# zeahmed/NeuralASR

Hardware: AMD Instinct MI355X
Metric: audio-frames/sec (fwd+bwd+CTC+Adam) at batch 16 per GPU (higher is better)
Workload: dtype f32

## Files before the change

### neuralasr_amd/build.py

```python
import os
import subprocess
import sys
from concurrent.futures import ThreadPoolExecutor

HERE = os.path.dirname(os.path.abspath(__file__))
CSRC = os.path.join(HERE, 'csrc')
LIB = os.path.join(HERE, 'libnasr.so')
KT_LIB = os.path.join(HERE, 'libnasr_kt.so')
KT_DIR = os.path.join(HERE, '..', 'tests', 'kernel_harness')
KT_SRCS = ['harness.hip', 'rec_harness.hip']
KT_HEADERS = [os.path.join(KT_DIR, 'arena.h')]
KT_OBJS = ['gemm.o', 'gemm_tph.o', 'optim.o', 'lstm.o', 'lstm_persist.o', 'lstm_wide.o']
SOURCES = ['gemm.hip', 'gemm_tph.hip', 'lstm.hip', 'rows.hip', 'lstm_persist.hip', 'lstm_wide.hip', 'ctc.hip', 'dense.hip', 'optim.hip', 'nasr_layout.hip',
           'nasr_rec.hip', 'nasr_batch.hip', 'nasr_pass.hip', 'nasr_stream.hip', 'nasr_lstm.hip', 'nasr_api.hip', 'nasr_comm.hip', 'beam.cpp',
           'wavenet.hip', 'nasr_wavenet.hip', 'las.hip', 'las_beam.hip', 'nasr_las.hip', 'mfcc.hip', 'nasr_fz.hip', 'resample.hip', 'wave_aug.hip']
HEADERS = [os.path.join(CSRC, 'kernels.h'), os.path.join(CSRC, 'lstm_device.h'), os.path.join(CSRC, 'nasr_ctx.h'), os.path.join(CSRC, 'nasr_lstm.h'), os.path.join(CSRC, 'wavenet.h'), os.path.join(CSRC, 'las.h'), os.path.join(CSRC, 'las_beam.h'), os.path.join(CSRC, 'resample.h'), os.path.join(CSRC, 'wave_aug.h'),
           os.path.join(CSRC, 'mfcc.h'), os.path.join(CSRC, 'nasr_fz.h'), os.path.join(HERE, '..', 'include', 'nasr.h')]
FLAGS = ['--offload-arch=gfx950', '-O3', '-std=c++17', '-fPIC', '-Wall', '-Wno-unused-function']
EXTRA_FLAGS = {'wave_aug.hip': ['-fno-slp-vectorize']}


def _hipcc():
    for c in (os.environ.get('HIPCC'), '/opt/rocm/bin/hipcc', 'hipcc'):
        if c and (os.path.isabs(c) and os.path.exists(c) or not os.path.isabs(c)):
            return c
    return 'hipcc'


def _stale(target, deps):
    if not os.path.exists(target):
        return True
    t = os.path.getmtime(target)
    return any(os.path.getmtime(d) > t for d in deps if os.path.exists(d))


def build(force=False, verbose=False):
    hipcc = _hipcc()
    bdir = os.path.join(HERE, 'build')
    os.makedirs(bdir, exist_ok=True)
    jobs = []
    objs = []
    for s in SOURCES:
        src = os.path.join(CSRC, s)
        obj = os.path.join(bdir, os.path.splitext(s)[0] + '.o')
        objs.append(obj)
        if force or _stale(obj, [src] + HEADERS):
            jobs.append([hipcc] + FLAGS + EXTRA_FLAGS.get(s, []) + ['-c', src, '-o', obj])

    def run(cmd):
        if verbose:
            print(' '.join(cmd), flush=True)
        r = subprocess.run(cmd, capture_output=True, text=True)
        if r.returncode != 0:
            raise RuntimeError('hipcc failed:\n' + ' '.join(cmd) + '\n' + r.stdout + r.stderr)
        if verbose and r.stderr.strip():
            print(r.stderr)

    kt_objs = []
    for s in KT_SRCS:
        src = os.path.join(KT_DIR, s)
        obj = os.path.join(bdir, 'kt_' + os.path.splitext(s)[0] + '.o')
        kt_objs.append(obj)
        if force or _stale(obj, [src] + KT_HEADERS + HEADERS):
            jobs.append([hipcc] + FLAGS + ['-c', src, '-o', obj])

    with ThreadPoolExecutor(max_workers=min(4, max(1, len(jobs)))) as ex:
        list(ex.map(run, jobs))
    if force or jobs or _stale(LIB, objs):
        run([hipcc, '--offload-arch=gfx950', '-shared', '-fPIC', '-o', LIB] + objs + ['-lpthread'])
    kt_objs += [os.path.join(bdir, o) for o in KT_OBJS]
    if force or jobs or _stale(KT_LIB, kt_objs):
        run([hipcc, '--offload-arch=gfx950', '-shared', '-fPIC', '-o', KT_LIB] + kt_objs)
    return LIB


if __name__ == '__main__':
    print(build(force='--force' in sys.argv, verbose=True))
```

### neuralasr_amd/csrc/ctc.hip

```cpp
#include "kernels.h"

#include <cmath>
#include <cstdlib>
#include <type_traits>

namespace nasr {

constexpr float NEG = -1e30f;
typedef __attribute__((address_space(3))) void* lds_ptr_t;
typedef const __attribute__((address_space(1))) void* gbl_ptr_t;

__device__ __forceinline__ float ldf(const float* base, unsigned byteoff) {
  return *reinterpret_cast<const float*>(reinterpret_cast<const char*>(base) + byteoff);
}
__device__ __forceinline__ void stf(float* base, unsigned byteoff, float v) {
  *reinterpret_cast<float*>(reinterpret_cast<char*>(base) + byteoff) = v;
}

__device__ __forceinline__ float lse3(float a, float b, float c) {
  const float m = fmaxf(a, fmaxf(b, c));
  const float L2E = 1.44269504088896341f, LN2 = 0.69314718055994531f;
  const float s = __builtin_amdgcn_exp2f((a - m) * L2E) + __builtin_amdgcn_exp2f((b - m) * L2E) +
                  __builtin_amdgcn_exp2f((c - m) * L2E);
  return m + __builtin_amdgcn_logf(s) * LN2;
}

__device__ __forceinline__ float lane_up1(float v, float edge) {
  return __int_as_float(__builtin_amdgcn_update_dpp(__float_as_int(edge), __float_as_int(v), 0x138, 0xf, 0xf, false));
}
__device__ __forceinline__ float lane_down1(float v, float edge) {
  return __int_as_float(__builtin_amdgcn_update_dpp(__float_as_int(edge), __float_as_int(v), 0x130, 0xf, 0xf, false));
}

__device__ __forceinline__ float wave_max(float v) {
#pragma unroll
  for (int o = 32; o > 0; o >>= 1) v = fmaxf(v, __shfl_xor(v, o));
  return v;
}
__device__ __forceinline__ float wave_max_dpp(float v) {
  auto dpp = [](float x, auto ctrl) {
    return __int_as_float(__builtin_amdgcn_update_dpp(__float_as_int(x), __float_as_int(x), decltype(ctrl)::value, 0xf, 0xf, false));
  };
  v = fmaxf(v, dpp(v, std::integral_constant<int, 0xB1>{}));
  v = fmaxf(v, dpp(v, std::integral_constant<int, 0x4E>{}));
  v = fmaxf(v, dpp(v, std::integral_constant<int, 0x141>{}));
  v = fmaxf(v, dpp(v, std::integral_constant<int, 0x140>{}));
  const int vi = __float_as_int(v);
  const float r0 = __int_as_float(__builtin_amdgcn_readlane(vi, 0)), r1 = __int_as_float(__builtin_amdgcn_readlane(vi, 16));
  const float r2 = __int_as_float(__builtin_amdgcn_readlane(vi, 32)), r3 = __int_as_float(__builtin_amdgcn_readlane(vi, 48));
  return fmaxf(fmaxf(r0, r1), fmaxf(r2, r3));
}
__device__ __forceinline__ float wave_sum(float v) {
#pragma unroll
  for (int o = 32; o > 0; o >>= 1) v += __shfl_xor(v, o);
  return v;
}

static bool ctc_fast_ok(const CtcDims& d) { return d.lprobs && d.goff && d.Cp == 32 && d.C <= 31 && d.KS >= 2; }

__global__ __launch_bounds__(256) void ctc_logz_kernel(const float* __restrict__ logits, const int* __restrict__ seq_len,
                                                       float* __restrict__ logz, float* __restrict__ lprobs, int Tp, int B, int Bp,
                                                       int C, int Cp) {
  const int row = blockIdx.x * 4 + (threadIdx.x >> 6);
  const int lane = threadIdx.x & 63;
  if (row >= Tp * Bp) return;
  const int t = row / Bp, b = row % Bp;
  if (b >= B || t >= seq_len[b]) return;
  const float* x = logits + (size_t)row * Cp;
  float m = NEG;
  for (int c = lane; c < C; c += 64) m = fmaxf(m, x[c]);
  m = wave_max(m);
  float s = 0.f;
  for (int c = lane; c < C; c += 64) s += __expf(x[c] - m);
  s = wave_sum(s);
  const float z = m + __logf(s);
  if (lane == 0) logz[row] = z;
  if (lprobs)
    for (int c = lane; c < Cp; c += 64) lprobs[(size_t)row * Cp + c] = c < C ? (x[c] - z) * 1.44269504088896341f : NEG;
}

void launch_ctc_logz(const CtcDims& d, const float* logits, const int* seq_len, float* logz, hipStream_t st) {
  const int rows = d.Tp * d.Bp;
  hipLaunchKernelGGL(ctc_logz_kernel, dim3((rows + 3) / 4), dim3(256), 0, st, logits, seq_len, logz, ctc_fast_ok(d) ? d.lprobs : nullptr,
                     d.Tp, d.B, d.Bp, d.C, d.Cp);
}

template <int KS>
__device__ __forceinline__ void ctc_ab_log(
    const float* __restrict__ logits, const float* __restrict__ logz, const int* __restrict__ labels,
    const int* __restrict__ label_len, const int* __restrict__ seq_len, float* __restrict__ alpha,
    float* __restrict__ beta, double* __restrict__ aoff, double* __restrict__ boff, float* __restrict__ nll,
    double* __restrict__ logp_out, int Bp, int Cp, int C, int Lmax, int Tws, float* fin) {
  constexpr int G = 4;
  const int b = blockIdx.x;
  const int lane = threadIdx.x & 63, w = threadIdx.x >> 6;
  const int L = label_len[b], Tb = seq_len[b], S = 2 * L + 1;
  const int blank = C - 1;
  const int* lab = labels + (size_t)b * Lmax;

  int ext[KS];
  bool act[KS], skip[KS];
#pragma unroll
  for (int i = 0; i < KS; ++i) {
    const int s = lane * KS + i;
    act[i] = s < S;
    ext[i] = (act[i] && (s & 1)) ? lab[s >> 1] : blank;
  }
  const unsigned rstride = (unsigned)Bp * (unsigned)Cp;
  const float* lg = logits + (size_t)b * Cp;
  const float* lz = logz + b;
  auto emit = [&](int t, float (&e)[KS]) {
    const float z = ldf(lz, (unsigned)t * (unsigned)Bp * 4u);
    float v[KS];
#pragma unroll
    for (int i = 0; i < KS; ++i) v[i] = ldf(lg, ((unsigned)t * rstride + (unsigned)ext[i]) * 4u);
#pragma unroll
    for (int i = 0; i < KS; ++i) e[i] = act[i] ? v[i] - z : NEG;
  };
  auto emit_raw = [&](int t, float (&v)[KS], float& z) {
    z = ldf(lz, (unsigned)t * (unsigned)Bp * 4u);
#pragma unroll
    for (int i = 0; i < KS; ++i) v[i] = ldf(lg, ((unsigned)t * rstride + (unsigned)ext[i]) * 4u);
  };
  auto emit_finish = [&](float (&v)[KS], float z, float (&e)[KS]) {
    asm volatile("" : "+v"(z));
#pragma unroll
    for (int i = 0; i < KS; ++i) {
      float x = v[i];
      asm volatile("" : "+v"(x));
      e[i] = act[i] ? x - z : NEG;
    }
  };
  float* ws = (w == 0 ? alpha : beta) + (size_t)b * Tws * KS * 64;
  double* off = (w == 0 ? aoff : boff) + (size_t)b * Tws;
  auto store = [&](int t, const float (&a)[KS], double o) {
#pragma unroll
    for (int i = 0; i < KS; ++i) stf(ws, (((unsigned)t * KS + i) * 64u + (unsigned)lane) * 4u, a[i]);
    if (lane == 0) off[t] = o;
  };
  auto renorm = [&](float (&a)[KS], double& o) {
    float m = a[0];
#pragma unroll
    for (int i = 1; i < KS; ++i) m = fmaxf(m, a[i]);
    m = wave_max_dpp(m);
#pragma unroll
    for (int i = 0; i < KS; ++i) a[i] = a[i] > 0.5f * NEG ? a[i] - m : NEG;
    o += (double)m;
  };

  if (w == 0) {
#pragma unroll
    for (int i = 0; i < KS; ++i) {
      const int s = lane * KS + i;
      const int e2 = (act[i] && s >= 2 && (s & 1)) ? lab[(s >> 1) - 1] : blank;
      skip[i] = act[i] && s >= 2 && ext[i] != blank && ext[i] != e2;
    }
    float a[KS], e[G][KS];
    double A = 0.0;
    emit(0, e[0]);
#pragma unroll
    for (int i = 0; i < KS; ++i) {
      const int s = lane * KS + i;
      a[i] = (s < 2 && act[i]) ? e[0][i] : NEG;
    }
    store(0, a, A);
#pragma unroll
    for (int k = 0; k < G; ++k) emit(min(1 + k, Tb - 1), e[k]);
    for (int t0 = 1; t0 < Tb; t0 += G) {
      float vn[G][KS], zn[G];
#pragma unroll
      for (int k = 0; k < G; ++k) emit_raw(min(t0 + G + k, Tb - 1), vn[k], zn[k]);
      renorm(a, A);
#pragma unroll
      for (int k = 0; k < G; ++k) {
        const int t = t0 + k;
        const bool live = t < Tb;
        float p1 = lane_up1(a[KS - 1], NEG);
        float p2 = (KS >= 2) ? lane_up1(a[KS >= 2 ? KS - 2 : 0], NEG) : __shfl_up(a[0], 2);
        if (KS == 1 && lane <= 1) p2 = NEG;
        float na[KS];
#pragma unroll
        for (int i = 0; i < KS; ++i) {
          const float x1 = (i >= 1) ? a[i >= 1 ? i - 1 : 0] : p1;
          const float x2 = (i >= 2) ? a[i >= 2 ? i - 2 : 0] : (i == 1 ? p1 : p2);
          na[i] = e[k][i] + lse3(a[i], x1, skip[i] ? x2 : NEG);
        }
#pragma unroll
        for (int i = 0; i < KS; ++i) a[i] = live ? na[i] : a[i];
        store(t, a, A);
      }
      asm volatile("" ::: "memory");
#pragma unroll
      for (int k = 0; k < G; ++k) emit_finish(vn[k], zn[k], e[k]);
    }
#pragma unroll
    for (int i = 0; i < KS; ++i) fin[lane * KS + i] = a[i];
    __builtin_amdgcn_s_waitcnt(0xc07f);
    if (lane == 0) {
      const float x = fin[S - 1];
      const float y = S > 1 ? fin[S - 2] : NEG;
      const double lp = A + (double)lse3(x, y, NEG);
      logp_out[b] = lp;
      nll[b] = (float)(-lp);
    }
  } else {
#pragma unroll
    for (int i = 0; i < KS; ++i) {
      const int s = lane * KS + i;
      const int e2 = (s + 2 < S && (s & 1)) ? lab[(s >> 1) + 1] : blank;
      skip[i] = (s + 2 < S) && e2 != blank && e2 != ext[i];
    }
    float bt[KS], e[G][KS];
    double Bo = 0.0;
#pragma unroll
    for (int i = 0; i < KS; ++i) {
      const int s = lane * KS + i;
      bt[i] = (act[i] && (s == S - 1 || s == S - 2)) ? 0.f : NEG;
    }
    store(Tb - 1, bt, Bo);
#pragma unroll
    for (int k = 0; k < G; ++k) emit(max(Tb - 1 - k, 0), e[k]);
    for (int t0 = Tb - 2; t0 >= 0; t0 -= G) {
      float vn[G][KS], zn[G];
#pragma unroll
      for (int k = 0; k < G; ++k) emit_raw(max(t0 - G - k + 1, 0), vn[k], zn[k]);
      renorm(bt, Bo);
#pragma unroll
      for (int k = 0; k < G; ++k) {
        const int t = t0 - k;
        const bool live = t >= 0;
        float bb[KS];
#pragma unroll
        for (int i = 0; i < KS; ++i) bb[i] = bt[i] + e[k][i];
        float n1 = lane_down1(bb[0], NEG);
        float n2 = (KS >= 2) ? lane_down1(bb[KS >= 2 ? 1 : 0], NEG) : __shfl_down(bb[0], 2);
        if (KS == 1 && lane >= 62) n2 = NEG;
        float nb[KS];
#pragma unroll
        for (int i = 0; i < KS; ++i) {
          const float x1 = (i + 1 < KS) ? bb[i + 1 < KS ? i + 1 : 0] : n1;
          const float x2 = (i + 2 < KS) ? bb[i + 2 < KS ? i + 2 : 0] : (i + 1 < KS ? n1 : n2);
          nb[i] = lse3(bb[i], x1, skip[i] ? x2 : NEG);
        }
#pragma unroll
        for (int i = 0; i < KS; ++i) bt[i] = live ? nb[i] : bt[i];
        if (live) store(t, bt, Bo);
      }
      asm volatile("" ::: "memory");
#pragma unroll
      for (int k = 0; k < G; ++k) emit_finish(vn[k], zn[k], e[k]);
    }
  }
}

constexpr int FAST_G = 4, FAST_CH = 32, FAST_RING = 64;

typedef float fast_f2 __attribute__((ext_vector_type(2)));
typedef float fast_f3 __attribute__((ext_vector_type(3)));
typedef float fast_f4 __attribute__((ext_vector_type(4)));
template <int KS>
__device__ __forceinline__ void fast_store(float* base, unsigned voff, const float (&a)[KS]) {
#pragma unroll
  for (int j = 0; j + 4 <= KS; j += 4) {
    const fast_f4 v = {a[j], a[j + 1], a[j + 2], a[j + 3]};
    asm volatile("global_store_dwordx4 %0, %1, %2 offset:%3\n\ts_nop 1" : : "v"(voff), "v"(v), "s"(base), "n"(j * 4) : "memory");
  }
  constexpr int j = KS & ~3;
  if constexpr (KS % 4 == 3) {
    const fast_f3 v = {a[j], a[j + 1], a[j + 2]};
    asm volatile("global_store_dwordx3 %0, %1, %2 offset:%3\n\ts_nop 1" : : "v"(voff), "v"(v), "s"(base), "n"(j * 4) : "memory");
  } else if constexpr (KS % 4 == 2) {
    const fast_f2 v = {a[j], a[j + 1]};
    asm volatile("global_store_dwordx2 %0, %1, %2 offset:%3" : : "v"(voff), "v"(v), "s"(base), "n"(j * 4) : "memory");
  } else if constexpr (KS % 4 == 1) {
    asm volatile("global_store_dword %0, %1, %2 offset:%3" : : "v"(voff), "v"(a[j]), "s"(base), "n"(j * 4) : "memory");
  }
}
__device__ __forceinline__ float fast_up(float v) { return lane_up1(v, NEG); }
__device__ __forceinline__ float fast_down(float v) { return lane_down1(v, NEG); }

__device__ __forceinline__ float lse3_2(float a, float b, float c) {
  const float mx = __builtin_fmaxf(a, __builtin_fmaxf(b, c));
  const float md = __builtin_amdgcn_fmed3f(a, b, c);
  const float mn = __builtin_fminf(a, __builtin_fminf(b, c));
  const float s = 1.f + __builtin_amdgcn_exp2f(md - mx) + __builtin_amdgcn_exp2f(mn - mx);
  return mx + __builtin_amdgcn_logf(s);
}

template <int KS, bool fwd>
__device__ __forceinline__ void ctc_fast_walk(const int* __restrict__ labels, const int* __restrict__ label_len,
                                              const int* __restrict__ seq_len, float* __restrict__ alpha, float* __restrict__ beta,
                                              double* __restrict__ goff, float* __restrict__ nll, double* __restrict__ logp_out,
                                              const float* __restrict__ lprobs, int Bp, int C, int Lmax, int Tws, int KG, float* ring,
                                              float* fin, int* sync) {
  static_assert(KS >= 2, "two states per lane at least: the skip transition then never reaches past the neighbour lane");
  constexpr int G = FAST_G;
  constexpr double LN2 = 0.693147180559945309417;
  const int b = blockIdx.x;
  const int lane = threadIdx.x & 63, w = fwd ? 0 : 1;
  const int L = label_len[b], Tb = seq_len[b], S = 2 * L + 1;
  const int blank = C - 1;
  const int* lab = labels + (size_t)b * Lmax;
  int ext[KS];
  bool skip[KS];
#pragma unroll
  for (int i = 0; i < KS; ++i) {
    const int s = lane * KS + i;
    const bool act = s < S;
    ext[i] = act ? ((s & 1) ? lab[s >> 1] : blank) : 31;
    if (fwd) {
      const int e2 = (act && s >= 2 && (s & 1)) ? lab[(s >> 1) - 1] : blank;
      skip[i] = act && s >= 2 && ext[i] != blank && ext[i] != e2;
    } else {
      const int e2 = (s + 2 < S && (s & 1)) ? lab[(s >> 1) + 1] : blank;
      skip[i] = (s + 2 < S) && e2 != blank && e2 != ext[i];
    }
  }
  const int npos = Tb - 1;
  float* rg = ring + w * (FAST_RING * 32);
  auto read_group = [&](int g, float (&e)[G][KS]) {
    asm volatile("" ::: "memory");
    const float* r0 = rg + ((G * g) & (FAST_RING - 1)) * 32;
#pragma unroll
    for (int i = 0; i < KS; ++i)
#pragma unroll
      for (int k = 0; k < G; ++k) e[k][i] = r0[k * 32 + ext[i]];
    asm volatile("" ::: "memory");
  };
  const unsigned sync_lds = (unsigned)(size_t)((lds_ptr_t)sync);
  auto wait_ready = [&](int n) {
    for (unsigned spin = 0; spin < (1u << 24); ++spin) {
      int v;
      asm volatile("ds_read_b32 %0, %1\n\ts_waitcnt lgkmcnt(0)" : "=v"(v) : "v"(sync_lds) : "memory");
      if (v >= n) break;
      __builtin_amdgcn_s_sleep(1);
    }
  };
  float* ws = (fwd ? alpha : beta) + (size_t)b * Tws * KS * 64;
  double* go = goff + ((size_t)b * 2 + w) * KG;
  constexpr unsigned ROWB = 64u * KS * 4u;
  const unsigned lane_off = (unsigned)lane * (KS * 4u);
  auto store = [&](int t, const float (&a)[KS]) { fast_store<KS>(ws, lane_off + (unsigned)t * ROWB, a); };

  float a[KS];
  double A = 0.0;
  if (fwd) {
    const float* y0 = lprobs + (size_t)b * 32;
#pragma unroll
    for (int i = 0; i < KS; ++i) a[i] = (lane * KS + i < 2) ? y0[ext[i]] : NEG;
    store(0, a);
  } else {
#pragma unroll
    for (int i = 0; i < KS; ++i) {
      const int s = lane * KS + i;
      a[i] = (s < S && (s == S - 1 || s == S - 2)) ? 0.f : NEG;
    }
    store(Tb - 1, a);
  }
  if (lane == 0) go[0] = 0.0;
  auto group = [&](int g, float (&e)[G][KS], float (&en)[G][KS], auto maskedc) {
    constexpr bool MASKED = decltype(maskedc)::value;
    const int p0 = G * g;
    read_group(g + 1, en);
    {
      float m = a[0];
#pragma unroll
      for (int i = 1; i < KS; ++i) m = fmaxf(m, a[i]);
      m = wave_max_dpp(m);
#pragma unroll
      for (int i = 0; i < KS; ++i) a[i] = a[i] > 0.5f * NEG ? a[i] - m : NEG;
      A += (double)m;
      if (lane == 0) go[g + 1] = A;
    }
#pragma unroll
    for (int k = 0; k < G; ++k) {
      float na[KS];
      if (fwd) {
        const float p1 = fast_up(a[KS - 1]), p2 = fast_up(a[KS - 2]);
#pragma unroll
        for (int i = 0; i < KS; ++i) {
          const float x1 = (i >= 1) ? a[i >= 1 ? i - 1 : 0] : p1;
          const float x2 = (i >= 2) ? a[i >= 2 ? i - 2 : 0] : (i == 1 ? p1 : p2);
          na[i] = e[k][i] + lse3_2(a[i], x1, skip[i] ? x2 : NEG);
        }
      } else {
        float bb[KS];
#pragma unroll
        for (int i = 0; i < KS; ++i) bb[i] = a[i] + e[k][i];
        const float n1 = fast_down(bb[0]), n2 = fast_down(bb[1]);
#pragma unroll
        for (int i = 0; i < KS; ++i) {
          const float x1 = (i + 1 < KS) ? bb[i + 1 < KS ? i + 1 : 0] : n1;
          const float x2 = (i + 2 < KS) ? bb[i + 2 < KS ? i + 2 : 0] : (i + 1 < KS ? n1 : n2);
          na[i] = lse3_2(bb[i], x1, skip[i] ? x2 : NEG);
        }
      }
      if constexpr (MASKED) {
        const bool live = p0 + k < npos;
#pragma unroll
        for (int i = 0; i < KS; ++i) a[i] = live ? na[i] : a[i];
      } else {
#pragma unroll
        for (int i = 0; i < KS; ++i) a[i] = na[i];
      }
      store(fwd ? p0 + k + 1 : max(Tb - 2 - p0 - k, 0), a);
    }
  };
  if (npos > 0) {
    const int nch = (npos + FAST_CH - 1) / FAST_CH;
    wait_ready(1);
    float e[G][KS], en[G][KS];
    read_group(0, e);
    for (int c = 0; c < nch; ++c) {
      for (int gi = 0; gi < FAST_CH / G; gi += 2) {
        const int g = c * (FAST_CH / G) + gi;
        if (G * g >= npos) break;
        if (G * g + G <= npos) group(g, e, en, std::false_type{});
        else group(g, e, en, std::true_type{});
        if (G * (g + 1) >= npos) break;
        if (gi + 2 == FAST_CH / G && c + 1 < nch) wait_ready(c + 2);
        if (G * (g + 1) + G <= npos) group(g + 1, en, e, std::false_type{});
        else group(g + 1, en, e, std::true_type{});
      }
      asm volatile("s_waitcnt lgkmcnt(0)\n\tds_write_b32 %0, %1 offset:%2" : : "v"(sync_lds), "v"(c + 1), "n"(4 * (1 + w)) : "memory");
    }
  }
  if (fwd) {
#pragma unroll
    for (int i = 0; i < KS; ++i) fin[lane * KS + i] = a[i];
    __builtin_amdgcn_s_waitcnt(0xc07f);
    if (lane == 0) {
      const float x = fin[S - 1];
      const float y = S > 1 ? fin[S - 2] : NEG;
      const double lp = (A + (double)lse3_2(x, y, NEG)) * LN2;
      logp_out[b] = lp;
      nll[b] = (float)(-lp);
    }
  }
}

__device__ __forceinline__ void ctc_fast_loader(const float* __restrict__ lprobs, const int* __restrict__ seq_len, int Bp, float* ring,
                                                volatile int* sync) {
  const int b = blockIdx.x, lane = threadIdx.x & 63;
  const int Tb = seq_len[b], npos = Tb - 1;
  const int nch = (npos + FAST_CH - 1) / FAST_CH;
  const char* yb = reinterpret_cast<const char*>(lprobs + (size_t)b * 32);
  const unsigned rstride = (unsigned)Bp * 32u * 4u;
  for (int n = 0; n < nch; ++n) {
    if (n >= 2)
      for (unsigned spin = 0; (sync[1] < n - 1 || sync[2] < n - 1) && spin < (1u << 24); ++spin) __builtin_amdgcn_s_sleep(1);
#pragma unroll
    for (int w = 0; w < 2; ++w)
#pragma unroll
      for (int q = 0; q < 4; ++q) {
        const int p = min(FAST_CH * n + 8 * q + (lane >> 3), npos - 1);
        const int f = w == 0 ? p + 1 : Tb - 1 - p;
        const char* g = yb + (size_t)((unsigned)f * rstride) + (lane & 7) * 16;
        __builtin_amdgcn_global_load_lds((gbl_ptr_t)g, (lds_ptr_t)(ring + w * (FAST_RING * 32) + (((FAST_CH * n) & (FAST_RING - 1)) + 8 * q) * 32),
                                         16, 0, 0);
      }
    asm volatile("s_waitcnt vmcnt(0)" ::: "memory");
    if (lane == 0) sync[0] = n + 1;
  }
}

template <int KS, bool FAST>
__global__ __launch_bounds__(FAST ? 192 : 128) void ctc_alpha_beta_kernel(
    const float* __restrict__ logits, const float* __restrict__ logz, const float* __restrict__ lprobs,
    const int* __restrict__ labels, const int* __restrict__ label_len, const int* __restrict__ seq_len,
    float* __restrict__ alpha, float* __restrict__ beta, double* __restrict__ aoff, double* __restrict__ boff,
    double* __restrict__ goff, float* __restrict__ nll, double* __restrict__ logp_out, int Bp, int Cp, int C, int Lmax, int Tws,
    int KG) {
  __shared__ float fin[64 * KS];
  if constexpr (FAST) {
    __shared__ __attribute__((aligned(1024))) float ring[2 * FAST_RING * 32];
    __shared__ int sync[3];
    if (threadIdx.x < 3) sync[threadIdx.x] = 0;
    __syncthreads();
    constexpr int K2 = KS >= 2 ? KS : 2;
    const int w = __builtin_amdgcn_readfirstlane(threadIdx.x >> 6);
    if (w == 0)
      ctc_fast_walk<K2, true>(labels, label_len, seq_len, alpha, beta, goff, nll, logp_out, lprobs, Bp, C, Lmax, Tws, KG, ring, fin, sync);
    else if (w == 1)
      ctc_fast_walk<K2, false>(labels, label_len, seq_len, alpha, beta, goff, nll, logp_out, lprobs, Bp, C, Lmax, Tws, KG, ring, fin, sync);
    else
      ctc_fast_loader(lprobs, seq_len, Bp, ring, sync);
  } else {
    ctc_ab_log<KS>(logits, logz, labels, label_len, seq_len, alpha, beta, aoff, boff, nll, logp_out, Bp, Cp, C, Lmax, Tws, fin);
  }
}

void launch_ctc_alpha_beta(const CtcDims& d, const float* logits, const float* logz, const int* labels,
                           const int* label_len, const int* seq_len, float* alpha, float* beta, double* aoff,
                           double* boff, float* nll, double* logp, hipStream_t st) {
  const bool fast = ctc_fast_ok(d);
  const int KG = d.Tws / FAST_G + 3;
#define NASR_AB2(K, F)                                                                                                   \
  hipLaunchKernelGGL((ctc_alpha_beta_kernel<K, F>), dim3(d.B), dim3(F ? 192 : 128), 0, st, logits, logz, d.lprobs, labels, \
                     label_len, seq_len, alpha, beta, aoff, boff, d.goff, nll, logp, d.Bp, d.Cp, d.C, d.Lmax, d.Tws, KG)
#define NASR_AB(K)                                                                                                       \
  if (fast) NASR_AB2(K, true);                                                                                           \
  else NASR_AB2(K, false)
  switch (d.KS) {
    case 1: NASR_AB2(1, false); break;
    case 2: NASR_AB(2); break;
    case 3: NASR_AB(3); break;
    case 4: NASR_AB(4); break;
    case 5: NASR_AB(5); break;
    case 6: NASR_AB(6); break;
    case 7: NASR_AB(7); break;
    case 8: NASR_AB(8); break;
    case 9: case 10: case 11: case 12: NASR_AB(12); break;
    default: NASR_AB(16); break;
  }
#undef NASR_AB2
#undef NASR_AB
}

__global__ __launch_bounds__(256) void ctc_grad_kernel(float* __restrict__ logits, const float* __restrict__ logz,
                                                       const int* __restrict__ label_len,
                                                       const int* __restrict__ seq_len,
                                                       const int* __restrict__ cstart, const int* __restrict__ cpos,
                                                       const float* __restrict__ alpha, const float* __restrict__ beta,
                                                       const double* __restrict__ aoff, const double* __restrict__ boff,
                                                       const double* __restrict__ logp, const double* __restrict__ goff,
                                                       float scale, int Tp, int B, int Bp, int C, int Cp, int Lmax, int KS,
                                                       int Tws, int KG) {
  extern __shared__ __attribute__((aligned(16))) float wl_all[];
  const int wv = threadIdx.x >> 6, lane = threadIdx.x & 63;
  const int row = blockIdx.x * (blockDim.x >> 6) + wv;
  if (row >= Tp * Bp) return;
  const int t = row / Bp, b = row % Bp;
  float* x = logits + (size_t)row * Cp;
  if (b >= B || t >= seq_len[b]) {
    for (int c = lane; c < Cp; c += 64) x[c] = 0.f;
    return;
  }
  float* wl = wl_all + (size_t)wv * KS * 64;
  const int L = label_len[b], S = 2 * L + 1;
  const float* al = alpha + ((size_t)b * Tws + t) * KS * 64;
  const float* be = beta + ((size_t)b * Tws + t) * KS * 64;
  float blank = 0.f;
  if (goff) {
    const int Tb = seq_len[b];
    const int ga = t == 0 ? 0 : 1 + (t - 1) / FAST_G, gb = t == Tb - 1 ? 0 : 1 + (Tb - 2 - t) / FAST_G;
    const float coff2 = (float)(goff[(size_t)b * 2 * KG + ga] + goff[((size_t)b * 2 + 1) * KG + gb] - logp[b] * 1.44269504088896341);
    for (int i = 0; i < KS; ++i) {
      const int s = lane * KS + i;
      const float wgt = s < S ? exp2f(al[lane * KS + i] + be[lane * KS + i] + coff2) : 0.f;
      wl[s] = wgt;
      if (!(s & 1)) blank += wgt;
    }
  } else {
    const float coff = (float)(aoff[(size_t)b * Tws + t] + boff[(size_t)b * Tws + t] - logp[b]);
    for (int i = 0; i < KS; ++i) {
      const int s = lane * KS + i;
      const float wgt = s < S ? __expf(al[i * 64 + lane] + be[i * 64 + lane] + coff) : 0.f;
      wl[s] = wgt;
      if (!(s & 1)) blank += wgt;
    }
  }
  blank = wave_sum(blank);
  __builtin_amdgcn_s_waitcnt(0xc07f);
  const float z = logz[row];
  const int* cs = cstart + (size_t)b * (C + 1);
  const int* cp = cpos + (size_t)b * Lmax;
  for (int c = lane; c < Cp; c += 64) {
    float g = 0.f;
    if (c < C) {
      float post = blank;
      if (c < C - 1) {
        post = 0.f;
        const int j1 = cs[c + 1];
        for (int j = cs[c]; j < j1; ++j) post += wl[2 * cp[j] + 1];
      }
      g = (__expf(x[c] - z) - post) * scale;
    }
    x[c] = g;
  }
}

void launch_ctc_grad(const CtcDims& d, float* logits, const float* logz, const int* label_len, const int* seq_len,
                     const int* cstart, const int* cpos, const float* alpha, const float* beta, const double* aoff,
                     const double* boff, const double* logp, float scale, hipStream_t st) {
  const int rows = d.Tp * d.Bp;
  const int rpb = 4;
  hipLaunchKernelGGL(ctc_grad_kernel, dim3((rows + rpb - 1) / rpb), dim3(64 * rpb), (size_t)rpb * d.KS * 64 * 4, st, logits,
                     logz, label_len, seq_len, cstart, cpos, alpha, beta, aoff, boff, logp, ctc_fast_ok(d) ? d.goff : nullptr, scale,
                     d.Tp, d.B, d.Bp, d.C, d.Cp, d.Lmax, d.KS, d.Tws, d.Tws / FAST_G + 3);
}

__global__ void mean_kernel(const float* __restrict__ v, int n, float* __restrict__ out) {
  if (threadIdx.x == 0 && blockIdx.x == 0) {
    float s = 0.f;
    for (int i = 0; i < n; ++i) s += v[i];
    *out = s / (float)n;
  }
}
void launch_mean(const float* v, int n, float* out, hipStream_t st) {
  hipLaunchKernelGGL(mean_kernel, dim3(1), dim3(64), 0, st, v, n, out);
}

__global__ __launch_bounds__(256) void argmax_kernel(const float* __restrict__ logits, const int* __restrict__ seq_len,
                                                     int* __restrict__ am, int Tp, int B, int Bp, int C, int Cp) {
  const int row = blockIdx.x * 4 + (threadIdx.x >> 6);
  const int lane = threadIdx.x & 63;
  if (row >= Tp * Bp) return;
  const int t = row / Bp, b = row % Bp;
  if (b >= B || t >= seq_len[b]) return;
  const float* x = logits + (size_t)row * Cp;
  float best = -INFINITY;
  int bi = 0x7fffffff;
  for (int c = lane; c < C; c += 64) {
    const float v = x[c];
    if (v > best) { best = v; bi = c; }
  }
#pragma unroll
  for (int o = 32; o > 0; o >>= 1) {
    const float ov = __shfl_xor(best, o);
    const int oi = __shfl_xor(bi, o);
    if (ov > best || (ov == best && oi < bi)) { best = ov; bi = oi; }
  }
  if (lane == 0) am[row] = bi;
}

__global__ __launch_bounds__(64) void collapse_kernel(const int* __restrict__ am, const int* __restrict__ seq_len,
                                                      int* __restrict__ ids, int* __restrict__ lens, int Tp, int B, int Bp,
                                                      int blank) {
  const int b = blockIdx.x, lane = threadIdx.x;
  const int Tb = seq_len[b];
  int n = 0, carry = -1;
  for (int t0 = 0; t0 < Tb; t0 += 64) {
    const int t = t0 + lane;
    const int k = t < Tb ? am[t * Bp + b] : blank;
    int prev = __shfl_up(k, 1);
    if (lane == 0) prev = carry;
    const bool keep = t < Tb && k != prev && k != blank;
    const unsigned long long m = __ballot(keep);
    if (keep) ids[(size_t)b * Tp + n + __popcll(m & ((1ull << lane) - 1ull))] = k;
    n += __popcll(m);
    carry = __shfl(k, 63);
  }
  if (lane == 0) lens[b] = n;
}

void launch_greedy(const CtcDims& d, const float* logits, const int* seq_len, int* argmax_ws, int* ids, int* lens,
                   hipStream_t st) {
  const int rows = d.Tp * d.Bp;
  hipLaunchKernelGGL(argmax_kernel, dim3((rows + 3) / 4), dim3(256), 0, st, logits, seq_len, argmax_ws, d.Tp, d.B, d.Bp,
                     d.C, d.Cp);
  hipLaunchKernelGGL(collapse_kernel, dim3(d.B), dim3(64), 0, st, argmax_ws, seq_len, ids, lens, d.Tp, d.B, d.Bp, d.C - 1);
}

constexpr int ALIGN_G = 4;
constexpr int ALIGN_LDS_BYTES = 56 * 1024;
constexpr int align_bpf(int KS) { return KS <= 4 ? 8 : KS <= 8 ? 16 : 32; }
constexpr int align_words(int KS) { return align_bpf(KS) * ALIGN_G / 32; }
static int align_ks(int L) {
  const int KS = std::max(1, (2 * std::max(L, 0) + 1 + 63) / 64);
  return KS <= 1 ? 2 : KS <= 8 ? KS : (KS <= 12 ? 12 : 16);
}
static int align_groups(int F) { return (std::max(F, 1) - 1 + ALIGN_G - 1) / ALIGN_G; }

bool ctc_align_bp_in_lds(int F, int L) { return (size_t)align_groups(F) * 256 * align_words(align_ks(L)) <= (size_t)ALIGN_LDS_BYTES; }
size_t ctc_align_ws_words(int B, int F, int L) {
  return ctc_align_bp_in_lds(F, L) ? 0 : (size_t)B * align_groups(F) * 64 * align_words(align_ks(L));
}

template <int KS, bool LDSBP>
__global__ __launch_bounds__(64) void ctc_align_kernel(const float* __restrict__ logits, const float* __restrict__ logz,
                                                       const int* __restrict__ labels, const int* __restrict__ label_len,
                                                       const int* __restrict__ seq_len, unsigned* __restrict__ bpws,
                                                       size_t bp_stride, int* __restrict__ path, double* __restrict__ score,
                                                       int Tp, int Bp, int Cp, int C, int Lmax) {
  static_assert(KS >= 2 && KS <= 16, "two states per lane at least (the skip never reaches past the neighbour lane), 32 bits of back-pointers at most");
  constexpr int G = ALIGN_G, BPF = align_bpf(KS), W = align_words(KS);
  extern __shared__ __attribute__((aligned(16))) unsigned bplds[];
  __shared__ float fin[64 * KS];
  const int b = blockIdx.x, lane = threadIdx.x;
  const int L = label_len[b], F = seq_len[b], S = 2 * L + 1;
  const int blank = C - 1;
  const int* lab = labels + (size_t)b * Lmax;
  int ext[KS];
  bool act[KS], skip[KS];
#pragma unroll
  for (int i = 0; i < KS; ++i) {
    const int s = lane * KS + i;
    act[i] = s < S;
    ext[i] = (act[i] && (s & 1)) ? lab[s >> 1] : blank;
    const int e2 = (act[i] && s >= 2 && (s & 1)) ? lab[(s >> 1) - 1] : blank;
    skip[i] = act[i] && s >= 2 && ext[i] != blank && ext[i] != e2;
  }
  const unsigned rstride = (unsigned)Bp * (unsigned)Cp;
  const float* lg = logits + (size_t)b * Cp;
  auto gather = [&](int t, float (&x)[KS]) {
#pragma unroll
    for (int i = 0; i < KS; ++i) x[i] = ldf(lg, ((unsigned)t * rstride + (unsigned)ext[i]) * 4u);
  };
  unsigned* bp = LDSBP ? bplds : bpws + (size_t)b * bp_stride;
  const int ngroups = (F - 1 + G - 1) / G;

  constexpr int NB = KS <= 4 ? 8 : KS <= 8 ? 4 : 2, PF = G * NB;
  float v[KS], e[PF][KS];
  gather(0, e[0]);
#pragma unroll
  for (int i = 0; i < KS; ++i) v[i] = (act[i] && lane * KS + i < 2) ? e[0][i] : NEG;
#pragma unroll
  for (int k = 0; k < PF; ++k) gather(min(1 + k, F - 1), e[k]);
  for (int g0 = 0; g0 < ngroups; g0 += NB) {
    float vn[PF][KS];
#pragma unroll
    for (int k = 0; k < PF; ++k) gather(min(1 + G * g0 + PF + k, F - 1), vn[k]);
#pragma unroll
    for (int sub = 0; sub < NB; ++sub) {
      const int g = g0 + sub;
      if (g < ngroups) {
        const int t0 = 1 + G * g;
        {
          float m = v[0];
#pragma unroll
          for (int i = 1; i < KS; ++i) m = fmaxf(m, v[i]);
          m = wave_max_dpp(m);
#pragma unroll
          for (int i = 0; i < KS; ++i) v[i] = v[i] > 0.5f * NEG ? v[i] - m : NEG;
        }
        unsigned w[W];
#pragma unroll
        for (int j = 0; j < W; ++j) w[j] = 0u;
#pragma unroll
        for (int k = 0; k < G; ++k) {
          const bool live = t0 + k < F;
          const float p1 = lane_up1(v[KS - 1], NEG), p2 = lane_up1(v[KS - 2], NEG);
          float nv[KS];
          unsigned code = 0u;
#pragma unroll
          for (int i = 0; i < KS; ++i) {
            const float x1 = (i >= 1) ? v[i >= 1 ? i - 1 : 0] : p1;
            const float x2r = (i >= 2) ? v[i >= 2 ? i - 2 : 0] : (i == 1 ? p1 : p2);
            const float x2 = skip[i] ? x2r : NEG;
            float best = v[i];
            unsigned c = 0u;
            if (x1 > best) { best = x1; c = 1u; }
            if (x2 > best) { best = x2; c = 2u; }
            nv[i] = act[i] ? best + e[sub * G + k][i] : NEG;
            code |= c << (2 * i);
          }
#pragma unroll
          for (int i = 0; i < KS; ++i) v[i] = live ? nv[i] : v[i];
          w[(k * BPF) / 32] |= code << ((k * BPF) % 32);
        }
#pragma unroll
        for (int j = 0; j < W; ++j) bp[((size_t)g * 64 + lane) * W + j] = w[j];
      }
    }
    asm volatile("" ::: "memory");
#pragma unroll
    for (int k = 0; k < PF; ++k)
#pragma unroll
      for (int i = 0; i < KS; ++i) {
        float x = vn[k][i];
        asm volatile("" : "+v"(x));
        e[k][i] = x;
      }
  }
#pragma unroll
  for (int i = 0; i < KS; ++i) fin[lane * KS + i] = v[i];
  if (!LDSBP) __threadfence();
  __syncthreads();

  int s = (S > 1 && fin[S - 2] > fin[S - 1]) ? S - 2 : S - 1;
  s = __builtin_amdgcn_readfirstlane(s);
  int* prow = path + (size_t)b * Tp;
  const float* lz = logz + b;
  double acc = 0.0;
  auto frame_score = [&](int t, int st) {
    const int cls = (st & 1) ? lab[st >> 1] : blank;
    return (double)lg[(size_t)t * rstride + cls] - (double)lz[(size_t)t * Bp];
  };
  const int nturns = (F - 1 + 63) / 64;
  for (int c = nturns - 1; c >= 0; --c) {
    const int tlo = 64 * c + 1, thi = min(tlo + 63, F - 1);
    const int g0 = 16 * c;
    if (!LDSBP) {
      const int nw = min(16, ngroups - g0) * 64 * W;
      __syncthreads();
      for (int j = lane; j < nw; j += 64) bplds[j] = bp[(size_t)g0 * 64 * W + j];
      __syncthreads();
    }
    const int gbase = LDSBP ? 0 : g0;
    int mine = 0;
    for (int t = thi; t >= tlo; --t) {
      if (lane == t - tlo) mine = s;
      const int g = (t - 1) >> 2, k = (t - 1) & 3;
      const int ls = s / KS, i = s - ls * KS;
      const unsigned word = bplds[((g - gbase) * 64 + ls) * W + ((k * BPF) >> 5)];
      s = max(s - (int)((word >> (((k * BPF) & 31) + 2 * i)) & 3u), 0);
      s = __builtin_amdgcn_readfirstlane(s);
    }
    const int t = tlo + lane;
    if (t <= thi) {
      prow[t] = mine;
      acc += frame_score(t, mine);
    }
  }
  if (lane == 0) {
    prow[0] = s;
    acc += frame_score(0, s);
  }
  for (int t = F + lane; t < Tp; t += 64) prow[t] = -1;
#pragma unroll
  for (int o = 32; o > 0; o >>= 1) acc += __shfl_xor(acc, o);
  if (lane == 0) score[b] = acc;
}

int launch_ctc_align(const CtcDims& d, int Fmax, const float* logits, const float* logz, const int* labels, const int* label_len,
                     const int* seq_len, unsigned* bpws, int* path, double* score, hipStream_t st) {
  if ((size_t)d.Tp * d.Bp * d.Cp * 4 >= ((size_t)1 << 32)) return -1;
  const int KS = align_ks(d.Lmax);
  const bool lds = ctc_align_bp_in_lds(Fmax, d.Lmax);
  const int W = align_words(KS);
  const size_t stride = (size_t)align_groups(Fmax) * 64 * W;
  const size_t shm = lds ? std::max<size_t>(stride * 4, 16) : (size_t)16 * 64 * W * 4;
  if (!lds && !bpws) return -2;
#define NASR_AL2(K, LD)                                                                                                     \
  hipLaunchKernelGGL((ctc_align_kernel<K, LD>), dim3(d.B), dim3(64), shm, st, logits, logz, labels, label_len, seq_len, bpws, \
                     stride, path, score, d.Tp, d.Bp, d.Cp, d.C, d.Lmax)
#define NASR_AL(K)                                                                                                          \
  if (lds) NASR_AL2(K, true);                                                                                               \
  else NASR_AL2(K, false)
  switch (KS) {
    case 2: NASR_AL(2); break;
    case 3: NASR_AL(3); break;
    case 4: NASR_AL(4); break;
    case 5: NASR_AL(5); break;
    case 6: NASR_AL(6); break;
    case 7: NASR_AL(7); break;
    case 8: NASR_AL(8); break;
    case 12: NASR_AL(12); break;
    default: NASR_AL(16); break;
  }
#undef NASR_AL2
#undef NASR_AL
  return 0;
}

}
```

### neuralasr_amd/csrc/gemm.hip

```cpp
#include "kernels.h"

namespace nasr {

typedef float f32x16 __attribute__((ext_vector_type(16)));

constexpr int BM = 128, BN = 128, BK = 16, LDT = 132;

struct GemmParams {
  const float* A;
  const float* B;
  float* C;
  int M, N, K, lda, ldb, ldc;
  const int* a_map;
  int a_shift, a_rows;
  const int* c_map;
  const float* bias;
  int split_k, kchunk;
  float* slabs;
};

__device__ __forceinline__ int phys_row(const int* map, int shift, int rows, int logical) {
  int r = map ? map[logical] : logical + shift;
  return (r >= 0 && r < rows) ? r : -1;
}

__device__ __forceinline__ float4 ld4(const float* __restrict__ p) { return *reinterpret_cast<const float4*>(p); }
__device__ __forceinline__ float4 sel4(bool ok, float4 v) {
  return make_float4(ok ? v.x : 0.f, ok ? v.y : 0.f, ok ? v.z : 0.f, ok ? v.w : 0.f);
}

template <bool ACOL, bool BCOL>
__global__ __launch_bounds__(256, 2) void gemm_kernel(GemmParams p) {
  __shared__ __attribute__((aligned(16))) float As[2][BK][LDT];
  __shared__ __attribute__((aligned(16))) float Bs[2][BK][LDT];
  const int tid = threadIdx.x, lane = tid & 63, w = tid >> 6;
  const int m0 = blockIdx.y * BM, n0 = blockIdx.x * BN;
  const int kbeg = blockIdx.z * p.kchunk;
  const int kend = min(p.K, kbeg + p.kchunk);
  const int nk = (kend - kbeg + BK - 1) / BK;
  const float* __restrict__ Ag = p.A;
  const float* __restrict__ Bg = p.B;

  constexpr int NS = BK / 8, KQ = BK / 4;
  bool aok[NS], bok[NS];
  size_t ao[NS], bo[NS];
#pragma unroll
  for (int j = 0; j < NS; ++j) {
    const int idx = tid + 256 * j;
    const int r = idx / KQ, kq = idx % KQ, q = idx & 31;
    if (!ACOL) {
      const int pa = (m0 + r < p.M) ? phys_row(p.a_map, p.a_shift, p.a_rows, m0 + r) : -1;
      aok[j] = pa >= 0;
      ao[j] = aok[j] ? (size_t)pa * p.lda + 4 * kq : 0;
    } else {
      aok[j] = (m0 + 4 * q < p.M);
      ao[j] = aok[j] ? (size_t)(m0 + 4 * q) : 0;
    }
    if (BCOL) {
      bok[j] = n0 + r < p.N;
      bo[j] = bok[j] ? (size_t)(n0 + r) * p.ldb + 4 * kq : 0;
    } else {
      bok[j] = (n0 + 4 * q < p.N);
      bo[j] = bok[j] ? (size_t)(n0 + 4 * q) : 0;
    }
  }

  float4 ra[NS], rb[NS];
#define NASR_GLOAD(K0)                                                                              \
  _Pragma("unroll") for (int j = 0; j < NS; ++j) {                                                  \
    const int kk_ = (tid + 256 * j) >> 5;                                                           \
    const bool kr_ = (K0) + 4 * ((tid + 256 * j) % KQ) < kend, kc_ = (K0) + kk_ < kend;             \
    if (!ACOL) {                                                                                    \
      const bool o_ = aok[j] && kr_;                                                                \
      ra[j] = sel4(o_, ld4(Ag + (o_ ? ao[j] + (K0) : 0)));                                          \
    } else {                                                                                        \
      const int pr_ = kc_ ? phys_row(p.a_map, p.a_shift, p.a_rows, (K0) + kk_) : -1;                \
      const bool o_ = aok[j] && pr_ >= 0;                                                           \
      ra[j] = sel4(o_, ld4(Ag + (o_ ? (size_t)pr_ * p.lda + ao[j] : 0)));                           \
    }                                                                                               \
    if (BCOL) {                                                                                     \
      const bool o_ = bok[j] && kr_;                                                                \
      rb[j] = sel4(o_, ld4(Bg + (o_ ? bo[j] + (K0) : 0)));                                          \
    } else {                                                                                        \
      const bool o_ = bok[j] && kc_;                                                                \
      rb[j] = sel4(o_, ld4(Bg + (o_ ? (size_t)((K0) + kk_) * p.ldb + bo[j] : 0)));                  \
    }                                                                                               \
  }
#define NASR_LSTORE(BUF)                                                                            \
  _Pragma("unroll") for (int j = 0; j < NS; ++j) {                                                  \
    const int idx_ = tid + 256 * j;                                                                 \
    const int r_ = idx_ / KQ, kq_ = idx_ % KQ, kk_ = idx_ >> 5, q_ = idx_ & 31;                     \
    if (!ACOL) {                                                                                    \
      As[BUF][4 * kq_ + 0][r_] = ra[j].x; As[BUF][4 * kq_ + 1][r_] = ra[j].y;                       \
      As[BUF][4 * kq_ + 2][r_] = ra[j].z; As[BUF][4 * kq_ + 3][r_] = ra[j].w;                       \
    } else {                                                                                        \
      *reinterpret_cast<float4*>(&As[BUF][kk_][4 * q_]) = ra[j];                                    \
    }                                                                                               \
    if (BCOL) {                                                                                     \
      Bs[BUF][4 * kq_ + 0][r_] = rb[j].x; Bs[BUF][4 * kq_ + 1][r_] = rb[j].y;                       \
      Bs[BUF][4 * kq_ + 2][r_] = rb[j].z; Bs[BUF][4 * kq_ + 3][r_] = rb[j].w;                       \
    } else {                                                                                        \
      *reinterpret_cast<float4*>(&Bs[BUF][kk_][4 * q_]) = rb[j];                                    \
    }                                                                                               \
  }

  f32x16 acc00, acc01, acc10, acc11;
#pragma unroll
  for (int r = 0; r < 16; ++r) { acc00[r] = 0.f; acc01[r] = 0.f; acc10[r] = 0.f; acc11[r] = 0.f; }

  const int wm = (w >> 1) * 64, wn = (w & 1) * 64;
  const int li = lane & 31, lk = lane >> 5;

  if (nk > 0) {
    NASR_GLOAD(kbeg);
    NASR_LSTORE(0);
  }
  __syncthreads();
  for (int kt = 0; kt < nk; ++kt) {
    const int buf = kt & 1;
    const bool more = kt + 1 < nk;
    if (more) NASR_GLOAD(kbeg + (kt + 1) * BK);
    float a0 = As[buf][lk][wm + li], a1 = As[buf][lk][wm + 32 + li];
    float b0 = Bs[buf][lk][wn + li], b1 = Bs[buf][lk][wn + 32 + li];
#pragma unroll
    for (int ks = 0; ks < BK / 2; ++ks) {
      float na0 = 0.f, na1 = 0.f, nb0 = 0.f, nb1 = 0.f;
      if (ks + 1 < BK / 2) {
        const int k = 2 * (ks + 1) + lk;
        na0 = As[buf][k][wm + li]; na1 = As[buf][k][wm + 32 + li];
        nb0 = Bs[buf][k][wn + li]; nb1 = Bs[buf][k][wn + 32 + li];
      }
      acc00 = __builtin_amdgcn_mfma_f32_32x32x2f32(a0, b0, acc00, 0, 0, 0);
      acc01 = __builtin_amdgcn_mfma_f32_32x32x2f32(a0, b1, acc01, 0, 0, 0);
      acc10 = __builtin_amdgcn_mfma_f32_32x32x2f32(a1, b0, acc10, 0, 0, 0);
      acc11 = __builtin_amdgcn_mfma_f32_32x32x2f32(a1, b1, acc11, 0, 0, 0);
      a0 = na0; a1 = na1; b0 = nb0; b1 = nb1;
    }
    if (more) NASR_LSTORE(buf ^ 1);
    __syncthreads();
  }
#undef NASR_GLOAD
#undef NASR_LSTORE

#pragma unroll
  for (int t = 0; t < 4; ++t) {
    const int mi = t >> 1, ni = t & 1;
    const f32x16 acc = t == 0 ? acc00 : t == 1 ? acc01 : t == 2 ? acc10 : acc11;
    const int col = n0 + wn + 32 * ni + li;
    if (col >= p.N) continue;
    const float bv = (p.bias && p.split_k == 1) ? p.bias[col] : 0.f;
#pragma unroll
    for (int r = 0; r < 16; ++r) {
      const int row = m0 + wm + 32 * mi + (r & 3) + 8 * (r >> 2) + 4 * lk;
      if (row >= p.M) continue;
      if (p.split_k > 1) {
        p.slabs[((size_t)blockIdx.z * p.M + row) * p.N + col] = acc[r];
      } else {
        const int pr = p.c_map ? p.c_map[row] : row;
        if (pr >= 0) p.C[(size_t)pr * p.ldc + col] = acc[r] + bv;
      }
    }
  }
}

__global__ __launch_bounds__(256) void gemm_reduce_kernel(GemmParams p) {
  const int64_t n4 = (int64_t)p.M * p.N / 4;
  for (int64_t i = blockIdx.x * (int64_t)blockDim.x + threadIdx.x; i < n4; i += (int64_t)gridDim.x * blockDim.x) {
    const int64_t e = i * 4;
    const int row = (int)(e / p.N), col = (int)(e % p.N);
    float4 s = *reinterpret_cast<const float4*>(p.slabs + e);
    for (int k = 1; k < p.split_k; ++k) {
      const float4 v = *reinterpret_cast<const float4*>(p.slabs + (size_t)k * p.M * p.N + e);
      s.x += v.x; s.y += v.y; s.z += v.z; s.w += v.w;
    }
    if (p.bias) { s.x += p.bias[col]; s.y += p.bias[col + 1]; s.z += p.bias[col + 2]; s.w += p.bias[col + 3]; }
    const int pr = p.c_map ? p.c_map[row] : row;
    if (pr >= 0) *reinterpret_cast<float4*>(p.C + (size_t)pr * p.ldc + col) = s;
  }
}

int gemm_pick_split(int M, int N, int K) {
  const int tiles = ((M + BM - 1) / BM) * ((N + BN - 1) / BN);
  int s = (512 + tiles - 1) / tiles;
  const int max_s = K / 128;
  if (s > max_s) s = max_s;
  if (s < 1) s = 1;
  return s;
}

void launch_gemm(const GemmDesc& g, hipStream_t st) {
  GemmParams p;
  p.A = g.A; p.B = g.B; p.C = g.C;
  p.M = g.M; p.N = g.N; p.K = g.K; p.lda = g.lda; p.ldb = g.ldb; p.ldc = g.ldc;
  p.a_map = g.a_map; p.a_shift = g.a_shift; p.a_rows = g.a_rows; p.c_map = g.c_map; p.bias = g.bias;
  p.split_k = g.split_k < 1 ? 1 : g.split_k;
  p.slabs = g.slabs;
  int kt = (g.K + BK - 1) / BK;
  int per = (kt + p.split_k - 1) / p.split_k;
  p.kchunk = per * BK;
  p.split_k = (kt + per - 1) / per;
  dim3 grid((g.N + BN - 1) / BN, (g.M + BM - 1) / BM, p.split_k), block(256);
  if (!g.a_col && !g.b_col) hipLaunchKernelGGL((gemm_kernel<false, false>), grid, block, 0, st, p);
  else if (g.a_col && !g.b_col) hipLaunchKernelGGL((gemm_kernel<true, false>), grid, block, 0, st, p);
  else if (!g.a_col && g.b_col) hipLaunchKernelGGL((gemm_kernel<false, true>), grid, block, 0, st, p);
  else hipLaunchKernelGGL((gemm_kernel<true, true>), grid, block, 0, st, p);
  if (p.split_k > 1) {
    int64_t n4 = (int64_t)g.M * g.N / 4;
    int blocks = (int)((n4 + 255) / 256);
    if (blocks > 2048) blocks = 2048;
    hipLaunchKernelGGL(gemm_reduce_kernel, dim3(blocks), dim3(256), 0, st, p);
  }
}

}
```

### neuralasr_amd/csrc/kernels.h

```cpp
#pragma once
#include <hip/hip_runtime.h>
#include <stdint.h>

namespace nasr {

const char* test_hook(const char* name);

struct GemmDesc {
  const float* A;
  const float* B;
  float* C;
  int M, N, K;
  int lda, ldb, ldc;
  bool a_col;
  bool b_col;
  const int* a_map;
  int a_shift;
  int a_rows;
  const int* c_map;
  const float* bias;
  int split_k;
  float* slabs;
};
void launch_gemm(const GemmDesc& g, hipStream_t st);
int gemm_pick_split(int M, int N, int K);

int tp_split2_parts(int rows);
int gemm_tp_tile_rows(int M);
size_t tph_bytes(int rows, int K);
size_t tph_scale_ws_floats(int rows, int K);
void launch_tph_scales(const float* src, int rows, int K, int ld, float* row_scale, float* row_inv, float* col_scale,
                       float* col_inv, float* ws, hipStream_t st);
constexpr int TPH_MAX_JOBS = 16;
struct TphScaleJob { const float* src; int rows, K, ld; float *row_scale, *row_inv, *col_scale, *col_inv; };
size_t tph_scale_batch_ws_floats(const TphScaleJob* jobs, int n);
void launch_tph_scales_batch(const TphScaleJob* jobs, int n, float* ws, hipStream_t st);
void launch_tph_scales_from_parts(const float* rowpart, int nrp, int rows, float* row_scale, float* row_inv, const float* colpart,
                                  int ncp, int K, float* col_scale, float* col_inv, hipStream_t st);
void launch_fill(float* p, float v, int n, hipStream_t st);
void launch_tph_split2(const float* src, unsigned char* tpN, unsigned char* tpT, int rows, int K, int ld,
                       const float* row_scale, float rs, const float* col_scale, float cs, float* colpart, hipStream_t st,
                       const int* rowmap = nullptr, const int* rowmap2 = nullptr, int col2 = 0);
void launch_gather_rows(float* dst, const float* src, const int* map, int n, float fill, hipStream_t st);
struct GemmTPHDesc {
  const unsigned char* A;
  const unsigned char* B;
  float* C;
  int M, N, K;
  int nkbA, nkbB;
  int ldc;
  int a_kshift;
  const float* bias;
  const float* a_inv;
  const float* b_inv;
  int split_k;
  float* slabs;
  int tile_rows;
  int nbatch;
  size_t a_bstride, b_bstride;
  int64_t c_bstride, ainv_bstride, binv_bstride;
  int a_kshift1;
  bool side;
  const int* c_map;
};
hipError_t gemm_tph_prepare();
int gemm_tph_pick_split(int M, int N, int K, int nbatch = 1);
void launch_gemm_tph(const GemmTPHDesc& g, hipStream_t st);

struct LstmDims { int T, B, Bp, H, Hp, D; };
void launch_repack_u(const float* U, float* Uf, float* Ub, int Hp, hipStream_t st);
int lstm_bwd_partials(int Hp);
struct StepWindow {
  LstmDims dm;
  const float *Uf, *Ub;
  float *hstate, *partial, *dcstate;
  float *gates, *cbuf, *out;
  float* dg;
  const float* dout;
  const int* seq_len;
  float forget_bias;
  const float* c0;
};
void lstm_steps_fwd(const StepWindow& w, int s0, int s1, hipStream_t st);
void lstm_steps_bwd(const StepWindow& w, int s0, int s1, hipStream_t st);
struct StepLeft { float *partial, *dc; };
float* lstm_steps_dcin(const StepWindow& w, int s);
StepLeft lstm_steps_left(const StepWindow& w, int s);
constexpr int LA_MAX_SLOTS = 64;
struct LaSlots { int held[LA_MAX_SLOTS], n[LA_MAX_SLOTS], emit[LA_MAX_SLOTS]; };
void launch_stream_load_state(const float* state, float* himg, float* cimg, int S, int H, int Bp, int Hp, hipStream_t st, int D = 1);
void launch_stream_save_state(const float* out, const float* cbuf, const LaSlots& sl, float* state, int S, int H, int Bp, int DH,
                              hipStream_t st);

struct LcGeom { int C, W, K, T, Bp; };
__host__ __device__ inline int lc_last_window(int len, int C, int W) { return len <= W ? 0 : (len - W + C - 1) / C; }
__host__ __device__ inline int lc_window_rows(int len, int k, int C, int W) {
  if (len < 1 || k > lc_last_window(len, C, W)) return 0;
  return len - k * C < W ? len - k * C : W;
}
void launch_lc_load_carry(const float* out, const float* cbuf, const int* wlen, int k, const LcGeom& g, float* himg, float* cimg,
                          int Hp, int D, hipStream_t st);
void launch_lc_carry_out(const float* part, int np, const float* dcs, const int* wlen_k, float* drow, float* dcc, int Bp, int Hp,
                         int DH, hipStream_t st);
void launch_lc_carry_dc(float* dcin, const float* dcc, int n, hipStream_t st);

void launch_pack_feats(const float* feats_bm, float* X0, int B, int Bp, int T, int F, int Fp, hipStream_t st);
void launch_expand_context(const float* centre, const float* pad, const int* seq_len, float* X0, int B, int Bp, int T,
                           int ctx, int ncep, int Fp, hipStream_t st);
void launch_expand_context_masked(const float* centre, const float* pad, const int* seq_len, const int* masks, int nm,
                                  int static_width, float* X0, int B, int Bp, int T, int ctx, int ncep, int Fp,
                                  hipStream_t st);
void launch_la_window(const float* hold_in, const float* fresh, const LaSlots& sl, float* win, float* hold_out, int S, int R,
                      int Tc, int T, int rows, int F, hipStream_t st);
void launch_lc_gather(const float* src, const int* wlen, float* dst, const LcGeom& g, int F, hipStream_t st);
void launch_lc_emit(const float* outv, const int* seq_len, float* top, const LcGeom& g, int DH, hipStream_t st);
void launch_lc_scatter(const float* dtop, const int* seq_len, const int* wlen, float* doutv, const LcGeom& g, int DH,
                       hipStream_t st);

struct XcdCtl {
  unsigned xcc_count[8];
  unsigned error;
  unsigned pad[23];
};
static_assert(sizeof(XcdCtl) == 32 * sizeof(unsigned), "the control blocks' head is 32 words");
struct PersistCtl : XcdCtl {
  unsigned flags[8 * 128];
#if defined(NASR_PSTAMP) && NASR_PSTAMP
  unsigned stamps[256][12];
#endif
};
bool persist_supported(int Hp);
size_t persist_image_floats(int Hp, bool bwd);
size_t persist_xch_floats(int Hp);
size_t persist_hx_bytes(int Hp);
size_t persist_px_bytes();
hipError_t persist_prepare();
constexpr int PERSIST_MAX_MATS = 16;
void launch_repack_persist(const float* P, const int64_t* offs, int n, float* Upf, float* Upb, int Hp, const float* col_scale,
                           hipStream_t st);
void launch_lstm_persist_fwd(const LstmDims& dm, const float* Upf, const float* cinv, float* gates, float* cbuf,
                             float* out, const int* seq_len, float* xch, PersistCtl* ctl, unsigned* sticky, float* fault,
                             float forget_bias, hipStream_t st, bool ctl_zeroed = false);
void launch_lstm_persist_bwd(const LstmDims& dm, const float* Upb, const float* gates, float* dgbuf, const float* cbuf,
                             const float* dout, const int* seq_len, float* xch, PersistCtl* ctl, unsigned* sticky,
                             float* fault, hipStream_t st, bool ctl_zeroed = false, float* rowpart = nullptr,
                             float* colpart = nullptr, bool lean = false);
size_t persist_dgmax_floats(int T, int Bp, int Hp, int D);

struct WideCtl : XcdCtl {
  unsigned stamps[160];
};
struct WideGeom {
  int T, Bp, Hp, D, d;
  int inject;
  int scale_shift;
  float* fault;
};
bool wide_supported(int Hp, int Bp);
size_t wide_image_bytes(int Hp);
size_t wide_hx_bytes(int Bp);
size_t wide_part_bytes(int Bp);
hipError_t wide_prepare();
void launch_repack_wide(const float* U, const float* cs, void* Uw, int Hp, hipStream_t st);
void launch_lstm_wide_fwd(const LstmDims& dm, int d, const void* Uw, const float* cinv, float* gates, float* cbuf,
                          float* out, const int* seq_len, void* hx, float* part, WideCtl* ctl, unsigned* sticky,
                          float* fault, float forget_bias, hipStream_t st);

size_t wide_px_bytes(int Bp);
void launch_repack_wide_bwd(const float* U, const float* rs, void* Uwb, int Hp, hipStream_t st);
void launch_wide_row_scales(const LstmDims& dm, const float* dout, const int* seq_len, float* srow, hipStream_t st);
void launch_lstm_wide_bwd(const LstmDims& dm, int d, const void* Uwb, const float* rinv, const float* srow,
                          const float* gates, float* dgbuf, const float* cbuf, const float* dout, const int* seq_len,
                          float* inbox, void* px, WideCtl* ctl, unsigned* sticky, float* fault, hipStream_t st);

void launch_dense_act(float* z, int R, int Bp, int B, int W, int ld, float clip, float p, uint32_t seed, uint32_t counter,
                      int stage, hipStream_t st);
void launch_dense_act_bwd(float* dy, const float* y, int64_t n, float clip, float p, hipStream_t st);

struct CtcDims {
  int Tp;
  int B, Bp, C, Cp, Lmax;
  int KS;
  int Tws;
  float* lprobs = nullptr;
  double* goff = nullptr;
};
void launch_ctc_logz(const CtcDims& d, const float* logits, const int* seq_len, float* logz, hipStream_t st);
void launch_ctc_alpha_beta(const CtcDims& d, const float* logits, const float* logz, const int* labels,
                           const int* label_len, const int* seq_len, float* alpha, float* beta, double* aoff,
                           double* boff, float* nll, double* logp, hipStream_t st);
void launch_ctc_grad(const CtcDims& d, float* logits, const float* logz, const int* label_len, const int* seq_len,
                     const int* cstart, const int* cpos, const float* alpha, const float* beta, const double* aoff,
                     const double* boff, const double* logp, float scale, hipStream_t st);
void launch_mean(const float* v, int n, float* out, hipStream_t st);
void launch_greedy(const CtcDims& d, const float* logits, const int* seq_len, int* argmax_ws, int* ids, int* lens,
                   hipStream_t st);

bool ctc_align_bp_in_lds(int F, int L);
size_t ctc_align_ws_words(int B, int F, int L);
int launch_ctc_align(const CtcDims& d, int F, const float* logits, const float* logz, const int* labels, const int* label_len,
                     const int* seq_len, unsigned* bpws, int* path, double* score, hipStream_t st);

struct AdamDev { long long step; float lr_t; int applied; };
void launch_adam(float* p, float* m, float* v, const float* g, int64_t n, AdamDev* state, float lr, float beta1, float beta2,
                 float eps, float gscale, const float* fault, hipStream_t st);
struct ClipDev { double last_norm; float last_coef, s; int skip, pad; double window_max_norm; long long steps, clipped, skipped; };
constexpr int GRAD_SUMSQ_MAX_BLOCKS = 1024;
int grad_sumsq_blocks(int64_t n);
void launch_adam_clipped(float* p, float* m, float* v, const float* g, int64_t n, AdamDev* state, ClipDev* clip, double* part,
                         float lr, float beta1, float beta2, float eps, float gscale, float max_norm, const float* fault,
                         hipStream_t st);
void launch_colsum(const float* M, int R, int N, int ld, float* out, float* ws, hipStream_t st);
void launch_colsum_parts(const float* part, int nparts, int N, float* out, hipStream_t st);
void launch_reduce_slabs(const float* slabs, int S, int64_t n, float* out, hipStream_t st);
void launch_reduce_slabs_rows(const float* slabs, int S, int M, int N, int ldc, const int* map, float* out, hipStream_t st);
void launch_ring_standin(float* buf, int64_t n, int nblocks, int passes, hipStream_t st);

}
```

### neuralasr_amd/csrc/nasr_batch.hip

```cpp
#include "nasr_lstm.h"

using namespace nasr;
using namespace nasr_impl;

namespace nasr_impl {

int ensure_ctc_buffers(nasr_ctx* h, int B, int Bp, int T, int Tp, int Lmax, bool* grew) {
  const int KS = std::max(1, (2 * std::max(Lmax, 0) + 1 + 63) / 64);
  if (KS > 16) return h->fail(NASR_ERR_ARG, "label length > 511 not supported by the CTC lattice kernel");
  const int KSa = KS <= 1 ? 2 : KS <= 8 ? KS : (KS <= 12 ? 12 : 16);
  bool ok = true;
  ok &= h->logits.ensure((size_t)Tp * Bp * h->Cp * 4, grew);
  ok &= h->logz.ensure((size_t)Tp * Bp * 4, grew);
  ok &= h->alpha.ensure((size_t)B * (T + 8) * KSa * 64 * 4, grew);
  ok &= h->beta.ensure((size_t)B * (T + 8) * KSa * 64 * 4, grew);
  ok &= h->aoff.ensure((size_t)B * (T + 8) * 8, grew);
  ok &= h->boff.ensure((size_t)B * (T + 8) * 8, grew);
  ok &= h->logp.ensure((size_t)Bp * 8, grew);
  ok &= h->ctcprobs.ensure((size_t)Tp * Bp * h->Cp * 4, grew);
  ok &= h->ctckexp.ensure((size_t)B * 2 * ((T + 8) / 4 + 3) * 8, grew);
  ok &= h->nll.ensure((size_t)Bp * 4, grew);
  ok &= h->loss.ensure(16, grew);
  ok &= h->amax.ensure((size_t)Tp * Bp * 4, grew);
  ok &= h->ids.ensure((size_t)B * Tp * 4, grew);
  ok &= h->lens.ensure((size_t)Bp * 4, grew);
  if (!ok) return h->fail(NASR_ERR_HIP, "hipMalloc failed while sizing batch buffers");
  return KSa;
}

int ensure_shape(nasr_ctx* h, int B, int T, int Lmax, bool chunked) {
  switch (h->family) {
    case Family::WaveNet: return wn_ensure_shape(h, B, T, Lmax);
    case Family::Las: return las_ensure_shape(h, B, T, Lmax);
    default: return lstm_ensure_shape(h, B, T, Lmax, chunked);
  }
}

int lstm_ensure_shape(nasr_ctx* h, int B, int T, int Lmax, bool chunked) {
  LstmState* const ls = h->lstm.get();
  const int Bp = rup(B, 16);
  const int Tp = lstm_logit_frames(h, T);
  LcGeom lg{};
  if (chunked) {
    lg.C = ls->lcC; lg.W = std::min(ls->lcC + ls->lcR, T); lg.K = lc_last_window(T, lg.C, lg.W) + 1; lg.T = T; lg.Bp = Bp;
    if ((int64_t)lg.K * lg.W * Bp > ((int64_t)1 << 22))
      return h->fail(NASR_ERR_ARG, "chunked batch: " + std::to_string(lg.K) + " windows of " + std::to_string(lg.W) + " rows x " +
                                       std::to_string(Bp) + " utterances are more than 2^22 rows: use a longer chunk or a shorter look-ahead");
  }
  const int Tv = chunked ? lg.K * lg.W : T;
  const size_t R = (size_t)Tv * Bp;
  const int D = ls->D, Hp = ls->Hp, N4 = ls->N4;
  bool grew = false;
  bool ok = true;
  const int KSa = ensure_ctc_buffers(h, B, Bp, T, Tp, Lmax, &grew);
  if (KSa < 0) return KSa;
  ok &= h->X0.ensure(R * h->Fp * 4, &grew);
  if (chunked) {
    ok &= ls->lc_x0.ensure((size_t)T * Bp * h->Fp * 4, &grew);
    ok &= ls->lc_top.ensure((size_t)T * Bp * ls->Pinp * 4, &grew) && ls->lc_dtop.ensure((size_t)T * Bp * ls->Pinp * 4, &grew);
    ok &= ls->lc_cimg.ensure((size_t)D * Bp * Hp * 4, &grew) && ls->lc_dcc.ensure((size_t)Bp * Hp * 4, &grew);
  }
  ok &= h->seqbuf.ensure((size_t)Bp * 4, &grew);
  ok &= ls->dout.ensure(R * D * Hp * 4, &grew);
  ok &= ls->hstate.ensure((size_t)2 * D * Bp * Hp * 4, &grew);
  ok &= ls->partial.ensure((size_t)2 * D * (Hp / 32) * Bp * Hp * 4, &grew);
  ok &= ls->dcstate.ensure((size_t)2 * D * Bp * Hp * 4, &grew);
  ok &= ls->dgbuf.ensure(R * D * N4 * 4, &grew);
  if (ls->rec_kind == RecKind::Persist) ok &= ls->dgmax.ensure(persist_dgmax_floats(T, Bp, Hp, D) * 4, &grew);
  {
    int ipmax = h->Fp, wmax = D * N4;
    for (int l = 0; l < ls->L; ++l) ipmax = std::max(ipmax, ls->Ip[l]);
    for (int i = 0; i < ls->ndense; ++i) { ipmax = std::max(ipmax, ls->dIp[i]); wmax = std::max(wmax, ls->dWp[i]); }
    ok &= ls->XTP.ensure(tph_bytes((int)R, ipmax), &grew);
    ok &= ls->X0TTP.ensure(tph_bytes(ls->Ip[0], (int)R), &grew);
    for (int l = 0; l < ls->L; ++l) ok &= ls->OTT[l].ensure(tph_bytes(D * Hp, (int)R), &grew);
    ok &= ls->GTP.ensure(tph_bytes((int)R, wmax), &grew);
    ok &= ls->GTTP.ensure(tph_bytes(wmax, (int)R), &grew);
    if (ls->wg_overlap) {
      ok &= ls->GTTP2.ensure(tph_bytes(wmax, (int)R), &grew);
      ok &= ls->sc_gc2.ensure((size_t)wmax);
    }
    if (ls->ndense) ok &= ls->DTP.ensure(tph_bytes(ipmax, (int)R), &grew);
    {
      const size_t n15 = std::max<size_t>(R, (size_t)std::max(ipmax, wmax));
      if (n15 > ls->sc15_n) {
        ok &= ls->sc15.ensure(n15);
        if (ok) {
          launch_fill(ls->sc15.sp(), 32768.f, (int)n15, h->st);
          launch_fill(ls->sc15.ip(), 1.f / 32768.f, (int)n15, h->st);
          ls->sc15_n = n15;
        }
      }
      ok &= ls->sc_x0r.ensure(R) && ls->sc_x0c.ensure((size_t)h->Fp);
      ok &= ls->sc_gr.ensure(R) && ls->sc_gc.ensure((size_t)wmax);
      if (ls->compactable || chunked) {
        ok &= ls->sc_cr.ensure(R + 64) && ls->sc_cx.ensure(R + 64);
        ok &= ls->OTS.ensure((ls->wg_overlap ? 2 : 1) * tph_bytes(D * Hp, (int)R), &grew);
      }
      for (int i = 0; i < ls->ndense; ++i) ok &= ls->sc_yr[i].ensure(R) && ls->sc_yc[i].ensure((size_t)ls->dWp[i]);
      bool g2 = false;
      ok &= ls->scws.ensure(tph_scale_ws_floats((int)R, std::max(ipmax, wmax)) * 4, &g2);
    }
  }
  int csw = std::max(D * N4, h->Cp);
  for (int i = 0; i < ls->ndense; ++i) csw = std::max(csw, ls->dWp[i]);
  ok &= ls->csws.ensure((size_t)std::max(32, tp_split2_parts((int)R)) * csw * 4, &grew);
  if (ls->wg_overlap) ok &= ls->csws2.ensure((size_t)std::max(32, tp_split2_parts((int)R)) * csw * 4, &grew);
  for (int i = 0; i < ls->ndense; ++i) {
    ok &= ls->Ybuf[i].ensure(R * ls->dWp[i] * 4, &grew);
    ok &= ls->dYbuf[i].ensure(R * ls->dWp[i] * 4, &grew);
  }
  for (int l = 0; l < ls->L; ++l) {
    ok &= ls->gates[l].ensure(R * D * N4 * 4, &grew);
    ok &= ls->outb[l].ensure(R * D * Hp * 4, &grew);
    ok &= ls->cbuf[l].ensure(R * D * Hp * 4, &grew);
  }
  if (!ok) return h->fail(NASR_ERR_HIP, "hipMalloc failed while sizing batch buffers");
  if (grew || Bp != h->Bp) drop_graphs(h);
  h->B = B; h->Bp = Bp; h->T = T; h->Lmax = Lmax; h->Tp = Tp; h->KS = KSa;
  ls->Tv = Tv; ls->lc_live = chunked; ls->lcg = lg;
  return NASR_OK;
}

int validate_batch(nasr_ctx* h, const int32_t* seq_len, const int32_t* labels, const int32_t* label_len, int B, int T,
                   int Lmax, int num_classes) {
  const bool las = !num_classes && h->family == Family::Las;
  const int C = num_classes ? num_classes : h->C;
  if (B < 1 || B > 64) return h->fail(NASR_ERR_ARG, "per-GPU batch must be in [1,64]");
  if (T < 1) return h->fail(NASR_ERR_ARG, "T must be >= 1");
  for (int b = 0; b < B; ++b) {
    if (seq_len[b] < 1 || seq_len[b] > T)
      return h->fail(NASR_ERR_ARG, "seq_len[" + std::to_string(b) + "] out of [1,T]");
    if (!labels) continue;
    if (las) {
      if (label_len[b] < 0 || label_len[b] > Lmax)
        return h->fail(NASR_ERR_ARG, "label_len[" + std::to_string(b) + "] out of [0,Lmax]");
      for (int i = 0; i < Lmax; ++i) {
        const int v = labels[(size_t)b * Lmax + i];
        if (v < 0 || v >= C) return h->fail(NASR_ERR_ARG, "label id out of [0, num_classes-1]");
      }
      continue;
    }
    const int L = label_len[b];
    if (L < 0 || L > Lmax) return h->fail(NASR_ERR_ARG, "label_len[" + std::to_string(b) + "] out of [0,Lmax]");
    int rep = 0;
    for (int i = 0; i < L; ++i) {
      const int v = labels[(size_t)b * Lmax + i];
      if (v < 0 || v >= C - 1)
        return h->fail(NASR_ERR_ARG, "label id out of [0, num_classes-2] (blank = num_classes-1 is not a label)");
      if (i > 0 && v == labels[(size_t)b * Lmax + i - 1]) ++rep;
    }
    if (L + rep > seq_len[b])
      return h->fail(NASR_ERR_INFEASIBLE, "Not enough time for target transition sequence (required: " +
                                              std::to_string(L + rep) + ", available: " + std::to_string(seq_len[b]) +
                                              ") in sequence " + std::to_string(b));
  }
  return NASR_OK;
}

int validate_chunk(nasr_ctx* h, const int32_t* n_frames, int S, int Tc) {
  if (Tc < 1) return h->fail(NASR_ERR_ARG, "a stream chunk needs Tc >= 1");
  for (int b = 0; b < S; ++b)
    if (n_frames[b] < 0 || n_frames[b] > Tc)
      return h->fail(NASR_ERR_ARG, "n_frames[" + std::to_string(b) + "] = " + std::to_string(n_frames[b]) + " out of [0,Tc = " +
                                       std::to_string(Tc) + "]");
  return NASR_OK;
}

static int validate_aug(nasr_ctx* h, const nasr_batch_aug* a, const int32_t* seq_len, int B, int ctx, int ncep, bool* masked) {
  *masked = false;
  if (a->n_time < 0 || a->n_time > NASR_AUG_MAX_MASKS || a->n_freq < 0 || a->n_freq > NASR_AUG_MAX_MASKS)
    return h->fail(NASR_ERR_ARG, "augmentation: n_time = " + std::to_string(a->n_time) + ", n_freq = " + std::to_string(a->n_freq) +
                                     ": each must be in [0," + std::to_string(NASR_AUG_MAX_MASKS) + "]");
  if (a->static_width < 1 || ncep % a->static_width)
    return h->fail(NASR_ERR_ARG, "augmentation: static_width " + std::to_string(a->static_width) + " does not divide the frame width " +
                                     std::to_string(ncep));
  if ((a->n_time && !a->time_mask) || (a->n_freq && !a->freq_mask)) return h->fail(NASR_ERR_ARG, "augmentation: null mask array");
  if (2 * (int64_t)ctx + 1 + ncep > 32768) return h->fail(NASR_ERR_ARG, "augmentation: 2*numcontext+1 + frame width > 32768");
  for (int b = 0; b < B; ++b) {
    for (int k = 0; k < a->n_time; ++k) {
      const int64_t t0 = a->time_mask[((size_t)b * a->n_time + k) * 2], tw = a->time_mask[((size_t)b * a->n_time + k) * 2 + 1];
      if (t0 < 0 || tw < 0 || t0 + tw > seq_len[b])
        return h->fail(NASR_ERR_ARG, "augmentation: time mask " + std::to_string(k) + " of utterance " + std::to_string(b) + " [" +
                                         std::to_string(t0) + ", " + std::to_string(t0 + tw) + ") is not inside its " +
                                         std::to_string(seq_len[b]) + " frames");
      *masked |= tw > 0;
    }
    for (int k = 0; k < a->n_freq; ++k) {
      const int64_t f0 = a->freq_mask[((size_t)b * a->n_freq + k) * 2], fw = a->freq_mask[((size_t)b * a->n_freq + k) * 2 + 1];
      if (f0 < 0 || fw < 0 || f0 + fw > a->static_width)
        return h->fail(NASR_ERR_ARG, "augmentation: frequency mask " + std::to_string(k) + " of utterance " + std::to_string(b) + " [" +
                                         std::to_string(f0) + ", " + std::to_string(f0 + fw) + ") is not inside the static block of " +
                                         std::to_string(a->static_width) + " columns");
      *masked |= fw > 0;
    }
  }
  return NASR_OK;
}

bool pinned_ensure(Pinned<void>& p, size_t* cap, size_t bytes) {
  if (bytes <= *cap) return true;
  *cap = 0;
  const size_t want = bytes + bytes / 8;
  if (hipHostMalloc(p.out(), want, hipHostMallocMapped) != hipSuccess) return false;
  *cap = want;
  return true;
}

BatchSlot* slot_acquire(nasr_ctx* h, bool for_stage) {
  std::lock_guard<std::mutex> lk(h->slot_mu);
  if (for_stage) {
    int ahead = 0;
    for (const BatchSlot& s : h->slots) ahead += s.state == SLOT_STAGED || s.state == SLOT_FILLING;
    if (ahead >= NSTAGE) return nullptr;
  }
  for (int k = 0; k < NSLOT; ++k) {
    BatchSlot& s = h->slots[(h->slot_rr + k) % NSLOT];
    if (s.state == SLOT_FREE) {
      h->slot_rr = (h->slot_rr + k + 1) % NSLOT;
      s.state = SLOT_FILLING;
      s.gen += 1;
      return &s;
    }
  }
  return nullptr;
}

void slot_set_state(nasr_ctx* h, BatchSlot* s, int st) {
  std::lock_guard<std::mutex> lk(h->slot_mu);
  s->state = st;
}

static bool stack_reshape(const nasr_ctx* h) {
  return h->lstm && h->lstm->cfg.merge == NASR_MERGE_STACK_RESHAPE && h->lstm->D == 2;
}

static int check_batch(nasr_ctx* h, const BatchSrc& b, bool* masked) {
  *masked = false;
  if ((b.feats != nullptr) + (b.centre != nullptr) + (b.producer != nullptr) + (b.stacked != nullptr) != 1 || !b.seq_len)
    return h->fail(NASR_ERR_ARG, "null input buffer");
  if (b.centre_form() && ((b.centre && !b.pad_value) || b.ctx < 0 || b.ncep < 1 || (2 * b.ctx + 1) * b.ncep != h->F))
    return h->fail(NASR_ERR_ARG, "context upload: feature_size must equal (2*numcontext+1)*numcep");
  if (b.labels && !b.label_len) return h->fail(NASR_ERR_ARG, "labels without label_len");
  if (b.chunk) return validate_chunk(h, b.seq_len, b.B, b.T);
  if (int rc = validate_batch(h, b.seq_len, b.labels, b.label_len, b.B, b.T, b.Lmax)) return rc;
  if (!b.aug) return NASR_OK;
  if (!b.centre_form()) return h->fail(NASR_ERR_ARG, "augmentation masks need a batch in the centre form");
  return validate_aug(h, b.aug, b.seq_len, b.B, b.ctx, b.ncep, masked);
}

static void meta_layout(nasr_ctx* h, BatchSlot* s, const BatchSrc& b, bool masked) {
  const LstmState* const ls = h->lstm.get();
  const int B = b.B, T = b.T;
  s->B = B; s->T = T; s->Lmax = b.labels ? b.Lmax : 0; s->ctx = b.ctx; s->ncep = b.ncep;
  s->Bp = rup(B, 16);
  s->Tp = h->family == Family::Las ? T : nasr_logit_frames(h, T);
  s->has_labels = b.labels != nullptr;
  s->centre = b.centre_form();
  s->masked = masked;
  s->aug_nm = masked ? std::max(b.aug->n_time, b.aug->n_freq) : 0;
  s->aug_sw = masked ? b.aug->static_width : 0;
  s->frames = 0;
  for (int i = 0; i < B; ++i) s->frames += b.seq_len[i];
  const size_t BLm = (size_t)B * std::max(s->Lmax, 1);
  s->o_seq = 0;
  s->o_lablen = s->o_seq + s->Bp;
  s->o_labels = s->o_lablen + s->Bp;
  s->o_cstart = s->o_labels + BLm;
  s->o_cpos = s->o_cstart + (b.labels ? (size_t)B * (h->C + 1) : 0);
  s->o_rowmap = s->o_cpos + BLm;
  s->cmp = ls && ls->compactable && b.labels && s->frames * 20 <= (int64_t)T * s->Bp * 17;
  s->Rv = s->cmp ? (int)s->frames : 0;
  const bool lc = ls && ls->lcC > 0 && !b.chunk;
  s->chunk = b.chunk;
  s->lcC = lc ? ls->lcC : 0; s->lcR = lc ? ls->lcR : 0;
  s->lcW = lc ? std::min(s->lcC + s->lcR, T) : 0;
  s->lcK = lc ? lc_last_window(T, s->lcC, s->lcW) + 1 : 0;
  if (lc) {
    int64_t rows = 0;
    for (int i = 0; i < B; ++i)
      for (int k = 0; k < s->lcK; ++k) rows += lc_window_rows(b.seq_len[i], k, s->lcC, s->lcW);
    s->cmp = true;
    s->Rv = (int)std::min<int64_t>(rows, (int64_t)1 << 22);
  }
  s->Rvp = s->cmp ? rup(s->Rv, 64) : 0;
  s->o_vrow = s->o_rowmap + (stack_reshape(h) ? (size_t)s->Tp * s->Bp : 0);
  s->o_vprev = s->o_vrow + s->Rvp;
  s->o_vnext = s->o_vprev + s->Rvp;
  s->o_wlen = s->o_vnext + s->Rvp;
  const size_t end = s->o_wlen + (size_t)s->lcK * s->Bp;
  s->o_aug = (end + 3) / 4 * 4;
  s->nmeta = masked ? s->o_aug + (size_t)B * s->aug_nm * 4 : end;
  s->nfeat = s->centre ? (size_t)B * T * b.ncep + B : (size_t)B * T * h->F;
}

static void write_meta(const nasr_ctx* h, BatchSlot* s, const BatchSrc& src) {
  const int B = src.B, T = src.T, Bp = s->Bp, Tp = s->Tp, C = h->C, Lmax = src.Lmax, Lm = std::max(s->Lmax, 1), nm = s->aug_nm;
  const int32_t *seq_len = src.seq_len, *labels = src.labels, *label_len = src.label_len;
  const nasr_batch_aug* aug = src.aug;
  int32_t* m = static_cast<int32_t*>(s->hmeta.get());
  memset(m, 0, s->nmeta * 4);
  memcpy(m + s->o_seq, seq_len, (size_t)B * 4);
  if (labels) {
    memcpy(m + s->o_lablen, label_len, (size_t)B * 4);
    if (Lmax > 0) memcpy(m + s->o_labels, labels, (size_t)B * Lmax * 4);
    std::vector<int32_t> fill((size_t)C);
    for (int b = 0; b < B; ++b) {
      int32_t* c0 = m + s->o_cstart + (size_t)b * (C + 1);
      const int32_t* lb = labels + (size_t)b * Lmax;
      for (int i = 0; i < label_len[b]; ++i) c0[lb[i] + 1] += 1;
      for (int c = 0; c < C; ++c) c0[c + 1] += c0[c];
      std::copy(c0, c0 + C, fill.begin());
      for (int i = 0; i < label_len[b]; ++i) m[s->o_cpos + (size_t)b * Lm + fill[lb[i]]++] = i;
    }
  }
  if (stack_reshape(h)) {
    int32_t* map = m + s->o_rowmap;
    for (size_t i = 0; i < (size_t)Tp * Bp; ++i) map[i] = -1;
    for (int tp = 0; tp < Tp; ++tp)
      for (int bq = 0; bq < B; ++bq) {
        const int64_t q = (int64_t)bq * 2 * T + tp;
        const int d = (int)(q / ((int64_t)B * T));
        const int64_t rem = q % ((int64_t)B * T);
        const int b = (int)(rem / T), t = (int)(rem % T);
        map[(size_t)tp * Bp + bq] = (t * Bp + b) * 2 + d;
      }
  }
  if (s->lcC) {
    const int Cc = s->lcC, W = s->lcW;
    int32_t *vr = m + s->o_vrow, *vp = m + s->o_vprev, *vn = m + s->o_vnext, *wl = m + s->o_wlen;
    int i = 0;
    for (int k = 0; k < s->lcK; ++k) {
      for (int b = 0; b < B; ++b) wl[(size_t)k * Bp + b] = lc_window_rows(seq_len[b], k, Cc, W);
      for (int tl = 0; tl < W && i < s->Rv; ++tl)
        for (int b = 0; b < B && i < s->Rv; ++b) {
          const int P = wl[(size_t)k * Bp + b];
          if (tl >= P) continue;
          const int r = (k * W + tl) * Bp + b;
          vr[i] = r;
          vp[i] = tl > 0 ? r - Bp : k > 0 ? ((k - 1) * W + Cc - 1) * Bp + b : -1;
          vn[i] = tl + 1 < P ? r + Bp : -1;
          ++i;
        }
    }
    for (; i < s->Rvp; ++i) vr[i] = vp[i] = vn[i] = -1;
  } else if (s->cmp) {
    int32_t *vr = m + s->o_vrow, *vp = m + s->o_vprev, *vn = m + s->o_vnext;
    int i = 0;
    for (int t = 0; t < T; ++t)
      for (int b = 0; b < B; ++b)
        if (seq_len[b] > t) {
          vr[i] = t * Bp + b;
          vp[i] = t > 0 ? (t - 1) * Bp + b : -1;
          vn[i] = t + 1 < seq_len[b] ? (t + 1) * Bp + b : -1;
          ++i;
        }
    for (; i < s->Rvp; ++i) vr[i] = vp[i] = vn[i] = -1;
  }
  if (s->masked)
    for (int b = 0; b < B; ++b)
      for (int k = 0; k < nm; ++k) {
        int32_t* q = m + s->o_aug + ((size_t)b * nm + k) * 4;
        if (k < aug->n_time) { q[0] = aug->time_mask[((size_t)b * aug->n_time + k) * 2]; q[1] = aug->time_mask[((size_t)b * aug->n_time + k) * 2 + 1]; }
        if (k < aug->n_freq) { q[2] = aug->freq_mask[((size_t)b * aug->n_freq + k) * 2]; q[3] = aug->freq_mask[((size_t)b * aug->n_freq + k) * 2 + 1]; }
      }
}

static int copy_feats(nasr_ctx* h, BatchSlot* s, const BatchSrc& b, hipStream_t cs, bool pinned_feats) {
  const size_t nc = s->nfeat - b.B;
  float* d = s->dfeats.as<float>();
  if (b.producer || b.stacked) {
    const int rc = b.stacked ? b.stacked->run(d, cs) : b.producer->run(d, d + nc, pinned_feats ? s->hfeats.get() : nullptr, cs);
    if (rc && hipEventRecord(s->ev_copy, cs) == hipSuccess) s->copy_valid = true;
    return rc;
  }
  if (pinned_feats) {
    float* p = static_cast<float*>(s->hfeats.get());
    memcpy(p, b.centre ? b.centre : b.feats, (b.centre ? nc : s->nfeat) * 4);
    if (b.centre) memcpy(p + nc, b.pad_value, (size_t)b.B * 4);
    HIPCHK(h, hipMemcpyAsync(d, p, s->nfeat * 4, hipMemcpyHostToDevice, cs));
  } else if (b.centre) {
    HIPCHK(h, hipMemcpyAsync(d, b.centre, nc * 4, hipMemcpyHostToDevice, cs));
    HIPCHK(h, hipMemcpyAsync(d + nc, b.pad_value, (size_t)b.B * 4, hipMemcpyHostToDevice, cs));
  } else {
    HIPCHK(h, hipMemcpyAsync(d, b.feats, s->nfeat * 4, hipMemcpyHostToDevice, cs));
  }
  return NASR_OK;
}

static int slot_fill(nasr_ctx* h, BatchSlot* s, const BatchSrc& b, hipStream_t cs, bool pinned_feats) {
  bool masked = false;
  if (int rc = check_batch(h, b, &masked)) return rc;
  HIPCHK(h, hipSetDevice(h->device));
  meta_layout(h, s, b, masked);
  bool grew = false;
  if (!s->dmeta.ensure(s->nmeta * 4, &grew) || !s->dfeats.ensure(s->nfeat * 4, &grew) ||
      !pinned_ensure(s->hmeta, &s->hmeta_cap, s->nmeta * 4) ||
      (pinned_feats && !b.stacked &&
       !pinned_ensure(s->hfeats, &s->hfeats_cap, b.producer ? b.producer->stage_bytes : s->nfeat * 4)))
    return h->fail(NASR_ERR_HIP, "allocation of a batch slot failed");
  if (s->copy_valid) HIPCHK(h, hipEventSynchronize(s->ev_copy));
  if (s->released_valid && cs != h->st) HIPCHK(h, hipStreamWaitEvent(cs, s->ev_released, 0));
  write_meta(h, s, b);
  if (int rc = copy_feats(h, s, b, cs, pinned_feats)) return rc;
  HIPCHK(h, hipMemcpyAsync(s->dmeta.p, s->hmeta, s->nmeta * 4, hipMemcpyHostToDevice, cs));
  HIPCHK(h, hipEventRecord(s->ev_copy, cs));
  s->copy_valid = true;
  return NASR_OK;
}

int slot_commit(nasr_ctx* h, BatchSlot* s) {
  LstmState* const ls = h->lstm.get();
  HIPCHK(h, hipSetDevice(h->device));
  if (ls && !s->chunk && (s->lcC != ls->lcC || s->lcR != (ls->lcC ? ls->lcR : 0)))
    return h->fail(NASR_ERR_STATE, "the batch was staged under another nasr_set_chunking than the handle has now: stage it again");
  int rc = ensure_shape(h, s->B, s->T, s->Lmax, s->lcC > 0);
  if (rc) return rc;
  const int B = s->B, T = s->T, Bp = h->Bp;
  {
    std::lock_guard<std::mutex> lk(h->slot_mu);
    if (h->cur && h->cur != s) {
      (void)hipEventRecord(h->cur->ev_released, h->st);
      h->cur->released_valid = true;
      h->cur->state = SLOT_FREE;
    }
    s->state = SLOT_RESIDENT;
    h->cur = s;
  }
  HIPCHK(h, hipStreamWaitEvent(h->st, s->ev_copy, 0));
  int32_t* md = s->meta_d();
  HIPCHK(h, hipMemcpyAsync(h->seqbuf.p, md + s->o_seq, (size_t)Bp * 4, hipMemcpyDeviceToDevice, h->st));
  h->seq_p = h->seqbuf.as<int32_t>(); h->lablen_p = md + s->o_lablen; h->labels_p = md + s->o_labels;
  h->cstart_p = md + s->o_cstart; h->cpos_p = md + s->o_cpos; h->rowmap_p = md + s->o_rowmap;
  const bool cmp = s->cmp && ls && (ls->compactable || s->lcC);
  h->wlen_p = md + s->o_wlen;
  h->cmp_rows = cmp ? s->Rv : 0;
  h->cmp_rows_p = cmp ? s->Rvp : 0;
  h->vrow_p = md + s->o_vrow; h->vprev_p = md + s->o_vprev; h->vnext_p = md + s->o_vnext;
  h->ev_used = 0;
  h->spans.clear();
  if (h->profiling) {
    (void)hipEventRecord(h->ev_total_a, h->st);
    h->window_open = true;
    h->total_valid = false;
  }
  h->h_seq.assign((size_t)Bp, 0);
  const int32_t* hm = static_cast<const int32_t*>(s->hmeta.get());
  for (int b = 0; b < B; ++b) h->h_seq[b] = hm[s->o_seq + b];
  h->frames = s->frames;
  {
    PhaseScope ps(h, PH_PACK);
    const bool lc = ls && ls->lc_live;
    float* x0 = (lc ? ls->lc_x0 : h->X0).as<float>();
    if (s->centre && s->masked)
      launch_expand_context_masked(s->dfeats.as<float>(), s->dfeats.as<float>() + (size_t)B * T * s->ncep, h->seq_p,
                                   md + s->o_aug, s->aug_nm, s->aug_sw, x0, B, Bp, T, s->ctx, s->ncep,
                                   h->Fp, h->st);
    else if (s->centre)
      launch_expand_context(s->dfeats.as<float>(), s->dfeats.as<float>() + (size_t)B * T * s->ncep, h->seq_p,
                            x0, B, Bp, T, s->ctx, s->ncep, h->Fp, h->st);
    else
      launch_pack_feats(s->dfeats.as<float>(), x0, B, Bp, T, h->F, h->Fp, h->st);
    if (lc) launch_lc_gather(x0, h->wlen_p, h->X0.as<float>(), ls->lcg, h->Fp, h->st);
    if (ls)
      pl_scales(h, h->X0.as<float>(), ls->Tv * Bp, h->Fp, h->Fp, &ls->sc_x0r, &ls->sc_x0c, h->st);
    if (h->cmp_rows)
      launch_gather_rows(ls->sc_cx.sp(), ls->sc_x0r.sp(), h->vrow_p, h->cmp_rows_p, 1.f, h->st),
      launch_gather_rows(ls->sc_cx.ip(), ls->sc_x0r.ip(), h->vrow_p, h->cmp_rows_p, 1.f, h->st);
    if (ls && s->has_labels && ls->npre == 0)
      launch_tph_split2(h->X0.as<float>(), nullptr, ls->X0TTP.as<unsigned char>(), h->cmp_rows ? h->cmp_rows : ls->Tv * Bp, h->Fp, h->Fp,
                        nullptr, 1.f, ls->sc_x0c.sp(), 1.f, nullptr, h->st, h->cmp_rows ? h->vrow_p : nullptr);
    HIPCHK(h, hipGetLastError());
  }
  h->resident = true;
  h->have_grads = false;
  h->have_fwd = false;
  h->have_decoded = false;
  return NASR_OK;
}

int upload(nasr_ctx* h, const BatchSrc& b) {
  BatchSlot* s = slot_acquire(h, false);
  if (!s) return h->fail(NASR_ERR_STATE, "every batch slot holds a staged batch: commit or discard one first");
  int rc = slot_fill(h, s, b, h->st, false);
  if (!rc) rc = slot_commit(h, s);
  if (rc && h->cur != s) slot_set_state(h, s, SLOT_FREE);
  return rc;
}

BatchSlot* slot_of_ticket(nasr_ctx* h, int ticket) {
  if (ticket < 0 || (ticket & 255) >= NSLOT) return nullptr;
  BatchSlot* s = &h->slots[ticket & 255];
  std::lock_guard<std::mutex> lk(h->slot_mu);
  return (s->state == SLOT_STAGED && (int)(s->gen & 0x7fffff) == (ticket >> 8)) ? s : nullptr;
}

int stage(nasr_ctx* h, const BatchSrc& b, int* ticket) {
  if (!ticket) return h->fail(NASR_ERR_ARG, "null ticket");
  *ticket = -1;
  BatchSlot* s = slot_acquire(h, true);
  if (!s) return h->fail(NASR_ERR_STATE, "no free batch slot: commit or discard a staged batch first");
  const int rc = slot_fill(h, s, b, h->cst, true);
  slot_set_state(h, s, rc ? SLOT_FREE : SLOT_STAGED);
  if (!rc) *ticket = (int)(s - h->slots) | (int)((s->gen & 0x7fffff) << 8);
  return rc;
}
}
```

### neuralasr_amd/csrc/nasr_ctx.h

```cpp
#pragma once
#include <hip/hip_runtime.h>

#include <dlfcn.h>
#include <sched.h>
#include <unistd.h>

#include <chrono>

#include <algorithm>
#include <cmath>
#include <cstdio>
#include <cstdlib>
#include <cstring>
#include <functional>
#include <memory>
#include <mutex>
#include <string>
#include <vector>

#include "../../include/nasr.h"
#include "kernels.h"

namespace nasr_impl {
using namespace nasr;

extern std::string g_create_error;
extern thread_local std::string t_err;
extern thread_local const void* t_err_handle;

inline int rup(int x, int m) { return (x + m - 1) / m * m; }

template <typename T, hipError_t (*Free)(T)>
class Owned {
 public:
  Owned() = default;
  Owned(const Owned&) = delete;
  Owned& operator=(const Owned&) = delete;
  Owned(Owned&& o) noexcept : v_(o.v_) { o.v_ = T{}; }
  Owned& operator=(Owned&& o) noexcept { std::swap(v_, o.v_); return *this; }
  ~Owned() { reset(); }
  void reset() {
    if (v_) (void)Free(v_);
    v_ = T{};
  }
  T* out() { reset(); return &v_; }
  T get() const { return v_; }
  operator T() const { return v_; }

 private:
  T v_{};
};
template <typename T> hipError_t free_device(T* p) { return hipFree(p); }
template <typename T> hipError_t free_pinned(T* p) { return hipHostFree(p); }
template <typename T> using DevPtr = Owned<T*, free_device<T>>;
template <typename T> using Pinned = Owned<T*, free_pinned<T>>;
using Event = Owned<hipEvent_t, hipEventDestroy>;

class Stream {
 public:
  Stream() = default;
  Stream(const Stream&) = delete;
  Stream& operator=(const Stream&) = delete;
  ~Stream() { reset(); }
  void reset() {
    if (s_ && own_) (void)hipStreamDestroy(s_);
    s_ = nullptr;
    own_ = false;
  }
  hipStream_t* out() { reset(); own_ = true; return &s_; }
  void borrow(hipStream_t s) { reset(); s_ = s; }
  operator hipStream_t() const { return s_; }

 private:
  hipStream_t s_ = nullptr;
  bool own_ = false;
};

struct DevBuf {
  void* p = nullptr;
  size_t cap = 0;
  DevBuf() = default;
  DevBuf(const DevBuf&) = delete;
  DevBuf& operator=(const DevBuf&) = delete;
  DevBuf(DevBuf&& o) noexcept : p(o.p), cap(o.cap) { o.p = nullptr; o.cap = 0; }
  DevBuf& operator=(DevBuf&& o) noexcept { std::swap(p, o.p); std::swap(cap, o.cap); return *this; }
  ~DevBuf() { release(); }
  bool ensure(size_t bytes, bool* grew) {
    if (bytes <= cap) return true;
    release();
    size_t want = bytes + bytes / 8;
    if (hipMalloc(&p, want) != hipSuccess) {
      if (hipMalloc(&p, bytes) != hipSuccess) return false;
      want = bytes;
    }
    cap = want;
    if (grew) *grew = true;
    return true;
  }
  void release() {
    if (p) (void)hipFree(p);
    p = nullptr;
    cap = 0;
  }
  template <typename T>
  T* as() const { return reinterpret_cast<T*>(p); }
};

struct TensorInfo {
  std::string name;
  int64_t offset, rows, cols;
};

enum Phase { PH_PACK = 0, PH_XPROJ, PH_RECF, PH_PROJCTC, PH_PROJB, PH_RECB, PH_WGRAD, PH_ADAM, PH_COUNT };

constexpr int GRAD_HEAD = 32;
constexpr int MAX_BUCKETS = 16;

constexpr int NSLOT = 4;
constexpr int NSTAGE = 2;
enum SlotState { SLOT_FREE = 0, SLOT_FILLING, SLOT_STAGED, SLOT_RESIDENT };
struct BatchSlot {
  DevBuf dfeats, dmeta;
  Pinned<void> hfeats, hmeta;
  size_t hfeats_cap = 0, hmeta_cap = 0;
  Event ev_copy, ev_released;
  bool copy_valid = false, released_valid = false;
  int state = SLOT_FREE;
  unsigned gen = 0;
  int B = 0, T = 0, Lmax = 0, Bp = 0, Tp = 0, ctx = 0, ncep = 0;
  bool has_labels = false, centre = false;
  int64_t frames = 0;
  size_t o_seq = 0, o_lablen = 0, o_labels = 0, o_cstart = 0, o_cpos = 0, o_rowmap = 0;
  size_t o_vrow = 0, o_vprev = 0, o_vnext = 0;
  int Rv = 0, Rvp = 0;
  bool cmp = false;
  int lcC = 0, lcR = 0, lcK = 0, lcW = 0;
  bool chunk = false;
  size_t o_wlen = 0;
  size_t nmeta = 0, nfeat = 0;
  size_t o_aug = 0;
  int aug_nm = 0, aug_sw = 0;
  bool masked = false;
  int32_t* meta_d() const { return dmeta.as<int32_t>(); }
};

enum class Family { Lstm, WaveNet, Las, Featurizer };

struct WnState;
struct WnStateDelete { void operator()(WnState* w) const; };
struct FzState;
struct FzStateDelete { void operator()(FzState* f) const; };
struct LasState;
struct LasStateDelete { void operator()(LasState* s) const; };
struct LstmState;
struct LstmStateDelete { void operator()(LstmState* s) const; };

struct FzStream;
struct FzStreamDelete { void operator()(FzStream* f) const; };

}

using namespace nasr;
using namespace nasr_impl;

struct nasr_ctx {

  Family family = Family::Lstm;
  std::unique_ptr<WnState, WnStateDelete> wn;
  std::unique_ptr<FzState, FzStateDelete> fz;
  std::unique_ptr<LasState, LasStateDelete> las;
  int device = 0;
  Stream st;
  void* comm = nullptr;
  void* comm2 = nullptr;
  Stream comm_st2;
  int comm_rank = 0, comm_n = 1;
  Stream comm_st;
  Event ev_comm;
  DevPtr<float> comm_scratch;

  int F, Fp, C, Cp;
  int64_t np_int = 0;
  std::vector<TensorInfo> tensors;
  int64_t np_tf = 0;
  std::vector<int32_t> tf2int;

  DevPtr<float> P, M, V;
  float* G = nullptr;
  DevPtr<float> Gbase;
  std::vector<std::pair<int64_t, int64_t>> buckets;
  std::vector<Event> ev_bucket;
  DevPtr<AdamDev> adam_dev;
  float lr;
  float beta1 = 0.f, beta2 = 0.f, epsilon = 0.f;
  float max_grad_norm = 0.f;
  DevPtr<ClipDev> clip_dev;
  DevPtr<double> clip_part;
  struct StepRes { Pinned<void> host; size_t cap = 0; Pinned<uint32_t> stamp; uint32_t seq = 0; bool valid = false; int B = 0, Bp = 0, Tp = 0; bool logits = false, greedy = false;
                   Event ev_lg; };
  StepRes res[2];
  int res_cur = 0;
  struct StepEnd { Pinned<float> host; uint32_t* stamp = nullptr; uint32_t seq = 0; bool valid = false; int64_t token = 0; };
  static constexpr int NEND = 4;
  StepEnd endw[NEND];
  int end_cur = 0;
  int64_t step_token = 0;
  uint32_t stamp_seq = 0;

  bool resident = false, have_grads = false, have_fwd = false;
  int B = 0, Bp = 0, T = 0, Lmax = 0, Tp = 0, KS = 1;
  int64_t frames = 0;
  std::vector<int32_t> h_seq;
  BatchSlot slots[NSLOT];
  BatchSlot* cur = nullptr;
  Stream cst;
  Stream d2h;
  Event ev_snap;
  DevBuf logits_snap;
  std::mutex slot_mu;
  int slot_rr = 0;
  int32_t *seq_p = nullptr, *lablen_p = nullptr, *labels_p = nullptr, *cstart_p = nullptr, *cpos_p = nullptr,
          *rowmap_p = nullptr;
  int cmp_rows = 0, cmp_rows_p = 0;
  int32_t *vrow_p = nullptr, *vprev_p = nullptr, *vnext_p = nullptr;
  int32_t* wlen_p = nullptr;

  DevBuf ctcprobs, ctckexp;
  DevBuf seqbuf, X0, logits, logz, alpha, beta, aoff, boff, logp, nll, loss, slabs, amax, ids, lens;
  DevBuf al_logz, al_bp, al_path, al_score, al_logits, al_meta;

  bool graph_mode = true;
  bool step_decode = false, step_logits = false, have_decoded = false;
  bool step_greedy = false;

  bool profiling = false;
  std::vector<Event> ev_pool;
  size_t ev_used = 0;
  struct Span { int ph; hipEvent_t a, b; };
  std::vector<Span> spans;
  Event ev_total_a, ev_total_b;
  bool window_open = false, total_valid = false;
  int n_fwd_launch = 0, n_bwd_launch = 0;
  nasr_phase_times last_times;

  std::unique_ptr<LstmState, LstmStateDelete> lstm;

  int fail(int code, const std::string& m) {
    t_err = m;
    t_err_handle = this;
    return code;
  }
};

namespace nasr_impl {

#define HIPCHK(h, expr)                                                                                   \
  do {                                                                                                    \
    hipError_t e_ = (expr);                                                                               \
    if (e_ != hipSuccess)                                                                                 \
      return (h)->fail(NASR_ERR_HIP, std::string(#expr) + ": " + hipGetErrorString(e_));                  \
  } while (0)
#define MODEL_CALL(h)                                                                                     \
  do {                                                                                                    \
    if ((h) && (h)->family == Family::Featurizer)                                                         \
      return (h)->fail(NASR_ERR_STATE, std::string(__func__) + ": a featurizer handle has no model");     \
  } while (0)
#define LSTM_CALL(h, reason)                                                                              \
  do {                                                                                                    \
    if ((h) && !(h)->lstm)                                                                                \
      return (h)->fail(NASR_ERR_STATE, std::string(__func__) + ": a WaveNet or LAS handle " reason);      \
  } while (0)
#define FAMILY_CALL(h, state, text)                                                                       \
  do {                                                                                                    \
    if (!(h)) return NASR_ERR_ARG;                                                                        \
    if (!(h)->state) return (h)->fail(NASR_ERR_STATE, std::string(__func__) + ": " text);                 \
  } while (0)
#define LAS_CALL(h) FAMILY_CALL(h, las, "not a LAS handle")
#define WAVENET_CALL(h) FAMILY_CALL(h, wn, "not a WaveNet handle")
int handle_open(const char* fn, Family family, int device_id, void* stream, nasr_ctx** out, hipDeviceProp_t* prop);
int create_fail(nasr_ctx* h, int code, const std::string& m);
bool alloc_param_buffers(nasr_ctx* h);
int handle_finish(nasr_ctx* h);

int repack(nasr_ctx* h);
int scatter_to_device(nasr_ctx* h, const float* tf_flat, float* dev);
int gather_from_device(nasr_ctx* h, const float* dev, float* tf_flat);
void launch_stamp(unsigned* dst, unsigned value, float* f0_dst, const float* f0_src, hipStream_t st);
void launch_publish_results(const float* loss, const float* fault, const int* lens, int Bp, const int* ids, int n_ids, void* host,
                            unsigned* stamp, unsigned value, hipStream_t st);
bool wait_stamp(const uint32_t* w, uint32_t want, double timeout_s);
int sync_checked(nasr_ctx* h);
hipEvent_t next_event(nasr_ctx* h);
struct PhaseScope {
  nasr_ctx* h;
  int ph;
  hipEvent_t a = nullptr;
  PhaseScope(nasr_ctx* h_, int ph_) : h(h_), ph(ph_) {
    if (h->profiling) {
      a = next_event(h);
      (void)hipEventRecord(a, h->st);
    }
  }
  ~PhaseScope() {
    if (h->profiling) {
      hipEvent_t b = next_event(h);
      (void)hipEventRecord(b, h->st);
      h->spans.push_back({ph, a, b});
    }
  }
};

int rec_check(nasr_ctx* h);
void rec_rearm(nasr_ctx* h);

struct LstmSwitches {
  bool compact, persist, rec_f32, wgrad_overlap, bucket_defer;
  int64_t rearm_after;
};
int lstm_create(const nasr_model_cfg* cfg, int device_id, void* stream, const LstmSwitches& sw, nasr_ctx** out);
void drop_graphs(nasr_ctx* h);
void lstm_sync_side(nasr_ctx* h);
int lstm_logit_frames(const nasr_ctx* h, int T);

int ensure_shape(nasr_ctx* h, int B, int T, int Lmax, bool chunked = false);
int ensure_ctc_buffers(nasr_ctx* h, int B, int Bp, int T, int Tp, int Lmax, bool* grew);
int validate_batch(nasr_ctx* h, const int32_t* seq_len, const int32_t* labels, const int32_t* label_len, int B, int T, int Lmax,
                   int num_classes = 0);
int validate_chunk(nasr_ctx* h, const int32_t* n_frames, int S, int Tc);
bool pinned_ensure(Pinned<void>& p, size_t* cap, size_t bytes);
void slot_set_state(nasr_ctx* h, BatchSlot* s, int st);
int slot_commit(nasr_ctx* h, BatchSlot* s);
struct CentreProducer {
  size_t stage_bytes = 0;
  std::function<int(float* dcentre, float* dpad, void* pinned, hipStream_t cs)> run;
};
struct StackedProducer {
  std::function<int(float* dfeats, hipStream_t cs)> run;
};
struct BatchSrc {
  const float *feats = nullptr, *centre = nullptr, *pad_value = nullptr;
  const CentreProducer* producer = nullptr;
  const StackedProducer* stacked = nullptr;
  int ctx = 0, ncep = 0;
  const int32_t *seq_len = nullptr, *labels = nullptr, *label_len = nullptr;
  int B = 0, T = 0, Lmax = 0;
  const nasr_batch_aug* aug = nullptr;
  bool chunk = false;
  bool centre_form() const { return centre || producer; }
};
inline BatchSrc stacked_batch(const float* feats, const int32_t* seq_len, const int32_t* labels, const int32_t* label_len, int B,
                              int T, int Lmax) {
  BatchSrc b;
  b.feats = feats; b.seq_len = seq_len; b.labels = labels; b.label_len = label_len; b.B = B; b.T = T; b.Lmax = Lmax;
  return b;
}
inline BatchSrc centre_batch(const float* centre, const float* pad_value, int ctx, int ncep, const int32_t* seq_len,
                             const int32_t* labels, const int32_t* label_len, int B, int T, int Lmax,
                             const nasr_batch_aug* aug) {
  BatchSrc b = stacked_batch(nullptr, seq_len, labels, label_len, B, T, Lmax);
  b.centre = centre; b.pad_value = pad_value; b.ctx = ctx; b.ncep = ncep; b.aug = aug;
  return b;
}
inline BatchSrc produced_batch(const CentreProducer* producer, int ctx, int ncep, const int32_t* seq_len, const int32_t* labels,
                               const int32_t* label_len, int B, int T, int Lmax, const nasr_batch_aug* aug) {
  BatchSrc b = centre_batch(nullptr, nullptr, ctx, ncep, seq_len, labels, label_len, B, T, Lmax, aug);
  b.producer = producer;
  return b;
}
int upload(nasr_ctx* h, const BatchSrc& b);
BatchSlot* slot_of_ticket(nasr_ctx* h, int ticket);
int stage(nasr_ctx* h, const BatchSrc& b, int* ticket);

int gemm_f32(nasr_ctx* h, GemmDesc g);
int gemm_dense(nasr_ctx* h, const float* A, const float* B, float* C, int M, int N, int K, int lda, int ldb, int ldc, bool a_col,
               bool b_col, const float* bias = nullptr, int a_shift = 0, int a_rows = -1);
inline float* fp(const DevBuf& b, size_t off = 0) { return b.as<float>() + off; }
int forward(nasr_ctx* h);
int loss_pass(nasr_ctx* h, bool training);
CtcDims ctc_dims(nasr_ctx* h);
int ctc_forward(nasr_ctx* h);
int backward(nasr_ctx* h);
int fetch_logits(nasr_ctx* h, float* logits_out, int rows = -1);

int wn_ensure_shape(nasr_ctx* h, int B, int T, int Lmax);
int wn_forward(nasr_ctx* h, bool training);
int wn_backward(nasr_ctx* h);

int las_ensure_shape(nasr_ctx* h, int B, int T, int Lmax);
int las_forward(nasr_ctx* h, bool sample);
int las_backward(nasr_ctx* h);

int lstm_ensure_shape(nasr_ctx* h, int B, int T, int Lmax, bool chunked);
int lstm_forward(nasr_ctx* h, bool chunk = false);
int lstm_backward(nasr_ctx* h);

}
```

### neuralasr_amd/csrc/nasr_lstm.h

```cpp
#pragma once
#include "nasr_ctx.h"

#include <map>

namespace nasr_impl {

enum class RecKind { Step = 0, Persist = 1, Wide = 2 };

struct GraphKey {
  int T, l, bwd;
  bool operator<(const GraphKey& o) const {
    if (T != o.T) return T < o.T;
    if (l != o.l) return l < o.l;
    return bwd < o.bwd;
  }
};

struct StreamState {
  int S = 0;
  int R = 0;
  std::unique_ptr<FzStream, FzStreamDelete> audio;
  DevBuf state;
  DevBuf cimg;
  DevBuf hold[2];
  int cur = 0;
  DevBuf fresh;
  std::vector<int32_t> held;
  std::vector<uint8_t> done;
  LaSlots sl{};
  std::vector<int64_t> frames;
};

struct SV {
  DevBuf s, inv;
  bool ensure(size_t n) { bool g = false; return s.ensure(n * 4, &g) && inv.ensure(n * 4, &g); }
  float* sp() const { return s.as<float>(); }
  float* ip() const { return inv.as<float>(); }
};

struct LstmState {
  nasr_model_cfg cfg;

  int H, Hp, N4, D, L, Pin, Pinp;
  std::vector<int> Ip;
  std::vector<int64_t> off_wx, off_bias;
  std::vector<int64_t> off_u;
  int64_t off_w = 0, off_b = 0;

  int npre = 0, ndense = 0;
  bool has_post = false;
  int F0 = 0;
  std::vector<int> dWid, dWp, dIn, dIp;
  std::vector<int64_t> off_dw, off_db;
  std::vector<size_t> off_dftp, off_dbtp;
  DevPtr<unsigned char> DfTP, DbTP;
  std::vector<DevBuf> Ybuf, dYbuf;
  DevBuf DTP;
  uint32_t drop_seed = 4567u, drop_counter = 0;

  DevPtr<unsigned char> WfTP;
  DevPtr<unsigned char> WbTP;
  std::vector<size_t> off_wftp, off_wbtp;
  SV sc15;
  size_t sc15_n = 0;
  SV sc_x0r, sc_x0c;
  std::vector<SV> sc_yr, sc_yc;
  SV sc_gr, sc_gc;
  std::vector<SV> sc_wr, sc_wc;
  std::vector<SV> sc_dr, sc_dc;
  DevBuf scws;
  int gttp_layer = -1;
  int dgmax_layer = -1;
  DevBuf dgmax;
  DevBuf XTP, X0TTP, GTP, GTTP;
  std::vector<DevBuf> OTT;
  std::vector<char> ott_valid;
  DevBuf csws;

  RecKind rec_kind = RecKind::Step;
  RecKind rec_use = RecKind::Step;
  bool rec_wanted = false;
  bool rec_inflight = false;
  bool rec_refused = false;
  int64_t rearm_after = 0, rearm_wait = 0, clean_steps = 0;
  int persist_aborts = 0, persist_rearms = 0;
  uint64_t repack_seq = 0;
  uint64_t step_img_seq = ~0ull;
  DevPtr<float> Uf, Ub;
  Pinned<unsigned> perr;
  DevPtr<float> Ucs, Ucinv;
  bool rec_f16 = false;
  DevPtr<float> Upf, Upb;
  size_t imf = 0, imb = 0;
  DevPtr<float> xchf;
  DevPtr<float> xchb;
  DevPtr<PersistCtl> pctl;
  DevPtr<unsigned char> Uw;
  DevPtr<unsigned char> Uwb;
  DevPtr<float> Urs, Urinv;
  DevPtr<float> wsrow;
  DevPtr<void> whx;
  DevPtr<float> wpart;
  DevPtr<void> wpx;
  DevPtr<WideCtl> wctl;
  std::map<GraphKey, hipGraphExec_t> graphs;

  std::unique_ptr<StreamState> stream;

  std::vector<int> bucket_of_layer;
  bool bucket_defer = true;

  int lcC = 0, lcR = 0;
  int Tv = 0;
  bool lc_live = false;
  LcGeom lcg{};
  DevBuf lc_x0, lc_top, lc_dtop;
  DevBuf lc_cimg, lc_dcc;

  bool compactable = false;
  SV sc_cr, sc_cx;
  DevBuf OTS;

  bool wg_overlap = false;
  bool bwd_lean = false;
  Stream wst;
  Event ev_dx;
  std::vector<Event> ev_wg;
  std::vector<char> wg_pending;
  DevBuf GTTP2, csws2, slabs2;
  SV sc_gc2;

  std::vector<DevBuf> gates, outb, cbuf;
  DevBuf dout, hstate, partial, dcstate, dgbuf;
};

inline size_t pl_rb_bytes(int nkb) { return (size_t)nkb * 2 * 1024; }
void pl_scales(nasr_ctx* h, const float* src, int rows, int K, int ld, SV* row, SV* col, hipStream_t st);
void pl_split(const float* src, unsigned char* tpN, unsigned char* tpT, int rows, int K, int ld, const float* rs,
              const float* cs, float* colpart, hipStream_t st);
void pl_gemm(GemmTPHDesc g, const float* a_inv, const float* b_inv, hipStream_t st, int64_t ainv_bstride = 0,
             int64_t binv_bstride = 0);
struct ActScale { const float *rs, *rinv, *cs, *cinv; };
inline ActScale act_x0(const LstmState* ls) { return {ls->sc_x0r.sp(), ls->sc_x0r.ip(), ls->sc_x0c.sp(), ls->sc_x0c.ip()}; }
inline ActScale act_y(const LstmState* ls, int i) { return {ls->sc_yr[i].sp(), ls->sc_yr[i].ip(), ls->sc_yc[i].sp(), ls->sc_yc[i].ip()}; }
inline ActScale act_out(const LstmState* ls) { return {ls->sc15.sp(), ls->sc15.ip(), ls->sc15.sp(), ls->sc15.ip()}; }
inline ActScale lstm_in_scale(const LstmState* ls, int l) {
  if (l > 0) return act_out(ls);
  return ls->npre ? act_y(ls, ls->npre - 1) : act_x0(ls);
}
inline ActScale dense_in_scale(const LstmState* ls, int i) {
  if (i == 0 && ls->npre > 0) return act_x0(ls);
  if (i < ls->npre) return act_y(ls, i - 1);
  return act_out(ls);
}

int build_layout(nasr_ctx* h);

int rec_setup(nasr_ctx* h, bool allowed, bool f32);
void rec_start(nasr_ctx* h);
int rec_launch(nasr_ctx* h, int l, bool bwd, hipStream_t st, int* launches);
std::vector<TphScaleJob> rec_scale_jobs(const nasr_ctx* h);
void rec_images(nasr_ctx* h);
void ensure_step_images(nasr_ctx* h);

inline float* dout_of(LstmState* ls, int) { return ls->dout.as<float>(); }
inline float* dg_of(LstmState* ls, int) { return ls->dgbuf.as<float>(); }
inline bool wg_alt(const LstmState* ls, int l) { return ls->wg_overlap && (l & 1); }
inline unsigned char* gttp_of(LstmState* ls, int l) { return (wg_alt(ls, l) ? ls->GTTP2 : ls->GTTP).as<unsigned char>(); }
inline float* csws_of(LstmState* ls, int l) { return (wg_alt(ls, l) ? ls->csws2 : ls->csws).as<float>(); }
inline SV& gc_of(LstmState* ls, int l) { return wg_alt(ls, l) ? ls->sc_gc2 : ls->sc_gc; }
inline const float* lstm_input(nasr_ctx* h, int l) {
  LstmState* ls = h->lstm.get();
  if (l > 0) return ls->outb[l - 1].as<float>();
  return ls->npre ? ls->Ybuf[ls->npre - 1].as<float>() : h->X0.as<float>();
}

int lc_run_steps(nasr_ctx* h, int l, bool bwd, hipStream_t st, int* launches);

}
```

### neuralasr_amd/csrc/nasr_pass.hip

```cpp
#include "nasr_lstm.h"

using namespace nasr;
using namespace nasr_impl;

namespace nasr_impl {

static StepWindow step_window(nasr_ctx* h, int l, int T, size_t row, const int* seq, const float* c0) {
  LstmState* const ls = h->lstm.get();
  const size_t sU = (size_t)l * ls->D * ls->Hp * ls->N4, DH = (size_t)ls->D * ls->Hp, DN = (size_t)ls->D * ls->N4;
  StepWindow w{};
  w.dm = {T, h->B, h->Bp, ls->H, ls->Hp, ls->D};
  w.Uf = ls->Uf + sU; w.Ub = ls->Ub + sU;
  w.hstate = ls->hstate.as<float>(); w.partial = ls->partial.as<float>(); w.dcstate = ls->dcstate.as<float>();
  w.gates = ls->gates[l].as<float>() + row * DN; w.cbuf = ls->cbuf[l].as<float>() + row * DH; w.out = ls->outb[l].as<float>() + row * DH;
  w.dg = dg_of(ls, l) + row * DN; w.dout = dout_of(ls, l) + row * DH;
  w.seq_len = seq; w.forget_bias = ls->cfg.forget_bias; w.c0 = c0;
  return w;
}

static int run_steps(nasr_ctx* h, int l, bool bwd, hipStream_t st, int* launches) {
  LstmState* const ls = h->lstm.get();
  if (ls->rec_use != RecKind::Step) return rec_launch(h, l, bwd, st, launches);
  *launches += h->T;
  const StepWindow w = step_window(h, l, h->T, 0, h->seq_p, nullptr);
  auto body = [&]() { bwd ? lstm_steps_bwd(w, 0, h->T, st) : lstm_steps_fwd(w, 0, h->T, st); };
  if (!h->graph_mode) {
    body();
    HIPCHK(h, hipGetLastError());
    return NASR_OK;
  }
  const GraphKey key{h->T, l, bwd ? 1 : 0};
  auto it = ls->graphs.find(key);
  if (it == ls->graphs.end()) {
    if (ls->graphs.size() > 256) drop_graphs(h);
    hipGraph_t g = nullptr;
    HIPCHK(h, hipStreamBeginCapture(st, hipStreamCaptureModeThreadLocal));
    body();
    HIPCHK(h, hipStreamEndCapture(st, &g));
    hipGraphExec_t ex = nullptr;
    HIPCHK(h, hipGraphInstantiate(&ex, g, nullptr, nullptr, 0));
    (void)hipGraphDestroy(g);
    it = ls->graphs.emplace(key, ex).first;
  }
  HIPCHK(h, hipGraphLaunch(it->second, st));
  return NASR_OK;
}

int lc_run_steps(nasr_ctx* h, int l, bool bwd, hipStream_t st, int* launches) {
  LstmState* const ls = h->lstm.get();
  const LcGeom& g = ls->lcg;
  const int Bp = h->Bp, Hp = ls->Hp, D = ls->D, W = g.W, DH = D * Hp;
  const int Ce = std::min(g.C, W);
  float *cimg = ls->lc_cimg.as<float>(), *dcc = ls->lc_dcc.as<float>();
  float *cb = ls->cbuf[l].as<float>(), *ob = ls->outb[l].as<float>();
  for (int i = 0; i < g.K; ++i) {
    const int k = bwd ? g.K - 1 - i : i;
    const int* wl = h->wlen_p + (size_t)k * Bp;
    const StepWindow w = step_window(h, l, W, (size_t)k * W * Bp, wl, cimg);
    if (!bwd) {
      launch_lc_load_carry(ob, cb, h->wlen_p, k, g, w.hstate, cimg, Hp, D, st);
      lstm_steps_fwd(w, 0, W, st);
      continue;
    }
    lstm_steps_bwd(w, Ce, W, st);
    if (k + 1 < g.K) launch_lc_carry_dc(lstm_steps_dcin(w, Ce - 1), dcc, Bp * Hp, st);
    lstm_steps_bwd(w, 1, Ce, st);
    launch_lc_load_carry(ob, cb, h->wlen_p, k, g, w.hstate, cimg, Hp, D, st);
    lstm_steps_bwd(w, 0, 1, st);
    const StepLeft left = lstm_steps_left(w, 0);
    if (k > 0)
      launch_lc_carry_out(left.partial, lstm_bwd_partials(Hp), left.dc, wl, dout_of(ls, l) + ((size_t)(k - 1) * W + g.C - 1) * Bp * DH,
                          dcc, Bp, Hp, DH, st);
  }
  *launches += g.K * W;
  HIPCHK(h, hipGetLastError());
  return NASR_OK;
}

float* ensure_slabs(nasr_ctx* h, int split, int M, int N) {
  if (split <= 1) return nullptr;
  bool grew = false;
  if (!h->slabs.ensure((size_t)split * M * N * 4, &grew)) return nullptr;
  return h->slabs.as<float>();
}

int gemm_f32(nasr_ctx* h, GemmDesc g) {
  g.slabs = ensure_slabs(h, g.split_k, g.M, g.N);
  if (g.split_k > 1 && !g.slabs) return h->fail(NASR_ERR_HIP, "slab workspace allocation failed");
  launch_gemm(g, h->st);
  HIPCHK(h, hipGetLastError());
  return NASR_OK;
}

int gemm_dense(nasr_ctx* h, const float* A, const float* B, float* C, int M, int N, int K, int lda, int ldb, int ldc, bool a_col,
               bool b_col, const float* bias, int a_shift, int a_rows) {
  GemmDesc g{};
  g.A = A; g.B = B; g.C = C;
  g.M = M; g.N = N; g.K = K; g.lda = lda; g.ldb = ldb; g.ldc = ldc;
  g.a_col = a_col; g.b_col = b_col;
  g.a_shift = a_shift;
  g.a_rows = a_rows >= 0 ? a_rows : (a_col ? K : M);
  g.bias = bias;
  g.split_k = bias ? 1 : gemm_pick_split(M, N, K);
  return gemm_f32(h, g);
}

void dg_scales(nasr_ctx* h, int l, int R, bool rows, hipStream_t st) {
  LstmState* const ls = h->lstm.get();
  const int DN = ls->D * ls->N4;
  if (ls->dgmax_layer == l) {
    const float* rp = ls->dgmax.as<float>();
    launch_tph_scales_from_parts(rp, ls->D * 32, R, rows ? ls->sc_gr.sp() : nullptr, rows ? ls->sc_gr.ip() : nullptr,
                                 rp + (size_t)ls->D * 32 * R, 8 / ls->D, DN, gc_of(ls, l).sp(), gc_of(ls, l).ip(), st);
  } else {
    pl_scales(h, dg_of(ls, l), R, DN, DN, rows ? &ls->sc_gr : nullptr, &gc_of(ls, l), st);
  }
}

void gemm_xproj(nasr_ctx* h, int l, int R, hipStream_t st) {
  LstmState* const ls = h->lstm.get();
  const int D = ls->D, N4 = ls->N4, Ip = ls->Ip[l];
  const int rows = h->cmp_rows ? h->cmp_rows : R;
  const int* vm = h->cmp_rows ? h->vrow_p : nullptr;
  ActScale as = lstm_in_scale(ls, l);
  if (vm && l == 0) { as.rs = ls->sc_cx.sp(); as.rinv = ls->sc_cx.ip(); }
  const bool both = l > 0 && h->cur && h->cur->has_labels;
  launch_tph_split2(lstm_input(h, l), ls->XTP.as<unsigned char>(), both ? ls->OTT[l - 1].as<unsigned char>() : nullptr, rows, Ip, Ip,
                    as.rs, 1.f, both ? as.cs : nullptr, 1.f, nullptr, st, vm);
  if (l > 0) ls->ott_valid[l - 1] = both;
  GemmTPHDesc g{};
  g.A = ls->XTP.as<unsigned char>(); g.B = ls->WfTP + ls->off_wftp[l]; g.C = ls->gates[l].as<float>();
  g.M = rows; g.N = D * N4; g.K = Ip; g.nkbA = (Ip + 15) / 16; g.nkbB = g.nkbA; g.ldc = D * N4;
  g.bias = h->P + ls->off_bias[l]; g.split_k = 1;
  g.c_map = vm;
  pl_gemm(g, as.rinv, ls->sc_wc[l].ip(), st);
}

void gemm_dx(nasr_ctx* h, int l, int R, hipStream_t st) {
  LstmState* const ls = h->lstm.get();
  const int D = ls->D, N4 = ls->N4;
  const int rows = h->cmp_rows ? h->cmp_rows : R;
  const int* vm = h->cmp_rows ? h->vrow_p : nullptr;
  const float* A = dg_of(ls, l);
  float* C = l > 0 ? dout_of(ls, l - 1) : ls->dYbuf[ls->npre - 1].as<float>();
  dg_scales(h, l, R, true, st);
  const float *rs = ls->sc_gr.sp(), *rinv = ls->sc_gr.ip();
  if (vm) {
    launch_gather_rows(ls->sc_cr.sp(), ls->sc_gr.sp(), vm, h->cmp_rows_p, 1.f, st);
    launch_gather_rows(ls->sc_cr.ip(), ls->sc_gr.ip(), vm, h->cmp_rows_p, 1.f, st);
    rs = ls->sc_cr.sp(); rinv = ls->sc_cr.ip();
  }
  launch_tph_split2(A, ls->GTP.as<unsigned char>(), gttp_of(ls, l), rows, D * N4, D * N4, rs, 1.f, gc_of(ls, l).sp(), 1.f,
                    csws_of(ls, l), st, vm);
  ls->gttp_layer = l;
  GemmTPHDesc g{};
  g.A = ls->GTP.as<unsigned char>(); g.B = ls->WbTP + ls->off_wbtp[l]; g.C = C;
  g.M = rows; g.N = ls->Ip[l]; g.K = D * N4; g.nkbA = (D * N4 + 15) / 16; g.nkbB = g.nkbA; g.ldc = ls->Ip[l];
  g.split_k = gemm_tph_pick_split(g.M, g.N, g.K);
  g.slabs = ensure_slabs(h, g.split_k, g.M, g.N);
  if (g.split_k > 1 && !g.slabs) g.split_k = 1;
  g.c_map = vm;
  pl_gemm(g, rinv, ls->sc_wr[l].ip(), st);
}

int dense_forward(nasr_ctx* h, int i, const float* X) {
  LstmState* const ls = h->lstm.get();
  const int R = h->T * h->Bp, Ip = ls->dIp[i], Wp = ls->dWp[i];
  const ActScale as = dense_in_scale(ls, i);
  pl_split(X, ls->XTP.as<unsigned char>(), nullptr, R, Ip, Ip, as.rs, nullptr, nullptr, h->st);
  GemmTPHDesc g{};
  g.A = ls->XTP.as<unsigned char>(); g.B = ls->DfTP + ls->off_dftp[i]; g.C = ls->Ybuf[i].as<float>();
  g.M = R; g.N = Wp; g.K = Ip; g.nkbA = (Ip + 15) / 16; g.nkbB = g.nkbA; g.ldc = Wp;
  g.bias = h->P + ls->off_db[i]; g.split_k = 1;
  pl_gemm(g, as.rinv, ls->sc_dc[i].ip(), h->st);
  launch_dense_act(ls->Ybuf[i].as<float>(), R, h->Bp, h->B, ls->dWid[i], Wp, ls->cfg.relu_clip, ls->cfg.dropout[i],
                   ls->drop_seed, ls->drop_counter, i, h->st);
  pl_scales(h, ls->Ybuf[i].as<float>(), R, Wp, Wp, &ls->sc_yr[i], &ls->sc_yc[i], h->st);
  HIPCHK(h, hipGetLastError());
  return NASR_OK;
}

int dense_backward(nasr_ctx* h, int i, const float* X, float* dX) {
  LstmState* const ls = h->lstm.get();
  const int R = h->T * h->Bp, Ip = ls->dIp[i], Wp = ls->dWp[i];
  const int nkb = (R + 15) / 16;
  float* dZ = ls->dYbuf[i].as<float>();
  launch_dense_act_bwd(dZ, ls->Ybuf[i].as<float>(), (int64_t)R * Wp, ls->cfg.relu_clip, ls->cfg.dropout[i], h->st);
  const ActScale as = dense_in_scale(ls, i);
  pl_scales(h, dZ, R, Wp, Wp, dX ? &ls->sc_gr : nullptr, &ls->sc_gc, h->st);
  pl_split(dZ, dX ? ls->GTP.as<unsigned char>() : nullptr, ls->GTTP.as<unsigned char>(), R, Wp, Wp, ls->sc_gr.sp(),
           ls->sc_gc.sp(), ls->csws.as<float>(), h->st);
  pl_split(X, nullptr, ls->DTP.as<unsigned char>(), R, Ip, Ip, nullptr, as.cs, nullptr, h->st);
  {
    GemmTPHDesc g{};
    g.A = ls->DTP.as<unsigned char>(); g.B = ls->GTTP.as<unsigned char>(); g.C = h->G + ls->off_dw[i];
    g.M = Ip; g.N = Wp; g.K = R; g.nkbA = nkb; g.nkbB = nkb; g.ldc = Wp;
    g.split_k = gemm_tph_pick_split(g.M, g.N, g.K);
    g.slabs = ensure_slabs(h, g.split_k, g.M, g.N);
    if (g.split_k > 1 && !g.slabs) return h->fail(NASR_ERR_HIP, "slab workspace allocation failed");
    pl_gemm(g, as.cinv, ls->sc_gc.ip(), h->st);
  }
  launch_colsum_parts(ls->csws.as<float>(), tp_split2_parts(R), Wp, h->G + ls->off_db[i], h->st);
  if (dX) {
    GemmTPHDesc g{};
    g.A = ls->GTP.as<unsigned char>(); g.B = ls->DbTP + ls->off_dbtp[i]; g.C = dX;
    g.M = R; g.N = Ip; g.K = Wp; g.nkbA = (Wp + 15) / 16; g.nkbB = g.nkbA; g.ldc = Ip;
    g.split_k = gemm_tph_pick_split(g.M, g.N, g.K);
    g.slabs = ensure_slabs(h, g.split_k, g.M, g.N);
    if (g.split_k > 1 && !g.slabs) g.split_k = 1;
    pl_gemm(g, ls->sc_gr.ip(), ls->sc_dr[i].ip(), h->st);
  }
  HIPCHK(h, hipGetLastError());
  return NASR_OK;
}

static int run_chunk_steps(nasr_ctx* h, int l, hipStream_t st) {
  LstmState* const ls = h->lstm.get();
  StreamState& ss = *ls->stream;
  float* state = ss.state.as<float>() + (size_t)l * ss.S * 2 * ls->H;
  const StepWindow w = step_window(h, l, h->T, 0, h->seq_p, ss.cimg.as<float>());
  launch_stream_load_state(state, w.hstate, ss.cimg.as<float>(), ss.S, ls->H, h->Bp, ls->Hp, st, ls->D);
  lstm_steps_fwd(w, 0, h->T, st);
  launch_stream_save_state(w.out, w.cbuf, ss.sl, state, ss.S, ls->H, h->Bp, ls->D * ls->Hp, st);
  h->n_fwd_launch += h->T;
  HIPCHK(h, hipGetLastError());
  return NASR_OK;
}

int forward(nasr_ctx* h) {
  if (!h->resident) return h->fail(NASR_ERR_STATE, "no resident batch: call nasr_upload_batch first");
  switch (h->family) {
    case Family::WaveNet: return wn_forward(h, false);
    case Family::Las: return h->fail(NASR_ERR_STATE, "a LAS handle has no CTC logits: use nasr_las_forward");
    default: return lstm_forward(h);
  }
}

int lstm_forward(nasr_ctx* h, bool chunk) {
  LstmState* const ls = h->lstm.get();
  const int Bp = h->Bp, T = h->T, D = ls->D, Hp = ls->Hp;
  const int R = T * Bp, Rv = ls->Tv * Bp;
  const bool lc = ls->lc_live;
  if (lc) ensure_step_images(h);
  h->n_fwd_launch = 0;
  std::fill(ls->ott_valid.begin(), ls->ott_valid.end(), 0);
  if (!chunk) HIPCHK(h, hipMemsetAsync(h->Gbase, 0, GRAD_HEAD * 4, h->st));
  if (ls->rec_use == RecKind::Persist && !chunk && !lc) {
    HIPCHK(h, hipMemsetAsync(ls->pctl + 1, 0, (size_t)ls->L * sizeof(PersistCtl), h->st));
    HIPCHK(h, hipMemsetAsync(ls->xchf, 0, (size_t)ls->L * persist_hx_bytes(ls->Hp), h->st));
  }
  for (int i = 0; i < ls->npre; ++i) {
    PhaseScope ps(h, PH_XPROJ);
    int rc = dense_forward(h, i, i == 0 ? h->X0.as<float>() : ls->Ybuf[i - 1].as<float>());
    if (rc) return rc;
  }
  for (int l = 0; l < ls->L; ++l) {
    {
      PhaseScope ps(h, PH_XPROJ);
      gemm_xproj(h, l, Rv, h->st);
      HIPCHK(h, hipGetLastError());
    }
    PhaseScope ps(h, PH_RECF);
    int rc = chunk ? run_chunk_steps(h, l, h->st)
             : lc  ? lc_run_steps(h, l, false, h->st, &h->n_fwd_launch)
                   : run_steps(h, l, false, h->st, &h->n_fwd_launch);
    if (rc) return rc;
  }
  if (lc) {
    PhaseScope ps(h, PH_RECF);
    launch_lc_emit(ls->outb[ls->L - 1].as<float>(), h->seq_p, ls->lc_top.as<float>(), ls->lcg, D * Hp, h->st);
  }
  if (ls->has_post) {
    PhaseScope ps(h, PH_XPROJ);
    int rc = dense_forward(h, ls->npre, ls->outb[ls->L - 1].as<float>());
    if (rc) return rc;
  }
  if (ls->ndense && !chunk) ls->drop_counter += 1;
  {
    PhaseScope ps(h, PH_PROJCTC);
    const bool sr = ls->cfg.merge == NASR_MERGE_STACK_RESHAPE && D == 2;
    GemmDesc g{};
    g.A = ls->has_post ? ls->Ybuf[ls->npre].as<float>() : lc ? ls->lc_top.as<float>() : ls->outb[ls->L - 1].as<float>();
    g.B = h->P + ls->off_w;
    g.C = h->logits.as<float>();
    g.M = h->Tp * Bp; g.N = h->Cp; g.K = ls->Pinp;
    g.lda = sr ? Hp : ls->Pinp; g.ldb = h->Cp; g.ldc = h->Cp;
    g.a_map = sr ? h->rowmap_p : nullptr;
    g.a_rows = sr ? 2 * R : R;
    g.bias = h->P + ls->off_b;
    g.split_k = gemm_pick_split(g.M, g.N, g.K);
    if (int rc = gemm_f32(h, g)) return rc;
  }
  h->have_fwd = !chunk;
  return NASR_OK;
}

CtcDims ctc_dims(nasr_ctx* h) {
  CtcDims d;
  d.Tp = h->Tp; d.B = h->B; d.Bp = h->Bp; d.C = h->C; d.Cp = h->Cp; d.Lmax = std::max(h->Lmax, 1);
  d.KS = h->KS; d.Tws = h->T + 8;
  d.lprobs = h->ctcprobs.as<float>(); d.goff = h->ctckexp.as<double>();
  return d;
}

int ctc_forward(nasr_ctx* h) {
  PhaseScope ps(h, PH_PROJCTC);
  const CtcDims d = ctc_dims(h);
  launch_ctc_logz(d, h->logits.as<float>(), h->seq_p, h->logz.as<float>(), h->st);
  launch_ctc_alpha_beta(d, h->logits.as<float>(), h->logz.as<float>(), h->labels_p, h->lablen_p,
                        h->seq_p, h->alpha.as<float>(), h->beta.as<float>(), h->aoff.as<double>(),
                        h->boff.as<double>(), h->nll.as<float>(), h->logp.as<double>(), h->st);
  launch_mean(h->nll.as<float>(), h->B, h->loss.as<float>(), h->st);
  if (h->step_decode) {
    if (h->step_greedy)
      launch_greedy(d, h->logits.as<float>(), h->seq_p, h->amax.as<int>(), h->ids.as<int>(), h->lens.as<int>(), h->st);
    h->have_decoded = h->step_greedy;
    h->res_cur ^= 1;
    nasr_ctx::StepRes& r = h->res[h->res_cur];
    const size_t ids_bytes = 8 + (size_t)h->Bp * 4 + (size_t)h->B * h->Tp * 4;
    const size_t lg_off = (ids_bytes + 255) / 256 * 256, lg_bytes = h->step_logits ? (size_t)h->Tp * h->Bp * h->Cp * 4 : 0;
    const size_t bytes = lg_off + lg_bytes;
    if (!pinned_ensure(r.host, &r.cap, bytes)) return h->fail(NASR_ERR_HIP, "hipHostMalloc of the step results failed");
    char* hp = static_cast<char*>(r.host.get());
    if (lg_bytes) {
      bool grew = false;
      if (!h->logits_snap.ensure(lg_bytes, &grew)) return h->fail(NASR_ERR_HIP, "hipMalloc of the logits snapshot failed");
      if (!r.ev_lg) HIPCHK(h, hipEventCreateWithFlags(r.ev_lg.out(), hipEventDisableTiming));
      nasr_ctx::StepRes& prev = h->res[h->res_cur ^ 1];
      if (prev.logits && prev.ev_lg) HIPCHK(h, hipStreamWaitEvent(h->st, prev.ev_lg, 0));
      HIPCHK(h, hipMemcpyAsync(h->logits_snap.p, h->logits.p, lg_bytes, hipMemcpyDeviceToDevice, h->st));
      HIPCHK(h, hipEventRecord(h->ev_snap, h->st));
      HIPCHK(h, hipStreamWaitEvent(h->d2h, h->ev_snap, 0));
      HIPCHK(h, hipMemcpyAsync(hp + lg_off, h->logits_snap.p, lg_bytes, hipMemcpyDeviceToHost, h->d2h));
      HIPCHK(h, hipEventRecord(r.ev_lg, h->d2h));
    }
    r.logits = lg_bytes != 0;
    r.seq = ++h->stamp_seq;
    launch_publish_results(h->loss.as<float>(), h->Gbase, h->lens.as<int>(), h->step_greedy ? h->Bp : 0, h->ids.as<int>(),
                           h->step_greedy ? h->B * h->Tp : 0, r.host, r.stamp, r.seq, h->st);
    r.greedy = h->step_greedy;
    r.valid = true; r.B = h->B; r.Bp = h->Bp; r.Tp = h->Tp;
  }
  HIPCHK(h, hipGetLastError());
  return NASR_OK;
}

int loss_pass(nasr_ctx* h, bool training) {
  int rc;
  switch (h->family) {
    case Family::Las: return las_forward(h, true);
    case Family::WaveNet: rc = wn_forward(h, training); break;
    default: rc = forward(h); break;
  }
  return rc ? rc : ctc_forward(h);
}

int weight_grads(nasr_ctx* h, int l, hipStream_t ws, bool side) {
  LstmState* const ls = h->lstm.get();
  const int Bp = h->Bp, D = ls->D, Hp = ls->Hp, N4 = ls->N4;
  const int R = ls->Tv * Bp;
  float* dG = dg_of(ls, l);
  unsigned char* GT = gttp_of(ls, l);
  float* cs_part = csws_of(ls, l);
  SV& gc = gc_of(ls, l);
  DevBuf& slab_buf = side ? ls->slabs2 : h->slabs;
  auto slabs_for = [&](int split, int M, int N) -> float* {
    if (split <= 1) return nullptr;
    bool grew = false;
    return slab_buf.ensure((size_t)split * M * N * 4, &grew) ? slab_buf.as<float>() : nullptr;
  };
  const int rows = h->cmp_rows ? h->cmp_rows : R;
  const int* vm = h->cmp_rows ? h->vrow_p : nullptr;
  const int nkb = (rows + 15) / 16;
  if (ls->gttp_layer != l) {
    dg_scales(h, l, R, false, ws);
    launch_tph_split2(dG, nullptr, GT, rows, D * N4, D * N4, nullptr, 1.f, gc.sp(), 1.f, cs_part, ws, vm);
  }
  ls->gttp_layer = -1;
  const ActScale ao = act_out(ls), ai = lstm_in_scale(ls, l);
  for (int m = std::max(l - 1, 0); m <= (vm ? l - 1 : l); ++m)
    if (!ls->ott_valid[m]) {
      launch_tph_split2(ls->outb[m].as<float>(), nullptr, ls->OTT[m].as<unsigned char>(), rows, D * Hp, D * Hp, nullptr, 1.f, ao.cs, 1.f,
                        nullptr, ws, vm);
      ls->ott_valid[m] = 1;
    }
  unsigned char* OS = ls->OTS.as<unsigned char>() + (wg_alt(ls, l) ? tph_bytes(D * Hp, R) : 0);
  if (vm)
    launch_tph_split2(ls->outb[l].as<float>(), nullptr, OS, rows, D * Hp, D * Hp, nullptr, 1.f, ao.cs, 1.f, nullptr, ws, h->vprev_p,
                      D == 2 ? h->vnext_p : nullptr, Hp);
  if (l == 0 && ls->npre)
    pl_split(lstm_input(h, l), nullptr, ls->X0TTP.as<unsigned char>(), R, ls->Ip[0], ls->Ip[0], nullptr, ai.cs, nullptr, ws);
  {
    GemmTPHDesc g{};
    g.A = l == 0 ? ls->X0TTP.as<unsigned char>() : ls->OTT[l - 1].as<unsigned char>();
    g.B = GT; g.C = h->G + ls->off_wx[l];
    g.M = ls->Ip[l]; g.N = D * N4; g.K = rows; g.nkbA = nkb; g.nkbB = nkb; g.ldc = D * N4;
    g.side = side;
    g.split_k = gemm_tph_pick_split(g.M, g.N, g.K);
    g.slabs = slabs_for(g.split_k, g.M, g.N);
    if (g.split_k > 1 && !g.slabs) return h->fail(NASR_ERR_HIP, "slab workspace allocation failed");
    pl_gemm(g, ai.cinv, gc.ip(), ws);
  }
  launch_colsum_parts(cs_part, tp_split2_parts(rows), D * N4, h->G + ls->off_bias[l], ws);
  {
    GemmTPHDesc g{};
    g.A = vm ? OS : ls->OTT[l].as<unsigned char>(); g.B = GT; g.C = h->G + ls->off_u[(size_t)l * D];
    g.M = Hp; g.N = N4; g.K = rows; g.nkbA = nkb; g.nkbB = nkb; g.ldc = N4;
    g.a_kshift = vm ? 0 : -Bp;
    g.nbatch = D;
    g.a_bstride = (size_t)(Hp / 32) * pl_rb_bytes(nkb); g.b_bstride = (size_t)(N4 / 32) * pl_rb_bytes(nkb);
    g.c_bstride = (int64_t)Hp * N4;
    g.a_kshift1 = vm ? 0 : Bp;
    g.side = side;
    g.split_k = gemm_tph_pick_split(g.M, g.N, g.K, D);
    g.slabs = slabs_for(g.split_k * D, g.M, g.N);
    if (g.split_k > 1 && !g.slabs) return h->fail(NASR_ERR_HIP, "slab workspace allocation failed");
    pl_gemm(g, ao.cinv, gc.ip(), ws, Hp, N4);
  }
  HIPCHK(h, hipGetLastError());
  return NASR_OK;
}

int wg_join(nasr_ctx* h, int l) {
  LstmState* const ls = h->lstm.get();
  if (l >= 0 && l < ls->L && ls->wg_pending[l]) {
    HIPCHK(h, hipStreamWaitEvent(h->st, ls->ev_wg[l], 0));
    ls->wg_pending[l] = 0;
  }
  return NASR_OK;
}

int backward(nasr_ctx* h) {
  switch (h->family) {
    case Family::WaveNet: return wn_backward(h);
    case Family::Las: return las_backward(h);
    default: return lstm_backward(h);
  }
}

int lstm_backward(nasr_ctx* h) {
  LstmState* const ls = h->lstm.get();
  const int Bp = h->Bp, T = h->T, D = ls->D, Hp = ls->Hp;
  const int R = T * Bp, Rp = h->Tp * Bp, Rv = ls->Tv * Bp;
  const bool sr = ls->cfg.merge == NASR_MERGE_STACK_RESHAPE && D == 2;
  const bool lc = ls->lc_live;
  const RecKind use = lc ? RecKind::Step : ls->rec_use;
  if (use == RecKind::Persist) {
    HIPCHK(h, hipMemsetAsync(ls->pctl + 1 + ls->L, 0, (size_t)ls->L * sizeof(PersistCtl), h->st));
    HIPCHK(h, hipMemsetAsync(ls->xchb, 0, (size_t)ls->L * persist_px_bytes(), h->st));
  }
  {
    PhaseScope ps(h, PH_PROJCTC);
    const CtcDims d = ctc_dims(h);
    launch_ctc_grad(d, h->logits.as<float>(), h->logz.as<float>(), h->lablen_p, h->seq_p,
                    h->cstart_p, h->cpos_p, h->alpha.as<float>(), h->beta.as<float>(),
                    h->aoff.as<double>(), h->boff.as<double>(), h->logp.as<double>(), 1.f / (float)h->B, h->st);
    HIPCHK(h, hipGetLastError());
  }
  {
    PhaseScope ps(h, PH_PROJB);
    GemmDesc g{};
    g.A = ls->has_post ? ls->Ybuf[ls->npre].as<float>() : lc ? ls->lc_top.as<float>() : ls->outb[ls->L - 1].as<float>();
    g.B = h->logits.as<float>();
    g.C = h->G + ls->off_w;
    g.M = ls->Pinp; g.N = h->Cp; g.K = Rp;
    g.lda = sr ? Hp : ls->Pinp; g.ldb = h->Cp; g.ldc = h->Cp;
    g.a_col = true; g.a_map = sr ? h->rowmap_p : nullptr; g.a_rows = sr ? 2 * R : R;
    g.split_k = gemm_pick_split(g.M, g.N, g.K);
    if (int rc = gemm_f32(h, g)) return rc;
    launch_colsum(h->logits.as<float>(), Rp, h->Cp, h->Cp, h->G + ls->off_b, ls->csws.as<float>(), h->st);
    GemmDesc x{};
    x.A = h->logits.as<float>();
    x.B = h->P + ls->off_w;
    x.C = ls->has_post ? ls->dYbuf[ls->npre].as<float>() : lc ? ls->lc_dtop.as<float>() : dout_of(ls, ls->L - 1);
    x.M = Rp; x.N = ls->Pinp; x.K = h->Cp;
    x.lda = h->Cp; x.ldb = h->Cp; x.ldc = sr ? Hp : ls->Pinp;
    x.b_col = true; x.a_rows = Rp; x.c_map = sr ? h->rowmap_p : nullptr; x.split_k = 1;
    if (int rc = gemm_f32(h, x)) return rc;
    if (lc) launch_lc_scatter(ls->lc_dtop.as<float>(), h->seq_p, h->wlen_p, dout_of(ls, ls->L - 1), ls->lcg, D * Hp, h->st);
  }
  if (ls->has_post) {
    PhaseScope ps(h, PH_WGRAD);
    int rc = dense_backward(h, ls->npre, ls->outb[ls->L - 1].as<float>(), dout_of(ls, ls->L - 1));
    if (rc) return rc;
  }
  h->n_bwd_launch = 0;
  ls->dgmax_layer = -1;
  for (int l = ls->L - 1; l >= 0; --l) {
    const bool defer = use != RecKind::Step && ls->bucket_defer;
    {
      PhaseScope ps(h, PH_RECB);
      int rc = lc ? lc_run_steps(h, l, true, h->st, &h->n_bwd_launch) : run_steps(h, l, true, h->st, &h->n_bwd_launch);
      if (rc) return rc;
    }
    if (defer && l + 1 < ls->L && ls->bucket_of_layer[l + 1] >= 0) {
      if (int rc = wg_join(h, l + 1)) return rc;
      HIPCHK(h, hipEventRecord(h->ev_bucket[ls->bucket_of_layer[l + 1]], h->st));
    }
    PhaseScope ps(h, PH_WGRAD);
    if (int rc = wg_join(h, l + 2)) return rc;
    if (l > 0 || ls->npre > 0) gemm_dx(h, l, Rv, h->st);
    const bool side = ls->wg_overlap && use == RecKind::Persist && l > 0 && ls->gttp_layer == l;
    if (side) {
      HIPCHK(h, hipEventRecord(ls->ev_dx, h->st));
      HIPCHK(h, hipStreamWaitEvent(ls->wst, ls->ev_dx, 0));
      int rc = weight_grads(h, l, ls->wst, true);
      if (rc) return rc;
      HIPCHK(h, hipEventRecord(ls->ev_wg[l], ls->wst));
      ls->wg_pending[l] = 1;
    } else {
      int rc = weight_grads(h, l, h->st, false);
      if (rc) return rc;
    }
    if (ls->bucket_of_layer[l] >= 0 && !(defer && l > 0)) {
      if (int rc = wg_join(h, l)) return rc;
      HIPCHK(h, hipEventRecord(h->ev_bucket[ls->bucket_of_layer[l]], h->st));
    }
  }
  for (int l = 0; l < ls->L; ++l)
    if (int rc = wg_join(h, l)) return rc;
  for (int i = ls->npre - 1; i >= 0; --i) {
    PhaseScope ps(h, PH_WGRAD);
    int rc = dense_backward(h, i, i == 0 ? h->X0.as<float>() : ls->Ybuf[i - 1].as<float>(),
                            i > 0 ? ls->dYbuf[i - 1].as<float>() : nullptr);
    if (rc) return rc;
  }
  HIPCHK(h, hipEventRecord(h->ev_bucket.back(), h->st));
  h->have_grads = true;
  return NASR_OK;
}

int fetch_logits(nasr_ctx* h, float* logits_out, int rows) {
  const int Tr = rows >= 0 ? std::min(rows, h->Tp) : h->Tp;
  const size_t n = (size_t)Tr * h->Bp * h->Cp;
  std::vector<float> host(n);
  HIPCHK(h, hipMemcpyAsync(host.data(), h->logits.p, n * 4, hipMemcpyDeviceToHost, h->st));
  if (int rc = sync_checked(h)) return rc;
  for (int t = 0; t < Tr; ++t)
    for (int b = 0; b < h->B; ++b)
      memcpy(logits_out + ((size_t)t * h->B + b) * h->C, host.data() + ((size_t)t * h->Bp + b) * h->Cp,
             (size_t)h->C * 4);
  return NASR_OK;
}

}
```

### neuralasr_amd/csrc/nasr_rec.hip

```cpp
#include "nasr_lstm.h"

namespace nasr_impl {

static bool persist_census(nasr_ctx* h) {
  LstmState* const ls = h->lstm.get();
  const int Bp = 16, T = 2;
  const size_t R = (size_t)T * Bp;
  DevBuf g, c, o, dg, sq;
  bool grew = false;
  bool ok = g.ensure(R * ls->D * ls->N4 * 4, &grew) && c.ensure(R * ls->D * ls->Hp * 4, &grew) &&
            o.ensure(R * ls->D * ls->Hp * 4, &grew) && dg.ensure(R * ls->D * ls->N4 * 4, &grew) && sq.ensure(Bp * 4, &grew);
  if (ok) {
    (void)hipMemsetAsync(g.p, 0, R * ls->D * ls->N4 * 4, h->st);
    (void)hipMemsetAsync(o.p, 0, R * ls->D * ls->Hp * 4, h->st);
    std::vector<int32_t> two((size_t)Bp, T);
    (void)hipMemcpyAsync(sq.p, two.data(), Bp * 4, hipMemcpyHostToDevice, h->st);
    const LstmDims dm{T, Bp, Bp, ls->H, ls->Hp, ls->D};
    launch_lstm_persist_fwd(dm, ls->Upf, ls->rec_f16 ? ls->Ucinv : nullptr, g.as<float>(), c.as<float>(), o.as<float>(),
                            sq.as<int>(), ls->xchf, ls->pctl, ls->perr, nullptr, 1.f, h->st);
    launch_lstm_persist_bwd(dm, ls->Upb, g.as<float>(), dg.as<float>(), c.as<float>(), o.as<float>(), sq.as<int>(),
                            ls->xchb, ls->pctl, ls->perr, nullptr, h->st, false, nullptr, nullptr, ls->bwd_lean);
    ok = hipStreamSynchronize(h->st) == hipSuccess && hipGetLastError() == hipSuccess && *ls->perr == 0;
  }
  *ls->perr = 0;
  return ok;
}

int rec_setup(nasr_ctx* h, bool allowed, bool f32) {
  LstmState* const ls = h->lstm.get();
  ls->rec_kind = !allowed ? RecKind::Step : persist_supported(ls->Hp) ? RecKind::Persist
                : wide_supported(ls->Hp, 16) ? RecKind::Wide : RecKind::Step;
  if (ls->rec_kind == RecKind::Step) return NASR_OK;
  ls->rec_f16 = ls->rec_kind == RecKind::Persist && !f32;
  const size_t nk = (size_t)ls->L * ls->D;
  bool g2 = false;
  if (hipHostMalloc(ls->perr.out(), 64, hipHostMallocMapped) != hipSuccess || hipMalloc(ls->Ucs.out(), nk * ls->N4 * 4) != hipSuccess ||
      hipMalloc(ls->Ucinv.out(), nk * ls->N4 * 4) != hipSuccess || !ls->scws.ensure(nk * tph_scale_ws_floats(ls->Hp, ls->N4) * 4, &g2))
    return h->fail(NASR_ERR_HIP, "allocation of the recurrent-weight scales failed");
  *ls->perr = 0;
  if (ls->rec_f16) {
    (void)hipMemsetAsync(ls->Ucs, 0, nk * ls->N4 * 4, h->st);
    (void)hipMemsetAsync(ls->Ucinv, 0, nk * ls->N4 * 4, h->st);
  }
  if (ls->rec_kind == RecKind::Persist) {
    ls->imf = persist_image_floats(ls->Hp, false);
    ls->imb = persist_image_floats(ls->Hp, true);
    if (persist_prepare() != hipSuccess || hipMalloc(ls->Upf.out(), nk * ls->imf * 4) != hipSuccess ||
        hipMalloc(ls->Upb.out(), nk * ls->imb * 4) != hipSuccess ||
        hipMalloc(ls->xchf.out(), (size_t)ls->L * persist_hx_bytes(ls->Hp)) != hipSuccess ||
        hipMalloc(ls->xchb.out(), (size_t)ls->L * persist_px_bytes()) != hipSuccess ||
        hipMalloc(ls->pctl.out(), (size_t)(1 + 2 * ls->L) * sizeof(PersistCtl)) != hipSuccess)
      return h->fail(NASR_ERR_HIP, "allocation of the persistent-recurrence buffers failed");
    (void)hipMemsetAsync(ls->Upf, 0, nk * ls->imf * 4, h->st);
    (void)hipMemsetAsync(ls->Upb, 0, nk * ls->imb * 4, h->st);
    return NASR_OK;
  }
  if (wide_prepare() != hipSuccess || hipMalloc(ls->Uw.out(), nk * wide_image_bytes(ls->Hp)) != hipSuccess ||
      hipMalloc(ls->whx.out(), wide_hx_bytes(64)) != hipSuccess || hipMalloc(ls->wpart.out(), wide_part_bytes(64)) != hipSuccess ||
      hipMalloc(ls->wctl.out(), sizeof(WideCtl)) != hipSuccess || hipMalloc(ls->Uwb.out(), nk * wide_image_bytes(ls->Hp)) != hipSuccess ||
      hipMalloc(ls->wpx.out(), wide_px_bytes(64)) != hipSuccess || hipMalloc(ls->Urs.out(), nk * ls->Hp * 4) != hipSuccess ||
      hipMalloc(ls->Urinv.out(), nk * ls->Hp * 4) != hipSuccess || hipMalloc(ls->wsrow.out(), 2 * 64 * 4) != hipSuccess)
    return h->fail(NASR_ERR_HIP, "allocation of the wide persistent-recurrence buffers failed");
  (void)hipMemsetAsync(ls->whx, 0, wide_hx_bytes(64), h->st);
  (void)hipMemsetAsync(ls->wpx, 0, wide_px_bytes(64), h->st);
  return NASR_OK;
}

void rec_start(nasr_ctx* h) {
  LstmState* const ls = h->lstm.get();
  if (ls->rec_kind == RecKind::Persist && !persist_census(h)) ls->rec_kind = RecKind::Step;
  ls->rec_use = ls->rec_kind;
  ls->rec_wanted = ls->rec_kind != RecKind::Step;
}

int rec_launch(nasr_ctx* h, int l, bool bwd, hipStream_t st, int* launches) {
  LstmState* const ls = h->lstm.get();
  const LstmDims dm{h->T, h->B, h->Bp, ls->H, ls->Hp, ls->D};
  if (ls->rec_use == RecKind::Persist) {
    const size_t k = (size_t)l * ls->D;
    if (!bwd) {
      launch_lstm_persist_fwd(dm, ls->Upf + k * ls->imf, ls->rec_f16 ? ls->Ucinv + k * ls->N4 : nullptr,
                              ls->gates[l].as<float>(), ls->cbuf[l].as<float>(),
                              ls->outb[l].as<float>(), h->seq_p, ls->xchf + (size_t)l * (persist_hx_bytes(ls->Hp) / 4),
                              ls->pctl + 1 + l, ls->perr, h->Gbase, ls->cfg.forget_bias, st, true);
    } else {
      launch_lstm_persist_bwd(dm, ls->Upb + k * ls->imb, ls->gates[l].as<float>(), dg_of(ls, l), ls->cbuf[l].as<float>(),
                              dout_of(ls, l), h->seq_p, ls->xchb + (size_t)l * (persist_px_bytes() / 4), ls->pctl + 1 + ls->L + l,
                              ls->perr, h->Gbase, st, true, ls->dgmax.as<float>(),
                              ls->dgmax.as<float>() + (size_t)ls->D * 32 * h->T * h->Bp, ls->bwd_lean);
      ls->dgmax_layer = l;
    }
    *launches += 1;
  } else {
    if (bwd) launch_wide_row_scales(dm, dout_of(ls, l), h->seq_p, ls->wsrow, st);
    for (int d = 0; d < ls->D; ++d) {
      const size_t k = (size_t)l * ls->D + d;
      if (!bwd)
        launch_lstm_wide_fwd(dm, d, ls->Uw + k * wide_image_bytes(ls->Hp), ls->Ucinv + k * ls->N4, ls->gates[l].as<float>(),
                             ls->cbuf[l].as<float>(), ls->outb[l].as<float>(), h->seq_p, ls->whx, ls->wpart, ls->wctl, ls->perr,
                             h->Gbase, ls->cfg.forget_bias, st);
      else
        launch_lstm_wide_bwd(dm, d, ls->Uwb + k * wide_image_bytes(ls->Hp), ls->Urinv + k * ls->Hp, ls->wsrow,
                             ls->gates[l].as<float>(), dg_of(ls, l), ls->cbuf[l].as<float>(), dout_of(ls, l), h->seq_p, ls->wpart,
                             ls->wpx, ls->wctl, ls->perr, h->Gbase, st);
    }
    *launches += ls->D;
  }
  ls->rec_inflight = true;
  HIPCHK(h, hipGetLastError());
  return NASR_OK;
}

int rec_check(nasr_ctx* h) {
  LstmState* const ls = h->lstm.get();
  if (!ls || !ls->rec_inflight) return NASR_OK;
  ls->rec_inflight = false;
  const unsigned code = *reinterpret_cast<volatile unsigned*>(ls->perr.get());
  if (!code) return NASR_OK;
  *reinterpret_cast<volatile unsigned*>(ls->perr.get()) = 0;
  ls->rec_use = RecKind::Step;
  ls->rec_refused = true;
  ls->persist_aborts += 1;
  ls->clean_steps = 0;
  ls->rearm_wait = ls->persist_aborts <= 1 ? ls->rearm_after : std::min<int64_t>(ls->rearm_wait * 2, (int64_t)1 << 20);
  (void)repack(h);
  return h->fail(NASR_ERR_HIP, "persistent recurrence aborted (code " + std::to_string(code) +
                                   ": 1 = hand-off timeout, 2 = workgroup placement, 4 = dG beyond its fp16 planes); the results of this step are "
                                   "invalid, later steps use the per-step kernels" +
                                   (ls->rearm_wait > 0 ? " (the persistent kernels are tried again after " +
                                                            std::to_string(ls->rearm_wait) + " clean steps)"
                                                      : ""));
}

void rec_rearm(nasr_ctx* h) {
  LstmState* const ls = h->lstm.get();
  if (!ls || ls->rec_use != RecKind::Step || !ls->rec_wanted || ls->persist_aborts == 0 || ls->rearm_wait <= 0) return;
  if (++ls->clean_steps <= ls->rearm_wait) return;
  ls->clean_steps = 0;
  if (hipStreamSynchronize(h->st) != hipSuccess) return;
  ls->rec_use = ls->rec_kind;
  if (repack(h) != NASR_OK || (ls->rec_kind == RecKind::Persist && !persist_census(h))) {
    ls->rec_use = RecKind::Step;
    ls->rearm_wait = std::min<int64_t>(ls->rearm_wait * 2, (int64_t)1 << 20);
    (void)repack(h);
    return;
  }
  ls->rec_refused = false;
  ls->persist_rearms += 1;
  drop_graphs(h);
}

std::vector<TphScaleJob> rec_scale_jobs(const nasr_ctx* h) {
  const LstmState* const ls = h->lstm.get();
  std::vector<TphScaleJob> jobs;
  for (size_t k = 0; k < ls->off_u.size(); ++k) {
    const float* U = h->P + ls->off_u[k];
    if (ls->rec_use == RecKind::Persist && ls->rec_f16)
      jobs.push_back({U, ls->Hp, ls->N4, ls->N4, nullptr, nullptr, ls->Ucs + k * ls->N4, ls->Ucinv + k * ls->N4});
    else if (ls->rec_use == RecKind::Wide)
      jobs.push_back({U, ls->Hp, ls->N4, ls->N4, ls->Urs + k * ls->Hp, ls->Urinv + k * ls->Hp, ls->Ucs + k * ls->N4, ls->Ucinv + k * ls->N4});
  }
  return jobs;
}

static void step_images(nasr_ctx* h) {
  LstmState* const ls = h->lstm.get();
  for (size_t k = 0; k < ls->off_u.size(); ++k)
    launch_repack_u(h->P + ls->off_u[k], ls->Uf + k * ls->Hp * ls->N4, ls->Ub + k * ls->Hp * ls->N4, ls->Hp, h->st);
  ls->step_img_seq = ls->repack_seq;
}

void rec_images(nasr_ctx* h) {
  LstmState* const ls = h->lstm.get();
  if (ls->rec_use == RecKind::Persist) {
    launch_repack_persist(h->P, ls->off_u.data(), (int)ls->off_u.size(), ls->Upf, ls->Upb, ls->Hp, ls->rec_f16 ? ls->Ucs : nullptr, h->st);
  } else if (ls->rec_use == RecKind::Wide) {
    for (size_t k = 0; k < ls->off_u.size(); ++k) {
      const float* U = h->P + ls->off_u[k];
      launch_repack_wide(U, ls->Ucs + k * ls->N4, ls->Uw + k * wide_image_bytes(ls->Hp), ls->Hp, h->st);
      launch_repack_wide_bwd(U, ls->Urs + k * ls->Hp, ls->Uwb + k * wide_image_bytes(ls->Hp), ls->Hp, h->st);
    }
  } else {
    step_images(h);
  }
}

void ensure_step_images(nasr_ctx* h) {
  LstmState* const ls = h->lstm.get();
  if (ls->rec_use != RecKind::Step && ls->step_img_seq != ls->repack_seq) step_images(h);
}

}

extern "C" int nasr_get_recurrence_mode(nasr_handle h) {
  MODEL_CALL(h);
  LSTM_CALL(h, "has no recurrence");
  return h ? (int)h->lstm->rec_use : 0;
}

extern "C" int nasr_set_recurrence_mode(nasr_handle h, int persistent) {
  MODEL_CALL(h);
  if (!h) return NASR_ERR_ARG;
  LSTM_CALL(h, "has no recurrence");
  LstmState* const ls = h->lstm.get();
  if (persistent && ls->rec_kind != RecKind::Wide && (ls->rec_kind == RecKind::Step || ls->rec_refused))
    return h->fail(NASR_ERR_STATE, "the persistent recurrence is not available on this device / hidden size");
  HIPCHK(h, hipStreamSynchronize(h->st));
  ls->rec_use = persistent ? ls->rec_kind : RecKind::Step;
  ls->rec_wanted = persistent != 0;
  return repack(h);
}
```

Baseline: 1.252 million.

## Fuse split-K reduce with CTC logZ, add narrow GEMM tile, merge persist clears

```diff
diff --git a/neuralasr_amd/build.py b/neuralasr_amd/build.py
--- a/neuralasr_amd/build.py
+++ b/neuralasr_amd/build.py
@@ -8,9 +8,9 @@
 LIB = os.path.join(HERE, 'libnasr.so')
 KT_LIB = os.path.join(HERE, 'libnasr_kt.so')
 KT_DIR = os.path.join(HERE, '..', 'tests', 'kernel_harness')
-KT_SRCS = ['harness.hip', 'rec_harness.hip']
+KT_SRCS = ['harness.hip', 'rec_harness.hip', 'small_harness.hip']
 KT_HEADERS = [os.path.join(KT_DIR, 'arena.h')]
-KT_OBJS = ['gemm.o', 'gemm_tph.o', 'optim.o', 'lstm.o', 'lstm_persist.o', 'lstm_wide.o']
+KT_OBJS = ['gemm.o', 'gemm_tph.o', 'optim.o', 'lstm.o', 'lstm_persist.o', 'lstm_wide.o', 'ctc.o']
 SOURCES = ['gemm.hip', 'gemm_tph.hip', 'lstm.hip', 'rows.hip', 'lstm_persist.hip', 'lstm_wide.hip', 'ctc.hip', 'dense.hip', 'optim.hip', 'nasr_layout.hip',
            'nasr_rec.hip', 'nasr_batch.hip', 'nasr_pass.hip', 'nasr_stream.hip', 'nasr_lstm.hip', 'nasr_api.hip', 'nasr_comm.hip', 'beam.cpp',
            'wavenet.hip', 'nasr_wavenet.hip', 'las.hip', 'las_beam.hip', 'nasr_las.hip', 'mfcc.hip', 'nasr_fz.hip', 'resample.hip', 'wave_aug.hip']
diff --git a/neuralasr_amd/csrc/ctc.hip b/neuralasr_amd/csrc/ctc.hip
--- a/neuralasr_amd/csrc/ctc.hip
+++ b/neuralasr_amd/csrc/ctc.hip
@@ -57,6 +57,21 @@
 }
 
 static bool ctc_fast_ok(const CtcDims& d) { return d.lprobs && d.goff && d.Cp == 32 && d.C <= 31 && d.KS >= 2; }
+
+template <class X>
+__device__ __forceinline__ void ctc_logz_row(X x, int lane, int row, float* __restrict__ logz, float* __restrict__ lprobs, int C,
+                                             int Cp) {
+  float m = NEG;
+  for (int c = lane; c < C; c += 64) m = fmaxf(m, x(c));
+  m = wave_max(m);
+  float s = 0.f;
+  for (int c = lane; c < C; c += 64) s += __expf(x(c) - m);
+  s = wave_sum(s);
+  const float z = m + __logf(s);
+  if (lane == 0) logz[row] = z;
+  if (lprobs)
+    for (int c = lane; c < Cp; c += 64) lprobs[(size_t)row * Cp + c] = c < C ? (x(c) - z) * 1.44269504088896341f : NEG;
+}
 
 __global__ __launch_bounds__(256) void ctc_logz_kernel(const float* __restrict__ logits, const int* __restrict__ seq_len,
                                                        float* __restrict__ logz, float* __restrict__ lprobs, int Tp, int B, int Bp,
@@ -67,22 +82,44 @@
   const int t = row / Bp, b = row % Bp;
   if (b >= B || t >= seq_len[b]) return;
   const float* x = logits + (size_t)row * Cp;
-  float m = NEG;
-  for (int c = lane; c < C; c += 64) m = fmaxf(m, x[c]);
-  m = wave_max(m);
-  float s = 0.f;
-  for (int c = lane; c < C; c += 64) s += __expf(x[c] - m);
-  s = wave_sum(s);
-  const float z = m + __logf(s);
-  if (lane == 0) logz[row] = z;
-  if (lprobs)
-    for (int c = lane; c < Cp; c += 64) lprobs[(size_t)row * Cp + c] = c < C ? (x[c] - z) * 1.44269504088896341f : NEG;
+  ctc_logz_row([x](int c) { return x[c]; }, lane, row, logz, lprobs, C, Cp);
 }
 
 void launch_ctc_logz(const CtcDims& d, const float* logits, const int* seq_len, float* logz, hipStream_t st) {
   const int rows = d.Tp * d.Bp;
   hipLaunchKernelGGL(ctc_logz_kernel, dim3((rows + 3) / 4), dim3(256), 0, st, logits, seq_len, logz, ctc_fast_ok(d) ? d.lprobs : nullptr,
                      d.Tp, d.B, d.Bp, d.C, d.Cp);
+}
+
+__global__ __launch_bounds__(256) void ctc_reduce_logz_kernel(const float* __restrict__ slabs, int S, const float* __restrict__ bias,
+                                                              float* __restrict__ logits, const int* __restrict__ seq_len,
+                                                              float* __restrict__ logz, float* __restrict__ lprobs, int Tp, int B,
+                                                              int Bp, int C) {
+  constexpr int Cp = 32;
+  const int rows = Tp * Bp;
+  const int row = blockIdx.x * 4 + (threadIdx.x >> 6);
+  const int lane = threadIdx.x & 63;
+  if (row >= rows) return;
+  float v = 0.f;
+  if (lane < Cp) {
+    const size_t e = (size_t)row * Cp + lane;
+    v = slabs[e];
+    for (int k = 1; k < S; ++k) v += slabs[(size_t)k * rows * Cp + e];
+    if (bias) v += bias[lane];
+    logits[e] = v;
+  }
+  const int t = row / Bp, b = row % Bp;
+  if (b >= B || t >= seq_len[b]) return;
+  ctc_logz_row([v](int) { return v; }, lane, row, logz, lprobs, C, Cp);
+}
+
+bool ctc_reduce_logz_ok(const CtcDims& d) { return d.Cp == 32 && d.C <= 32; }
+
+void launch_ctc_reduce_logz(const CtcDims& d, const float* slabs, int S, const float* bias, float* logits, const int* seq_len,
+                            float* logz, hipStream_t st) {
+  const int rows = d.Tp * d.Bp;
+  hipLaunchKernelGGL(ctc_reduce_logz_kernel, dim3((rows + 3) / 4), dim3(256), 0, st, slabs, S, bias, logits, seq_len, logz,
+                     ctc_fast_ok(d) ? d.lprobs : nullptr, d.Tp, d.B, d.Bp, d.C);
 }
 
 template <int KS>
diff --git a/neuralasr_amd/csrc/gemm.hip b/neuralasr_amd/csrc/gemm.hip
--- a/neuralasr_amd/csrc/gemm.hip
+++ b/neuralasr_amd/csrc/gemm.hip
@@ -29,25 +29,29 @@
   return make_float4(ok ? v.x : 0.f, ok ? v.y : 0.f, ok ? v.z : 0.f, ok ? v.w : 0.f);
 }
 
-template <bool ACOL, bool BCOL>
+template <bool ACOL, bool BCOL, int TBN>
 __global__ __launch_bounds__(256, 2) void gemm_kernel(GemmParams p) {
-  __shared__ __attribute__((aligned(16))) float As[2][BK][LDT];
-  __shared__ __attribute__((aligned(16))) float Bs[2][BK][LDT];
+  constexpr int TBK = TBN == BN ? BK : 32;
+  constexpr int LDB = TBN + 4;
+  constexpr int MI = TBN == BN ? 2 : 1, NI = MI;
+  __shared__ __attribute__((aligned(16))) float As[2][TBK][LDT];
+  __shared__ __attribute__((aligned(16))) float Bs[2][TBK][LDB];
   const int tid = threadIdx.x, lane = tid & 63, w = tid >> 6;
-  const int m0 = blockIdx.y * BM, n0 = blockIdx.x * BN;
+  const int m0 = blockIdx.y * BM, n0 = blockIdx.x * TBN;
   const int kbeg = blockIdx.z * p.kchunk;
   const int kend = min(p.K, kbeg + p.kchunk);
-  const int nk = (kend - kbeg + BK - 1) / BK;
+  const int nk = (kend - kbeg + TBK - 1) / TBK;
   const float* __restrict__ Ag = p.A;
   const float* __restrict__ Bg = p.B;
 
-  constexpr int NS = BK / 8, KQ = BK / 4;
-  bool aok[NS], bok[NS];
-  size_t ao[NS], bo[NS];
-#pragma unroll
-  for (int j = 0; j < NS; ++j) {
+  constexpr int NSA = BM * TBK / 1024, NSB = TBN * TBK / 1024, KQ = TBK / 4, QA = BM / 4, QB = TBN / 4;
+  static_assert(NSA >= 1 && NSB >= 1, "every thread owns a slot of either operand");
+  bool aok[NSA], bok[NSB];
+  size_t ao[NSA], bo[NSB];
+#pragma unroll
+  for (int j = 0; j < NSA; ++j) {
     const int idx = tid + 256 * j;
-    const int r = idx / KQ, kq = idx % KQ, q = idx & 31;
+    const int r = idx / KQ, kq = idx % KQ, q = idx % QA;
     if (!ACOL) {
       const int pa = (m0 + r < p.M) ? phys_row(p.a_map, p.a_shift, p.a_rows, m0 + r) : -1;
       aok[j] = pa >= 0;
@@ -56,6 +60,11 @@
       aok[j] = (m0 + 4 * q < p.M);
       ao[j] = aok[j] ? (size_t)(m0 + 4 * q) : 0;
     }
+  }
+#pragma unroll
+  for (int j = 0; j < NSB; ++j) {
+    const int idx = tid + 256 * j;
+    const int r = idx / KQ, kq = idx % KQ, q = idx % QB;
     if (BCOL) {
       bok[j] = n0 + r < p.N;
       bo[j] = bok[j] ? (size_t)(n0 + r) * p.ldb + 4 * kq : 0;
@@ -65,37 +74,43 @@
     }
   }
 
-  float4 ra[NS], rb[NS];
+  float4 ra[NSA], rb[NSB];
 #define NASR_GLOAD(K0)                                                                              \
-  _Pragma("unroll") for (int j = 0; j < NS; ++j) {                                                  \
-    const int kk_ = (tid + 256 * j) >> 5;                                                           \
-    const bool kr_ = (K0) + 4 * ((tid + 256 * j) % KQ) < kend, kc_ = (K0) + kk_ < kend;             \
+  _Pragma("unroll") for (int j = 0; j < NSA; ++j) {                                                 \
+    const int kk_ = (tid + 256 * j) / QA;                                                           \
     if (!ACOL) {                                                                                    \
-      const bool o_ = aok[j] && kr_;                                                                \
+      const bool o_ = aok[j] && (K0) + 4 * ((tid + 256 * j) % KQ) < kend;                           \
       ra[j] = sel4(o_, ld4(Ag + (o_ ? ao[j] + (K0) : 0)));                                          \
     } else {                                                                                        \
-      const int pr_ = kc_ ? phys_row(p.a_map, p.a_shift, p.a_rows, (K0) + kk_) : -1;                \
+      const int pr_ = (K0) + kk_ < kend ? phys_row(p.a_map, p.a_shift, p.a_rows, (K0) + kk_) : -1;  \
       const bool o_ = aok[j] && pr_ >= 0;                                                           \
       ra[j] = sel4(o_, ld4(Ag + (o_ ? (size_t)pr_ * p.lda + ao[j] : 0)));                           \
     }                                                                                               \
+  }                                                                                                 \
+  _Pragma("unroll") for (int j = 0; j < NSB; ++j) {                                                 \
+    const int kk_ = (tid + 256 * j) / QB;                                                           \
     if (BCOL) {                                                                                     \
-      const bool o_ = bok[j] && kr_;                                                                \
+      const bool o_ = bok[j] && (K0) + 4 * ((tid + 256 * j) % KQ) < kend;                           \
       rb[j] = sel4(o_, ld4(Bg + (o_ ? bo[j] + (K0) : 0)));                                          \
     } else {                                                                                        \
-      const bool o_ = bok[j] && kc_;                                                                \
+      const bool o_ = bok[j] && (K0) + kk_ < kend;                                                  \
       rb[j] = sel4(o_, ld4(Bg + (o_ ? (size_t)((K0) + kk_) * p.ldb + bo[j] : 0)));                  \
     }                                                                                               \
   }
 #define NASR_LSTORE(BUF)                                                                            \
-  _Pragma("unroll") for (int j = 0; j < NS; ++j) {                                                  \
+  _Pragma("unroll") for (int j = 0; j < NSA; ++j) {                                                 \
     const int idx_ = tid + 256 * j;                                                                 \
-    const int r_ = idx_ / KQ, kq_ = idx_ % KQ, kk_ = idx_ >> 5, q_ = idx_ & 31;                     \
+    const int r_ = idx_ / KQ, kq_ = idx_ % KQ, kk_ = idx_ / QA, q_ = idx_ % QA;                     \
     if (!ACOL) {                                                                                    \
       As[BUF][4 * kq_ + 0][r_] = ra[j].x; As[BUF][4 * kq_ + 1][r_] = ra[j].y;                       \
       As[BUF][4 * kq_ + 2][r_] = ra[j].z; As[BUF][4 * kq_ + 3][r_] = ra[j].w;                       \
     } else {                                                                                        \
       *reinterpret_cast<float4*>(&As[BUF][kk_][4 * q_]) = ra[j];                                    \
     }                                                                                               \
+  }                                                                                                 \
+  _Pragma("unroll") for (int j = 0; j < NSB; ++j) {                                                 \
+    const int idx_ = tid + 256 * j;                                                                 \
+    const int r_ = idx_ / KQ, kq_ = idx_ % KQ, kk_ = idx_ / QB, q_ = idx_ % QB;                     \
     if (BCOL) {                                                                                     \
       Bs[BUF][4 * kq_ + 0][r_] = rb[j].x; Bs[BUF][4 * kq_ + 1][r_] = rb[j].y;                       \
       Bs[BUF][4 * kq_ + 2][r_] = rb[j].z; Bs[BUF][4 * kq_ + 3][r_] = rb[j].w;                       \
@@ -104,11 +119,15 @@
     }                                                                                               \
   }
 
-  f32x16 acc00, acc01, acc10, acc11;
-#pragma unroll
-  for (int r = 0; r < 16; ++r) { acc00[r] = 0.f; acc01[r] = 0.f; acc10[r] = 0.f; acc11[r] = 0.f; }
-
-  const int wm = (w >> 1) * 64, wn = (w & 1) * 64;
+  f32x16 acc[MI][NI];
+#pragma unroll
+  for (int mi = 0; mi < MI; ++mi)
+#pragma unroll
+    for (int ni = 0; ni < NI; ++ni)
+#pragma unroll
+      for (int r = 0; r < 16; ++r) acc[mi][ni][r] = 0.f;
+
+  const int wm = TBN == BN ? (w >> 1) * 64 : w * 32, wn = TBN == BN ? (w & 1) * 64 : 0;
   const int li = lane & 31, lk = lane >> 5;
 
   if (nk > 0) {
@@ -119,22 +138,39 @@
   for (int kt = 0; kt < nk; ++kt) {
     const int buf = kt & 1;
     const bool more = kt + 1 < nk;
-    if (more) NASR_GLOAD(kbeg + (kt + 1) * BK);
-    float a0 = As[buf][lk][wm + li], a1 = As[buf][lk][wm + 32 + li];
-    float b0 = Bs[buf][lk][wn + li], b1 = Bs[buf][lk][wn + 32 + li];
-#pragma unroll
-    for (int ks = 0; ks < BK / 2; ++ks) {
-      float na0 = 0.f, na1 = 0.f, nb0 = 0.f, nb1 = 0.f;
-      if (ks + 1 < BK / 2) {
-        const int k = 2 * (ks + 1) + lk;
-        na0 = As[buf][k][wm + li]; na1 = As[buf][k][wm + 32 + li];
-        nb0 = Bs[buf][k][wn + li]; nb1 = Bs[buf][k][wn + 32 + li];
+    if (more) NASR_GLOAD(kbeg + (kt + 1) * TBK);
+#pragma unroll
+    for (int kh = 0; kh < TBK; kh += BK) {
+      if (kh > 0 && kbeg + kt * TBK + kh >= kend) break;
+      float a[MI], b[NI];
+#pragma unroll
+      for (int i = 0; i < MI; ++i) a[i] = As[buf][kh + lk][wm + 32 * i + li];
+#pragma unroll
+      for (int i = 0; i < NI; ++i) b[i] = Bs[buf][kh + lk][wn + 32 * i + li];
+#pragma unroll
+      for (int ks = 0; ks < BK / 2; ++ks) {
+        float na[MI], nb[NI];
+#pragma unroll
+        for (int i = 0; i < MI; ++i) na[i] = 0.f;
+#pragma unroll
+        for (int i = 0; i < NI; ++i) nb[i] = 0.f;
+        if (ks + 1 < BK / 2) {
+          const int k = kh + 2 * (ks + 1) + lk;
+#pragma unroll
+          for (int i = 0; i < MI; ++i) na[i] = As[buf][k][wm + 32 * i + li];
+#pragma unroll
+          for (int i = 0; i < NI; ++i) nb[i] = Bs[buf][k][wn + 32 * i + li];
+        }
+#pragma unroll
+        for (int mi = 0; mi < MI; ++mi)
+#pragma unroll
+          for (int ni = 0; ni < NI; ++ni)
+            acc[mi][ni] = __builtin_amdgcn_mfma_f32_32x32x2f32(a[mi], b[ni], acc[mi][ni], 0, 0, 0);
+#pragma unroll
+        for (int i = 0; i < MI; ++i) a[i] = na[i];
+#pragma unroll
+        for (int i = 0; i < NI; ++i) b[i] = nb[i];
       }
-      acc00 = __builtin_amdgcn_mfma_f32_32x32x2f32(a0, b0, acc00, 0, 0, 0);
-      acc01 = __builtin_amdgcn_mfma_f32_32x32x2f32(a0, b1, acc01, 0, 0, 0);
-      acc10 = __builtin_amdgcn_mfma_f32_32x32x2f32(a1, b0, acc10, 0, 0, 0);
-      acc11 = __builtin_amdgcn_mfma_f32_32x32x2f32(a1, b1, acc11, 0, 0, 0);
-      a0 = na0; a1 = na1; b0 = nb0; b1 = nb1;
     }
     if (more) NASR_LSTORE(buf ^ 1);
     __syncthreads();
@@ -143,24 +179,24 @@
 #undef NASR_LSTORE
 
 #pragma unroll
-  for (int t = 0; t < 4; ++t) {
-    const int mi = t >> 1, ni = t & 1;
-    const f32x16 acc = t == 0 ? acc00 : t == 1 ? acc01 : t == 2 ? acc10 : acc11;
-    const int col = n0 + wn + 32 * ni + li;
-    if (col >= p.N) continue;
-    const float bv = (p.bias && p.split_k == 1) ? p.bias[col] : 0.f;
-#pragma unroll
-    for (int r = 0; r < 16; ++r) {
-      const int row = m0 + wm + 32 * mi + (r & 3) + 8 * (r >> 2) + 4 * lk;
-      if (row >= p.M) continue;
-      if (p.split_k > 1) {
-        p.slabs[((size_t)blockIdx.z * p.M + row) * p.N + col] = acc[r];
-      } else {
-        const int pr = p.c_map ? p.c_map[row] : row;
-        if (pr >= 0) p.C[(size_t)pr * p.ldc + col] = acc[r] + bv;
+  for (int mi = 0; mi < MI; ++mi)
+#pragma unroll
+    for (int ni = 0; ni < NI; ++ni) {
+      const int col = n0 + wn + 32 * ni + li;
+      if (col >= p.N) continue;
+      const float bv = (p.bias && p.split_k == 1) ? p.bias[col] : 0.f;
+#pragma unroll
+      for (int r = 0; r < 16; ++r) {
+        const int row = m0 + wm + 32 * mi + (r & 3) + 8 * (r >> 2) + 4 * lk;
+        if (row >= p.M) continue;
+        if (p.split_k > 1) {
+          p.slabs[((size_t)blockIdx.z * p.M + row) * p.N + col] = acc[mi][ni][r];
+        } else {
+          const int pr = p.c_map ? p.c_map[row] : row;
+          if (pr >= 0) p.C[(size_t)pr * p.ldc + col] = acc[mi][ni][r] + bv;
+        }
       }
     }
-  }
 }
 
 __global__ __launch_bounds__(256) void gemm_reduce_kernel(GemmParams p) {
@@ -168,9 +204,18 @@
   for (int64_t i = blockIdx.x * (int64_t)blockDim.x + threadIdx.x; i < n4; i += (int64_t)gridDim.x * blockDim.x) {
     const int64_t e = i * 4;
     const int row = (int)(e / p.N), col = (int)(e % p.N);
+    const size_t slab = (size_t)p.M * p.N;
     float4 s = *reinterpret_cast<const float4*>(p.slabs + e);
-    for (int k = 1; k < p.split_k; ++k) {
-      const float4 v = *reinterpret_cast<const float4*>(p.slabs + (size_t)k * p.M * p.N + e);
+    int k = 1;
+    for (; k + 8 <= p.split_k; k += 8) {
+      float4 v[8];
+#pragma unroll
+      for (int j = 0; j < 8; ++j) v[j] = *reinterpret_cast<const float4*>(p.slabs + (size_t)(k + j) * slab + e);
+#pragma unroll
+      for (int j = 0; j < 8; ++j) { s.x += v[j].x; s.y += v[j].y; s.z += v[j].z; s.w += v[j].w; }
+    }
+    for (; k < p.split_k; ++k) {
+      const float4 v = *reinterpret_cast<const float4*>(p.slabs + (size_t)k * slab + e);
       s.x += v.x; s.y += v.y; s.z += v.z; s.w += v.w;
     }
     if (p.bias) { s.x += p.bias[col]; s.y += p.bias[col + 1]; s.z += p.bias[col + 2]; s.w += p.bias[col + 3]; }
@@ -188,28 +233,41 @@
   return s;
 }
 
+int gemm_splits(int K, int split_k) {
+  if (split_k < 1) split_k = 1;
+  const int kt = (K + BK - 1) / BK, per = (kt + split_k - 1) / split_k;
+  return (kt + per - 1) / per;
+}
+
+template <int TBN>
+static void launch_gemm_tile(const GemmDesc& g, const GemmParams& p, hipStream_t st) {
+  dim3 grid((g.N + TBN - 1) / TBN, (g.M + BM - 1) / BM, p.split_k), block(256);
+  if (!g.a_col && !g.b_col) hipLaunchKernelGGL((gemm_kernel<false, false, TBN>), grid, block, 0, st, p);
+  else if (g.a_col && !g.b_col) hipLaunchKernelGGL((gemm_kernel<true, false, TBN>), grid, block, 0, st, p);
+  else if (!g.a_col && g.b_col) hipLaunchKernelGGL((gemm_kernel<false, true, TBN>), grid, block, 0, st, p);
+  else hipLaunchKernelGGL((gemm_kernel<true, true, TBN>), grid, block, 0, st, p);
+}
+
 void launch_gemm(const GemmDesc& g, hipStream_t st) {
   GemmParams p;
   p.A = g.A; p.B = g.B; p.C = g.C;
   p.M = g.M; p.N = g.N; p.K = g.K; p.lda = g.lda; p.ldb = g.ldb; p.ldc = g.ldc;
   p.a_map = g.a_map; p.a_shift = g.a_shift; p.a_rows = g.a_rows; p.c_map = g.c_map; p.bias = g.bias;
+  p.slabs = g.slabs;
   p.split_k = g.split_k < 1 ? 1 : g.split_k;
-  p.slabs = g.slabs;
-  int kt = (g.K + BK - 1) / BK;
-  int per = (kt + p.split_k - 1) / p.split_k;
+  const int kt = (g.K + BK - 1) / BK;
+  const int per = (kt + p.split_k - 1) / p.split_k;
   p.kchunk = per * BK;
   p.split_k = (kt + per - 1) / per;
-  dim3 grid((g.N + BN - 1) / BN, (g.M + BM - 1) / BM, p.split_k), block(256);
-  if (!g.a_col && !g.b_col) hipLaunchKernelGGL((gemm_kernel<false, false>), grid, block, 0, st, p);
-  else if (g.a_col && !g.b_col) hipLaunchKernelGGL((gemm_kernel<true, false>), grid, block, 0, st, p);
-  else if (!g.a_col && g.b_col) hipLaunchKernelGGL((gemm_kernel<false, true>), grid, block, 0, st, p);
-  else hipLaunchKernelGGL((gemm_kernel<true, true>), grid, block, 0, st, p);
-  if (p.split_k > 1) {
+  if (g.bn == 32 || (g.bn == 0 && g.N <= 32)) launch_gemm_tile<32>(g, p, st);
+  else launch_gemm_tile<BN>(g, p, st);
+  if (p.split_k > 1 && !g.no_reduce) {
     int64_t n4 = (int64_t)g.M * g.N / 4;
-    int blocks = (int)((n4 + 255) / 256);
+    const int bs = n4 < 65536 ? 64 : 256;
+    int blocks = (int)((n4 + bs - 1) / bs);
     if (blocks > 2048) blocks = 2048;
-    hipLaunchKernelGGL(gemm_reduce_kernel, dim3(blocks), dim3(256), 0, st, p);
-  }
-}
-
-}
+    hipLaunchKernelGGL(gemm_reduce_kernel, dim3(blocks), dim3(bs), 0, st, p);
+  }
+}
+
+}
diff --git a/neuralasr_amd/csrc/kernels.h b/neuralasr_amd/csrc/kernels.h
--- a/neuralasr_amd/csrc/kernels.h
+++ b/neuralasr_amd/csrc/kernels.h
@@ -21,9 +21,12 @@
   const float* bias;
   int split_k;
   float* slabs;
+  int bn;
+  bool no_reduce;
 };
 void launch_gemm(const GemmDesc& g, hipStream_t st);
 int gemm_pick_split(int M, int N, int K);
+int gemm_splits(int K, int split_k);
 
 int tp_split2_parts(int rows);
 int gemm_tp_tile_rows(int M);
@@ -186,6 +189,9 @@
   double* goff = nullptr;
 };
 void launch_ctc_logz(const CtcDims& d, const float* logits, const int* seq_len, float* logz, hipStream_t st);
+bool ctc_reduce_logz_ok(const CtcDims& d);
+void launch_ctc_reduce_logz(const CtcDims& d, const float* slabs, int S, const float* bias, float* logits, const int* seq_len,
+                            float* logz, hipStream_t st);
 void launch_ctc_alpha_beta(const CtcDims& d, const float* logits, const float* logz, const int* labels,
                            const int* label_len, const int* seq_len, float* alpha, float* beta, double* aoff,
                            double* boff, float* nll, double* logp, hipStream_t st);
diff --git a/neuralasr_amd/csrc/nasr_batch.hip b/neuralasr_amd/csrc/nasr_batch.hip
--- a/neuralasr_amd/csrc/nasr_batch.hip
+++ b/neuralasr_amd/csrc/nasr_batch.hip
@@ -73,6 +73,12 @@
     for (int i = 0; i < ls->ndense; ++i) { ipmax = std::max(ipmax, ls->dIp[i]); wmax = std::max(wmax, ls->dWp[i]); }
     ok &= ls->XTP.ensure(tph_bytes((int)R, ipmax), &grew);
     ok &= ls->X0TTP.ensure(tph_bytes(ls->Ip[0], (int)R), &grew);
+    if (ls->npre == 0) {
+      bool g0 = false;
+      ok &= ls->X0TP.ensure(tph_bytes((int)R, ls->Ip[0]), &g0);
+      if (g0) ls->x0tp_valid = false;
+      grew |= g0;
+    }
     for (int l = 0; l < ls->L; ++l) ok &= ls->OTT[l].ensure(tph_bytes(D * Hp, (int)R), &grew);
     ok &= ls->GTP.ensure(tph_bytes((int)R, wmax), &grew);
     ok &= ls->GTTP.ensure(tph_bytes(wmax, (int)R), &grew);
@@ -467,9 +473,12 @@
     if (h->cmp_rows)
       launch_gather_rows(ls->sc_cx.sp(), ls->sc_x0r.sp(), h->vrow_p, h->cmp_rows_p, 1.f, h->st),
       launch_gather_rows(ls->sc_cx.ip(), ls->sc_x0r.ip(), h->vrow_p, h->cmp_rows_p, 1.f, h->st);
-    if (ls && s->has_labels && ls->npre == 0)
-      launch_tph_split2(h->X0.as<float>(), nullptr, ls->X0TTP.as<unsigned char>(), h->cmp_rows ? h->cmp_rows : ls->Tv * Bp, h->Fp, h->Fp,
-                        nullptr, 1.f, ls->sc_x0c.sp(), 1.f, nullptr, h->st, h->cmp_rows ? h->vrow_p : nullptr);
+    if (ls) ls->x0tp_valid = ls->npre == 0 && !s->chunk && !lc;
+    if (ls && ls->npre == 0 && (s->has_labels || ls->x0tp_valid))
+      launch_tph_split2(h->X0.as<float>(), ls->x0tp_valid ? ls->X0TP.as<unsigned char>() : nullptr,
+                        s->has_labels ? ls->X0TTP.as<unsigned char>() : nullptr, h->cmp_rows ? h->cmp_rows : ls->Tv * Bp, h->Fp, h->Fp,
+                        h->cmp_rows ? ls->sc_cx.sp() : ls->sc_x0r.sp(), 1.f, s->has_labels ? ls->sc_x0c.sp() : nullptr, 1.f, nullptr,
+                        h->st, h->cmp_rows ? h->vrow_p : nullptr);
     HIPCHK(h, hipGetLastError());
   }
   h->resident = true;
diff --git a/neuralasr_amd/csrc/nasr_ctx.h b/neuralasr_amd/csrc/nasr_ctx.h
--- a/neuralasr_amd/csrc/nasr_ctx.h
+++ b/neuralasr_amd/csrc/nasr_ctx.h
@@ -208,6 +208,7 @@
   uint32_t stamp_seq = 0;
 
   bool resident = false, have_grads = false, have_fwd = false;
+  bool logz_fwd = false;
   int B = 0, Bp = 0, T = 0, Lmax = 0, Tp = 0, KS = 1;
   int64_t frames = 0;
   std::vector<int32_t> h_seq;
diff --git a/neuralasr_amd/csrc/nasr_lstm.h b/neuralasr_amd/csrc/nasr_lstm.h
--- a/neuralasr_amd/csrc/nasr_lstm.h
+++ b/neuralasr_amd/csrc/nasr_lstm.h
@@ -73,6 +73,8 @@
   int dgmax_layer = -1;
   DevBuf dgmax;
   DevBuf XTP, X0TTP, GTP, GTTP;
+  DevBuf X0TP;
+  bool x0tp_valid = false;
   std::vector<DevBuf> OTT;
   std::vector<char> ott_valid;
   DevBuf csws;
@@ -92,9 +94,10 @@
   bool rec_f16 = false;
   DevPtr<float> Upf, Upb;
   size_t imf = 0, imb = 0;
-  DevPtr<float> xchf;
-  DevPtr<float> xchb;
   DevPtr<PersistCtl> pctl;
+  float* xchf = nullptr;
+  float* xchb = nullptr;
+  size_t pclear_bytes = 0;
   DevPtr<unsigned char> Uw;
   DevPtr<unsigned char> Uwb;
   DevPtr<float> Urs, Urinv;
diff --git a/neuralasr_amd/csrc/nasr_pass.hip b/neuralasr_amd/csrc/nasr_pass.hip
--- a/neuralasr_amd/csrc/nasr_pass.hip
+++ b/neuralasr_amd/csrc/nasr_pass.hip
@@ -125,11 +125,13 @@
   ActScale as = lstm_in_scale(ls, l);
   if (vm && l == 0) { as.rs = ls->sc_cx.sp(); as.rinv = ls->sc_cx.ip(); }
   const bool both = l > 0 && h->cur && h->cur->has_labels;
-  launch_tph_split2(lstm_input(h, l), ls->XTP.as<unsigned char>(), both ? ls->OTT[l - 1].as<unsigned char>() : nullptr, rows, Ip, Ip,
-                    as.rs, 1.f, both ? as.cs : nullptr, 1.f, nullptr, st, vm);
+  const bool pre = l == 0 && ls->x0tp_valid && !test_hook("NASR_X0_SPLIT_IN_STEP");
+  if (!pre)
+    launch_tph_split2(lstm_input(h, l), ls->XTP.as<unsigned char>(), both ? ls->OTT[l - 1].as<unsigned char>() : nullptr, rows, Ip, Ip,
+                      as.rs, 1.f, both ? as.cs : nullptr, 1.f, nullptr, st, vm);
   if (l > 0) ls->ott_valid[l - 1] = both;
   GemmTPHDesc g{};
-  g.A = ls->XTP.as<unsigned char>(); g.B = ls->WfTP + ls->off_wftp[l]; g.C = ls->gates[l].as<float>();
+  g.A = (pre ? ls->X0TP : ls->XTP).as<unsigned char>(); g.B = ls->WfTP + ls->off_wftp[l]; g.C = ls->gates[l].as<float>();
   g.M = rows; g.N = D * N4; g.K = Ip; g.nkbA = (Ip + 15) / 16; g.nkbB = g.nkbA; g.ldc = D * N4;
   g.bias = h->P + ls->off_bias[l]; g.split_k = 1;
   g.c_map = vm;
@@ -245,10 +247,8 @@
   h->n_fwd_launch = 0;
   std::fill(ls->ott_valid.begin(), ls->ott_valid.end(), 0);
   if (!chunk) HIPCHK(h, hipMemsetAsync(h->Gbase, 0, GRAD_HEAD * 4, h->st));
-  if (ls->rec_use == RecKind::Persist && !chunk && !lc) {
-    HIPCHK(h, hipMemsetAsync(ls->pctl + 1, 0, (size_t)ls->L * sizeof(PersistCtl), h->st));
-    HIPCHK(h, hipMemsetAsync(ls->xchf, 0, (size_t)ls->L * persist_hx_bytes(ls->Hp), h->st));
-  }
+  if (ls->rec_use == RecKind::Persist && !chunk && !lc)
+    HIPCHK(h, hipMemsetAsync(ls->pctl + 1, 0, ls->pclear_bytes, h->st));
   for (int i = 0; i < ls->npre; ++i) {
     PhaseScope ps(h, PH_XPROJ);
     int rc = dense_forward(h, i, i == 0 ? h->X0.as<float>() : ls->Ybuf[i - 1].as<float>());
@@ -289,7 +289,15 @@
     g.a_rows = sr ? 2 * R : R;
     g.bias = h->P + ls->off_b;
     g.split_k = gemm_pick_split(g.M, g.N, g.K);
+    const CtcDims d = ctc_dims(h);
+    h->logz_fwd = !chunk && !sr && gemm_splits(g.K, g.split_k) > 1 && ctc_reduce_logz_ok(d);
+    g.no_reduce = h->logz_fwd;
     if (int rc = gemm_f32(h, g)) return rc;
+    if (h->logz_fwd) {
+      launch_ctc_reduce_logz(d, h->slabs.as<float>(), gemm_splits(g.K, g.split_k), g.bias, h->logits.as<float>(), h->seq_p,
+                             h->logz.as<float>(), h->st);
+      HIPCHK(h, hipGetLastError());
+    }
   }
   h->have_fwd = !chunk;
   return NASR_OK;
@@ -306,7 +314,8 @@
 int ctc_forward(nasr_ctx* h) {
   PhaseScope ps(h, PH_PROJCTC);
   const CtcDims d = ctc_dims(h);
-  launch_ctc_logz(d, h->logits.as<float>(), h->seq_p, h->logz.as<float>(), h->st);
+  if (!h->logz_fwd) launch_ctc_logz(d, h->logits.as<float>(), h->seq_p, h->logz.as<float>(), h->st);
+  h->logz_fwd = false;
   launch_ctc_alpha_beta(d, h->logits.as<float>(), h->logz.as<float>(), h->labels_p, h->lablen_p,
                         h->seq_p, h->alpha.as<float>(), h->beta.as<float>(), h->aoff.as<double>(),
                         h->boff.as<double>(), h->nll.as<float>(), h->logp.as<double>(), h->st);
@@ -445,10 +454,6 @@
   const bool sr = ls->cfg.merge == NASR_MERGE_STACK_RESHAPE && D == 2;
   const bool lc = ls->lc_live;
   const RecKind use = lc ? RecKind::Step : ls->rec_use;
-  if (use == RecKind::Persist) {
-    HIPCHK(h, hipMemsetAsync(ls->pctl + 1 + ls->L, 0, (size_t)ls->L * sizeof(PersistCtl), h->st));
-    HIPCHK(h, hipMemsetAsync(ls->xchb, 0, (size_t)ls->L * persist_px_bytes(), h->st));
-  }
   {
     PhaseScope ps(h, PH_PROJCTC);
     const CtcDims d = ctc_dims(h);
diff --git a/neuralasr_amd/csrc/nasr_rec.hip b/neuralasr_amd/csrc/nasr_rec.hip
--- a/neuralasr_amd/csrc/nasr_rec.hip
+++ b/neuralasr_amd/csrc/nasr_rec.hip
@@ -45,12 +45,17 @@
   if (ls->rec_kind == RecKind::Persist) {
     ls->imf = persist_image_floats(ls->Hp, false);
     ls->imb = persist_image_floats(ls->Hp, true);
+    auto rup256 = [](size_t n) { return (n + 255) / 256 * 256; };
+    const size_t ctl_bytes = rup256((1 + 2 * (size_t)ls->L) * sizeof(PersistCtl));
+    const size_t hx_bytes = rup256((size_t)ls->L * persist_hx_bytes(ls->Hp)), px_bytes = (size_t)ls->L * persist_px_bytes();
     if (persist_prepare() != hipSuccess || hipMalloc(ls->Upf.out(), nk * ls->imf * 4) != hipSuccess ||
         hipMalloc(ls->Upb.out(), nk * ls->imb * 4) != hipSuccess ||
-        hipMalloc(ls->xchf.out(), (size_t)ls->L * persist_hx_bytes(ls->Hp)) != hipSuccess ||
-        hipMalloc(ls->xchb.out(), (size_t)ls->L * persist_px_bytes()) != hipSuccess ||
-        hipMalloc(ls->pctl.out(), (size_t)(1 + 2 * ls->L) * sizeof(PersistCtl)) != hipSuccess)
+        hipMalloc(ls->pctl.out(), ctl_bytes + hx_bytes + px_bytes) != hipSuccess)
       return h->fail(NASR_ERR_HIP, "allocation of the persistent-recurrence buffers failed");
+    char* const arena = reinterpret_cast<char*>(ls->pctl.get());
+    ls->xchf = reinterpret_cast<float*>(arena + ctl_bytes);
+    ls->xchb = reinterpret_cast<float*>(arena + ctl_bytes + hx_bytes);
+    ls->pclear_bytes = ctl_bytes + hx_bytes + px_bytes - sizeof(PersistCtl);
     (void)hipMemsetAsync(ls->Upf, 0, nk * ls->imf * 4, h->st);
     (void)hipMemsetAsync(ls->Upb, 0, nk * ls->imb * 4, h->st);
     return NASR_OK;
```

New measurement: 1.264 million, median of 6. No clear change (+0.9%).
